# noahares/raxtax

Hardware: AMD Instinct MI355X
Metric: classified queries/sec (whole node) (higher is better)
Workload: dtype u32 bit-planes + f64

## Files before the change

include/raxtax_hip.h:

```cpp
#ifndef RAXTAX_HIP_H
#define RAXTAX_HIP_H

#include <stddef.h>
#include <stdint.h>

#ifdef __cplusplus
extern "C" {
#endif

#define RTX_ABI_VERSION 6
#define RTX_NUM_KMERS 65536u
#define RTX_MAX_DEPTH 32u

#define RTX_OK 0
#define RTX_ERR_INVALID (-1)
#define RTX_ERR_HIP (-2)
#define RTX_ERR_NO_DEVICE (-3)
#define RTX_ERR_OOM (-4)
#define RTX_ERR_PARSE (-5)
#define RTX_ERR_DEPTH (-6)
#define RTX_ERR_STATE (-7)
#define RTX_ERR_TOO_LONG (-8)
#define RTX_ERR_SENDER (-9)
#define RTX_RETRY_CHUNK 1
// ... 48 lines not shown
typedef struct rtx_queries rtx_queries;
int rtx_queries_parse_fasta(const char *text, uint64_t len, const char *const *skip, uint64_t n_skip,
                            rtx_queries **out);
#define RTX_FASTA_MORE_FOLLOWS 1u
#define RTX_FASTA_NOT_FIRST 2u
uint64_t rtx_fasta_block_end(const char *text, uint64_t len);
int rtx_queries_parse_fasta_block(const char *text, uint64_t len, const char *const *skip, uint64_t n_skip, uint32_t flags,
                                  rtx_queries **out);
void rtx_queries_destroy(rtx_queries *q);
uint64_t rtx_queries_len(const rtx_queries *q);
const char *rtx_queries_label(const rtx_queries *q, uint64_t i);
int rtx_queries_data(const rtx_queries *q, const uint8_t **bases, const uint64_t **base_off);

int rtx_index_create(int device, uint64_t n_refs, const uint64_t *offsets ,
                     const uint32_t *postings, uint32_t n_nodes, const uint32_t *node_begin,
                     const uint32_t *node_end, const uint32_t *node_first_child,
                     const uint32_t *node_n_children, const uint8_t *node_type, rtx_index **out);
int rtx_index_create_shard(int device, uint64_t n_refs_total, uint64_t ref_lo, uint64_t ref_hi,
                           const uint64_t *shard_cuts, uint32_t n_cuts, const uint64_t *offsets,
                           const uint32_t *postings, uint32_t n_nodes, const uint32_t *node_begin,
                           const uint32_t *node_end, const uint32_t *node_first_child,
                           const uint32_t *node_n_children, const uint8_t *node_type, rtx_index **out);
int rtx_index_create_from_sequences(int device, uint64_t n_refs, const uint8_t *seq_bytes, const uint64_t *seq_off,
                                    uint32_t n_nodes, const uint32_t *node_begin, const uint32_t *node_end,
                                    const uint32_t *node_first_child, const uint32_t *node_n_children,
                                    const uint8_t *node_type, rtx_index **out);
int rtx_index_create_from_tree(int device, const rtx_tree *tree, rtx_index **out);
void rtx_index_destroy(rtx_index *index);
uint64_t rtx_index_num_refs(const rtx_index *index);
uint64_t rtx_index_device_bytes(const rtx_index *index);
uint64_t rtx_index_workspace_bytes(const rtx_index *index);
int rtx_index_workspace_parts(const rtx_index *index, uint64_t out[9]);
int rtx_index_set_batch(rtx_index *index, uint32_t sub_batch);
#define RTX_OPT_SUB_BATCH 1
#define RTX_OPT_PROB_MODE 2
#define RTX_OPT_STAGE_TIMING 6
#define RTX_OPT_DEBUG_TAPS 14
#define RTX_OPT_DEVICE_EXACT 15
#define RTX_OPT_CLUSTER 7
#define RTX_OPT_PACKED_COUNTS 8
#define RTX_OPT_HIT_PAIR 11
#define RTX_OPT_TILE_SKIP 10
#define RTX_OPT_LOCATOR 12
#define RTX_OPT_TILE_PRUNE 13
#define RTX_OPT_FINE_BOUNDS 17
#define RTX_OPT_RECORDS 18
#define RTX_OPT_OVERLAP 19
#define RTX_OPT_MIN_SUB_BATCHES 20
#define RTX_OPT_TWO_LEVEL_BOUNDS 21
#define RTX_OPT_PRUNE_SELF_SAMPLE 22
#define RTX_OPT_RUN_AHEAD 23
#define RTX_OPT_DEVICE_TEXT 24
#define RTX_OPT_STRAND 25
int rtx_index_set_option(rtx_index *index, int option, uint64_t value);

int rtx_index_self_sample(rtx_index *index, const uint8_t *seq_bytes, const uint64_t *seq_off, uint64_t n_refs, uint32_t n_sample, double *live_fraction);
int rtx_index_prune_verdict(const rtx_index *index, int *pruning, double *live_fraction);
int rtx_index_run_ahead_stats(const rtx_index *index, uint64_t *enqueued_ahead, uint64_t *abandoned);
#define RTX_DEFAULT_SEGMENT_CLASSES 1
#define RTX_DEFAULT_EXACT_HASH_MASK 2
int rtx_set_default_option(int option, uint64_t value);

typedef struct {
    uint32_t n_queries;
    uint64_t n_rows;
    const uint32_t *t;
    const uint8_t *status;
    const double *global_signal;
    const uint64_t *row_begin;
    const uint32_t *row_count;
    const uint32_t *row_lineage;
    const uint32_t *row_node;
    const uint32_t *row_depth;
    const double *row_conf;
    const double *row_local_signal;
    uint32_t row_conf_stride;
    const uint8_t *row_depth_u8;
    const uint8_t *row_conf_hundredths;
} rtx_result_view;

int rtx_batch_prefetch(rtx_index *index, uint64_t n_queries, const uint8_t *bases, const uint64_t *base_off,
                       const uint32_t *exact_ids, const uint64_t *exact_off);
int rtx_batch_activate(rtx_index *index);
int rtx_pack_bases(const uint8_t *bases, uint64_t n_bases, uint8_t *packed);
int rtx_classify_batch(rtx_index *index, uint64_t n_queries, const uint8_t *bases,
                       const uint64_t *base_off, const uint32_t *exact_ids,
                       const uint64_t *exact_off, uint32_t flags, rtx_result_view *out);
int rtx_index_has_exact_lookup(const rtx_index *index);
int rtx_batch_exact_matches(rtx_index *index, const uint64_t **exact_off , const uint32_t **exact_ids);

int rtx_batch_strands(rtx_index *index, const uint8_t **strand, const uint32_t **peak);
int rtx_revcomp(const uint8_t *in, uint64_t n, uint8_t *out);

int rtx_batch_upload(rtx_index *index, uint64_t n_queries, const uint8_t *bases,
                     const uint64_t *base_off, const uint32_t *exact_ids,
                     const uint64_t *exact_off);
int rtx_batch_run(rtx_index *index, uint32_t flags);
int rtx_batch_sync(rtx_index *index);
int rtx_batch_download(rtx_index *index, rtx_result_view *out);
int rtx_batch_download_then_run(rtx_index *index, rtx_result_view *out, uint32_t flags);

typedef struct {
    uint64_t n_queries;
    const char *out;
    const uint64_t *out_off;
    const char *tsv;
    const uint64_t *tsv_off;
} rtx_text_view;
int rtx_index_text_setup(rtx_index *index, const rtx_tree *tree, uint32_t flags);
int rtx_batch_prefetch_labels(rtx_index *index, uint64_t n_queries, const char *const *labels);
int rtx_batch_text(rtx_index *index, rtx_text_view *out);

#define RTX_BUF_HIST 1
#define RTX_BUF_PREFIX 2
int rtx_shard_begin(rtx_index *index, uint32_t *n_sub_batches, uint32_t *sub_batch);
#define RTX_OPT_SHARD_PRUNE 16
int rtx_shard_prunes(const rtx_index *index);
int rtx_shard_bounds(rtx_index *index, uint32_t sub_batch_idx, uint32_t flags);
int rtx_shard_count(rtx_index *index, uint32_t sub_batch_idx, uint32_t flags);
int rtx_shard_prob(rtx_index *index, uint32_t sub_batch_idx);
int rtx_shard_walk(rtx_index *index, uint32_t sub_batch_idx, const double *prefix_global );
int rtx_shard_info(const rtx_index *index, uint64_t *ref_lo, uint64_t *ref_hi, uint32_t *n_bnd_global,
                   uint32_t *n_bnd_local, uint32_t *first_bnd);
int rtx_device_buffer(rtx_index *index, int which, void **device_ptr, uint64_t *row_stride_elems);
#define RTX_BUF_COUNTS 3
#define RTX_BUF_BEST 4
int rtx_shard_buffer(rtx_index *index, uint32_t sub_batch_idx, int which, void **device_ptr, uint64_t *row_stride_elems);
int rtx_shard_rehist(rtx_index *index, uint32_t sub_batch_idx);
int rtx_index_stream(rtx_index *index, void **hip_stream);

#define RTX_STAGE_KMER_EXTRACT 0
#define RTX_STAGE_HIT_COUNT 1
#define RTX_STAGE_PROB_TABLE 2
#define RTX_STAGE_TAXON_PREFIX 3
#define RTX_STAGE_LINEAGE_WALK 4
#define RTX_STAGE_TILE_BOUNDS 5
#define RTX_STAGE_TILE_PRUNE 6
#define RTX_STAGE_EXACT_MATCH 7
#define RTX_STAGE_ORDER 8
#define RTX_STAGE_PAIR_UNION 9
#define RTX_NUM_STAGES 10
int rtx_batch_stage_times(rtx_index *index, float ms[RTX_NUM_STAGES], uint32_t launches[RTX_NUM_STAGES]);
int rtx_batch_work(rtx_index *index, uint64_t *sum_hits, uint64_t *sum_query_bytes,
                   uint64_t *bitmap_bytes_read);
int rtx_batch_work_split(rtx_index *index, uint64_t *live_bytes, uint64_t *bounds_bytes);
int rtx_batch_prob_work(rtx_index *index, uint64_t *sum_grid_points, uint64_t *sum_distinct_counts);

int rtx_debug_kmers(rtx_index *index, uint64_t query, uint16_t *kmers , uint32_t *t);
int rtx_debug_hit_counts(rtx_index *index, uint64_t query, uint16_t *counts );
int rtx_debug_prob_table(rtx_index *index, uint64_t query, double *table_over_z , double *z);
int rtx_debug_probs(rtx_index *index, uint64_t query, double *probs );
int rtx_debug_tile_bounds(rtx_index *index, uint64_t query, uint16_t *tile_ub );
int rtx_debug_order(rtx_index *index, uint32_t *perm );
int rtx_batch_sub_batch(const rtx_index *index, uint32_t *sub_batch, uint32_t *n_sub_batches);
int rtx_batch_last_sub_batch(const rtx_index *index, uint64_t *first, uint32_t *n);
int rtx_batch_classes(const rtx_index *index, uint32_t *n_classes, uint64_t out[20]);
int rtx_debug_prune_stats(rtx_index *index, uint64_t *out );
int rtx_debug_pruned_prob_table(rtx_index *index, uint64_t query, double *table_over_z , double *z, uint32_t *threshold);
int rtx_debug_run_counts(rtx_index *index, uint64_t query, uint16_t *counts , uint8_t *tile_live ,
                         uint32_t *hist , uint32_t *threshold, uint32_t *i1);
int rtx_debug_run_mode(rtx_index *index, uint64_t query, uint32_t *n_segments);
int rtx_debug_prune_detail(rtx_index *index, uint64_t query, uint32_t *out );
int rtx_debug_evaluate(rtx_index *index, const double *probs , rtx_result_view *out);

int64_t rtx_format_query(const rtx_tree *tree, const rtx_result_view *res, uint64_t q,
                         const char *label, const uint8_t *seq, uint64_t seq_len,
                         const uint32_t *exact_ids, uint64_t n_exact, uint32_t flags, char *out_buf,
                         uint64_t out_cap, char *tsv_buf, uint64_t tsv_cap, int64_t *tsv_len);

int64_t rtx_result_pack(const rtx_result_view *res, uint8_t *buf, uint64_t cap);

#define RTX_NEED_BASE 1024
int64_t rtx_records_format(const rtx_tree *tree, const uint8_t *records, uint64_t n_bytes, const char *const *labels,
                           const uint32_t *exact_one, uint32_t flags, char *out, uint64_t cap, uint64_t *line_off, uint32_t threads);

typedef int (*rtx_sender_fn)(void *ctx, const char *label, const char *out_lines, const char *tsv_lines);
int rtx_raxtax(rtx_index *index, const rtx_tree *tree, uint64_t n_queries, const char *const *labels,
               const uint8_t *bases, const uint64_t *base_off, int skip_exact_matches, int raw_confidence,
               uint64_t chunk_size, rtx_sender_fn sender, void *sender_ctx, int tsv);

int rtx_raxtax_multi(rtx_index *const *indices, uint32_t n_indices, const rtx_tree *tree, uint64_t n_queries,
                     const char *const *labels, const uint8_t *bases, const uint64_t *base_off, int skip_exact_matches,
                     int raw_confidence, uint64_t chunk_size, rtx_sender_fn sender, void *sender_ctx, int tsv);
typedef int (*rtx_query_info_fn)(void *ctx, const char *label, int strand, uint32_t peak, uint32_t t);
int rtx_raxtax_multi_ex(rtx_index *const *indices, uint32_t n_indices, const rtx_tree *tree, uint64_t n_queries,
                        const char *const *labels, const uint8_t *bases, const uint64_t *base_off, int skip_exact_matches,
                        int raw_confidence, uint64_t chunk_size, rtx_sender_fn sender, void *sender_ctx, int tsv,
                        rtx_query_info_fn info, void *info_ctx);
int rtx_sender_discard(void *ctx, const char *label, const char *out_lines, const char *tsv_lines);
int rtx_raxtax_last_timing(double busy[4], uint64_t *n_chunks);

int rtx_set_host_share(uint32_t n_ranks_on_this_host);
uint32_t rtx_host_threads(void);

#ifdef __cplusplus
}
#endif
#endif
```

raxtax_amd/_build.py:

```python
from __future__ import annotations

import os
import shutil
import subprocess
from pathlib import Path

PKG = Path(__file__).resolve().parent
ROOT = PKG.parent
CSRC = PKG / "csrc"
LIB = PKG / "libraxtax_hip.so"
SOURCES = ["rtx_kernels.hip", "rtx_hit_pair.hip", "rtx_prob_tables.hip", "rtx_cluster.hip", "rtx_segments.hip", "rtx_prune.hip", "rtx_bounds2.hip", "rtx_records.hip", "rtx_finalise.hip", "rtx_text.hip", "rtx_exact.hip", "rtx_strand.hip", "rtx_ingest.hip", "rtx_api_index.hip", "rtx_api_batch.hip", "rtx_api_download.hip", "rtx_api_shard.hip", "rtx_api_debug.hip", "host_tree.cpp", "host_format.cpp", "host_raxtax.cpp", "host_bin.cpp", "host_threads.cpp"]
HEADERS = ["rtx_index.hpp", "rtx_kernels.hpp", "rtx_hit_common.hpp", "rtx_internal.hpp", "rtx_math.hpp", "rtx_wave.hpp", "rtx_walk.hpp", "host_raxtax.hpp"]
CLI = PKG / "raxtax-hip"
SYNTH = PKG / "raxtax-synth"


def _hipcc() -> str:
    for c in (os.environ.get("HIPCC"), shutil.which("hipcc"), "/opt/rocm/bin/hipcc"):
        if c and Path(c).exists():
            return c
    raise RuntimeError("hipcc not found (ROCm toolchain required to build libraxtax_hip.so)")


def _stale(target: Path, deps) -> bool:
    if not target.exists():
        return True
    t = target.stat().st_mtime
    return any(Path(d).stat().st_mtime > t for d in deps if Path(d).exists())


OBJ = PKG / "_obj"


def build_lib(force: bool = False, verbose: bool = False) -> Path:
    from concurrent.futures import ThreadPoolExecutor

    srcs = [CSRC / s for s in SOURCES if (CSRC / s).exists()]
    hdrs = [CSRC / h for h in HEADERS] + [ROOT / "include" / "raxtax_hip.h"]
    if not force and not _stale(LIB, srcs + hdrs):
        return LIB
    OBJ.mkdir(exist_ok=True)
    flags = ["--offload-arch=gfx950", "-O3", "-std=c++17", "-fPIC", f"-I{ROOT / 'include'}", f"-I{CSRC}"] + os.environ.get("RTX_EXTRA_CXXFLAGS", "").split()

    def compile_one(src: Path) -> Path:
        obj = OBJ / (src.name + ".o")
        if force or _stale(obj, [src] + hdrs):
            cmd = [_hipcc()] + flags + ["-x", "hip", "-c", str(src), "-o", str(obj)]
            if verbose:
                print(" ".join(cmd))
            subprocess.check_call(cmd)
        return obj

    with ThreadPoolExecutor(max_workers=min(len(srcs), os.cpu_count() or 1)) as ex:
        objs = list(ex.map(compile_one, srcs))
    cmd = [_hipcc(), "--offload-arch=gfx950", "-fPIC", "-shared", "-o", str(LIB)] + [str(o) for o in objs] + ["-lpthread"]
    if verbose:
        print(" ".join(cmd))
    subprocess.check_call(cmd)
    return LIB


def build_cli(force: bool = False) -> Path | None:
    main = CSRC / "cli_main.cpp"
    if not main.exists():
        return None
# ... 21 lines not shown
```

raxtax_amd/_lib.py:

```python
from __future__ import annotations

import ctypes as C
from pathlib import Path

import numpy as np

PKG = Path(__file__).resolve().parent
import os as _os

LIB_PATH = Path(_os.environ.get("RTX_LIB_PATH") or PKG / "libraxtax_hip.so")

RTX_MAX_DEPTH = 32
RTX_NUM_KMERS = 65536
RTX_OK = 0
RTX_ERR_INVALID, RTX_ERR_HIP, RTX_ERR_NO_DEVICE, RTX_ERR_OOM = -1, -2, -3, -4
RTX_ERR_PARSE, RTX_ERR_DEPTH, RTX_ERR_STATE, RTX_ERR_TOO_LONG = -5, -6, -7, -8
RTX_SKIP_EXACT_MATCHES = 1
RTX_RAW_CONFIDENCE = 2
RTX_TEXT_TSV = 4
RTX_Q_OK, RTX_Q_NO_KMERS, RTX_Q_ALL_KMERS = 0, 1, 2
STAGES = ("kmer_extract", "hit_count", "prob_table", "taxon_prefix", "lineage_walk", "tile_bounds", "tile_prune", "exact_match", "order", "pair_union")

u8p = C.POINTER(C.c_uint8)
u16p = C.POINTER(C.c_uint16)
# ... 56 lines not shown
    "rtx_index_create": (C.c_int, [C.c_int, C.c_uint64, u64p, u32p, C.c_uint32, u32p, u32p, u32p, u32p, u8p,
                                   C.POINTER(C.c_void_p)]),
    "rtx_index_create_shard": (C.c_int, [C.c_int, C.c_uint64, C.c_uint64, C.c_uint64, u64p, C.c_uint32, u64p, u32p, C.c_uint32,
                                        u32p, u32p, u32p, u32p, u8p, C.POINTER(C.c_void_p)]),
    "rtx_shard_begin": (C.c_int, [C.c_void_p, u32p, u32p]),
    "rtx_shard_count": (C.c_int, [C.c_void_p, C.c_uint32, C.c_uint32]),
    "rtx_shard_bounds": (C.c_int, [C.c_void_p, C.c_uint32, C.c_uint32]),
    "rtx_shard_prunes": (C.c_int, [C.c_void_p]),
    "rtx_shard_prob": (C.c_int, [C.c_void_p, C.c_uint32]),
    "rtx_shard_walk": (C.c_int, [C.c_void_p, C.c_uint32, C.c_void_p]),
    "rtx_shard_info": (C.c_int, [C.c_void_p, u64p, u64p, u32p, u32p, u32p]),
    "rtx_device_buffer": (C.c_int, [C.c_void_p, C.c_int, C.POINTER(C.c_void_p), u64p]),
    "rtx_shard_buffer": (C.c_int, [C.c_void_p, C.c_uint32, C.c_int, C.POINTER(C.c_void_p), u64p]),
    "rtx_shard_rehist": (C.c_int, [C.c_void_p, C.c_uint32]),
    "rtx_index_stream": (C.c_int, [C.c_void_p, C.POINTER(C.c_void_p)]),
    "rtx_index_create_from_sequences": (C.c_int, [C.c_int, C.c_uint64, u8p, u64p, C.c_uint32, u32p, u32p, u32p, u32p, u8p,
                                                 C.POINTER(C.c_void_p)]),
    "rtx_index_create_from_tree": (C.c_int, [C.c_int, C.c_void_p, C.POINTER(C.c_void_p)]),
    "rtx_index_destroy": (None, [C.c_void_p]),
    "rtx_index_num_refs": (C.c_uint64, [C.c_void_p]),
    "rtx_index_device_bytes": (C.c_uint64, [C.c_void_p]),
    "rtx_index_workspace_bytes": (C.c_uint64, [C.c_void_p]),
    "rtx_index_workspace_parts": (C.c_int, [C.c_void_p, u64p]),
    "rtx_index_set_batch": (C.c_int, [C.c_void_p, C.c_uint32]),
    "rtx_set_default_option": (C.c_int, [C.c_int, C.c_uint64]),
    "rtx_index_set_option": (C.c_int, [C.c_void_p, C.c_int, C.c_uint64]),
    "rtx_index_self_sample": (C.c_int, [C.c_void_p, C.c_void_p, C.c_void_p, C.c_uint64, C.c_uint32, C.POINTER(C.c_double)]),
    "rtx_index_prune_verdict": (C.c_int, [C.c_void_p, C.POINTER(C.c_int), C.POINTER(C.c_double)]),
    "rtx_index_run_ahead_stats": (C.c_int, [C.c_void_p, C.POINTER(C.c_uint64), C.POINTER(C.c_uint64)]),
    "rtx_classify_batch": (C.c_int, [C.c_void_p, C.c_uint64, u8p, u64p, u32p, u64p, C.c_uint32,
                                     C.POINTER(ResultView)]),
    "rtx_index_has_exact_lookup": (C.c_int, [C.c_void_p]),
    "rtx_batch_exact_matches": (C.c_int, [C.c_void_p, C.POINTER(u64p), C.POINTER(u32p)]),
    "rtx_batch_upload": (C.c_int, [C.c_void_p, C.c_uint64, u8p, u64p, u32p, u64p]),
    "rtx_batch_run": (C.c_int, [C.c_void_p, C.c_uint32]),
    "rtx_batch_sync": (C.c_int, [C.c_void_p]),
    "rtx_batch_download": (C.c_int, [C.c_void_p, C.POINTER(ResultView)]),
    "rtx_batch_download_then_run": (C.c_int, [C.c_void_p, C.POINTER(ResultView), C.c_uint32]),
    "rtx_index_text_setup": (C.c_int, [C.c_void_p, C.c_void_p, C.c_uint32]),
    "rtx_batch_prefetch_labels": (C.c_int, [C.c_void_p, C.c_uint64, C.POINTER(C.c_char_p)]),
    "rtx_batch_text": (C.c_int, [C.c_void_p, C.POINTER(TextView)]),
    "rtx_batch_stage_times": (C.c_int, [C.c_void_p, f32p, u32p]),
    "rtx_batch_work": (C.c_int, [C.c_void_p, u64p, u64p, u64p]),
    "rtx_batch_prob_work": (C.c_int, [C.c_void_p, u64p, u64p]),
    "rtx_batch_work_split": (C.c_int, [C.c_void_p, u64p, u64p]),
    "rtx_debug_kmers": (C.c_int, [C.c_void_p, C.c_uint64, u16p, u32p]),
    "rtx_debug_hit_counts": (C.c_int, [C.c_void_p, C.c_uint64, u16p]),
    "rtx_debug_prob_table": (C.c_int, [C.c_void_p, C.c_uint64, f64p, f64p]),
    "rtx_debug_pruned_prob_table": (C.c_int, [C.c_void_p, C.c_uint64, f64p, f64p, u32p]),
    "rtx_debug_probs": (C.c_int, [C.c_void_p, C.c_uint64, f64p]),
    "rtx_debug_order": (C.c_int, [C.c_void_p, u32p]),
    "rtx_debug_tile_bounds": (C.c_int, [C.c_void_p, C.c_uint64, u16p]),
    "rtx_debug_prune_stats": (C.c_int, [C.c_void_p, u64p]),
    "rtx_debug_run_counts": (C.c_int, [C.c_void_p, C.c_uint64, u16p, u8p, u32p, u32p, u32p]),
    "rtx_debug_run_mode": (C.c_int, [C.c_void_p, C.c_uint64, u32p]),
    "rtx_batch_last_sub_batch": (C.c_int, [C.c_void_p, u64p, u32p]),
    "rtx_batch_classes": (C.c_int, [C.c_void_p, u32p, u64p]),
    "rtx_debug_prune_detail": (C.c_int, [C.c_void_p, C.c_uint64, u32p]),
    "rtx_debug_evaluate": (C.c_int, [C.c_void_p, f64p, C.POINTER(ResultView)]),
    "rtx_result_pack": (C.c_int64, [C.POINTER(ResultView), u8p, C.c_uint64]),
    "rtx_records_format": (C.c_int64, [C.c_void_p, u8p, C.c_uint64, C.POINTER(C.c_char_p), u32p, C.c_uint32, C.c_char_p, C.c_uint64, u64p, C.c_uint32]),
    "rtx_format_query": (C.c_int64, [C.c_void_p, C.POINTER(ResultView), C.c_uint64, C.c_char_p, u8p, C.c_uint64,
                                     u32p, C.c_uint64, C.c_uint32, C.c_char_p, C.c_uint64, C.c_char_p, C.c_uint64,
                                     C.POINTER(C.c_int64)]),
    "rtx_raxtax": (C.c_int, None),
    "rtx_raxtax_multi": (C.c_int, None),
    "rtx_raxtax_multi_ex": (C.c_int, None),
    "rtx_batch_strands": (C.c_int, [C.c_void_p, C.POINTER(u8p), C.POINTER(u32p)]),
    "rtx_revcomp": (C.c_int, [u8p, C.c_uint64, u8p]),
    "rtx_sender_discard": (C.c_int, [C.c_void_p, C.c_char_p, C.c_char_p, C.c_char_p]),
    "rtx_batch_prefetch": (C.c_int, [C.c_void_p, C.c_uint64, u8p, u64p, u32p, u64p]),
    "rtx_batch_activate": (C.c_int, [C.c_void_p]),
    "rtx_pack_bases": (C.c_int, [u8p, C.c_uint64, u8p]),
    "rtx_batch_sub_batch": (C.c_int, [C.c_void_p, C.POINTER(C.c_uint32), C.POINTER(C.c_uint32)]),
    "rtx_raxtax_last_timing": (C.c_int, [C.POINTER(C.c_double), C.POINTER(C.c_uint64)]),
    "rtx_set_host_share": (C.c_int, [C.c_uint32]),
    "rtx_host_threads": (C.c_uint32, []),
}

_lib = None


def load() -> C.CDLL:
    global _lib
    if _lib is not None:
        return _lib
    if not LIB_PATH.exists():
        raise ImportError(
            f"{LIB_PATH} is missing: build it with `python -m raxtax_amd._build` (hipcc, gfx950). "
            "raxtax_amd has no CPU fallback.")
    try:
        import torch
    except Exception:
        pass
    lib = C.CDLL(str(LIB_PATH))
    for name, (res, args) in _SIGNATURES.items():
        fn = getattr(lib, name)
        fn.restype = res
        if args is not None:
            fn.argtypes = args
    _lib = lib
    return lib


def check(code: int):
    if code < 0:
# ... 7 lines not shown
```

raxtax_amd/api.py:

```python
from __future__ import annotations

import ctypes as C
from dataclasses import dataclass
from typing import Callable, List, Optional, Sequence, Tuple

import numpy as np

from . import _lib
from ._lib import (RTX_MAX_DEPTH, RTX_RAW_CONFIDENCE, RTX_SKIP_EXACT_MATCHES, NodesView, ResultView, RtxError, check,
                   f32p, f64p, ptr, u8p, u16p, u32p, u64p)


def _flatten(seqs: Sequence[np.ndarray]) -> Tuple[np.ndarray, np.ndarray]:
    off = np.zeros(len(seqs) + 1, dtype=np.uint64)
    if len(seqs):
        off[1:] = np.cumsum([len(s) for s in seqs], dtype=np.uint64)
    flat = np.zeros(max(int(off[-1]), 1), dtype=np.uint8)
    for i, s in enumerate(seqs):
        flat[int(off[i]):int(off[i + 1])] = np.asarray(s, dtype=np.uint8)
    return flat, off


class Tree:

# ... 125 lines not shown
class EvaluationResult:
    lineage: int
    node: int
    confidence_values: List[float]
    local_signal: float
    global_signal: float


class Result:

    def __init__(self, view: ResultView, strand: Optional[np.ndarray] = None, peak: Optional[np.ndarray] = None):
        nq, nr = view.n_queries, view.n_rows
        self.strand, self.peak = strand, peak
        arr = lambda p, n: (np.ctypeslib.as_array(p, shape=(n,)).copy() if n else np.zeros(0))
        self.n_queries = nq
        self.t = arr(view.t, nq)
        self.status = arr(view.status, nq)
        self.global_signal = arr(view.global_signal, nq)
        begin = arr(view.row_begin, nq).astype(np.int64)
        count = arr(view.row_count, nq).astype(np.int64)
        self.row_off = np.zeros(nq + 1, dtype=np.uint64)
        self.row_off[1:] = np.cumsum(count)
        src = (np.repeat(begin - self.row_off[:-1].astype(np.int64), count) + np.arange(int(count.sum()))) if nq else np.zeros(0, np.int64)
        assert len(src) <= nr
        self.row_lineage = arr(view.row_lineage, nr)[src]
        self.row_node = arr(view.row_node, nr)[src]
        self.row_depth = arr(view.row_depth, nr)[src]
        stride = int(view.row_conf_stride) or RTX_MAX_DEPTH
        self.row_conf = (np.ctypeslib.as_array(view.row_conf, shape=(nr, stride))[src] if nr
                         else np.zeros((0, stride)))
        self.row_local_signal = arr(view.row_local_signal, nr)[src]

    def rows(self, q: int) -> List[EvaluationResult]:
        out = []
        for r in range(int(self.row_off[q]), int(self.row_off[q + 1])):
            d = int(self.row_depth[r])
            out.append(EvaluationResult(int(self.row_lineage[r]), int(self.row_node[r]),
                                        [float(x) for x in self.row_conf[r, :d]],
                                        float(self.row_local_signal[r]), float(self.global_signal[q])))
        return out


DEFAULT_SEGMENT_CLASSES = 1


class Index:

    def __init__(self, tree: Tree, device: int = 0, sub_batch: int = 0, prob_mode: int = 0,
                 stage_timing: bool = False, cluster: Optional[bool] = None, segment_classes=None,
                 packed_counts: Optional[bool] = None,
                 tile_skip: Optional[bool] = None, hit_pair=None, locator: Optional[bool] = None, tile_prune: Optional[bool] = None,
                 debug_taps: bool = False, device_exact: Optional[bool] = None, fine_bounds: Optional[bool] = None,
                 records: Optional[int] = None, overlap: Optional[bool] = None, two_level: Optional[int] = None,
                 prune_self_sample: Optional[bool] = None, device_text: bool = False, strand: str = "plus"):
        self._lib = _lib.load()
        self.tree = tree
        if segment_classes is None:
            segment_classes = DEFAULT_SEGMENT_CLASSES
        check(self._lib.rtx_set_default_option(1, int(segment_classes)))
        h = C.c_void_p()
        check(self._lib.rtx_index_create_from_tree(device, tree._h, C.byref(h)))
        self._h = h
        self.n_refs = self._lib.rtx_index_num_refs(self._h)
        if sub_batch:
            check(self._lib.rtx_index_set_batch(self._h, sub_batch))
        if prob_mode:
            check(self._lib.rtx_index_set_option(self._h, 2, prob_mode))
        if stage_timing:
            check(self._lib.rtx_index_set_option(self._h, 6, 1))
        if cluster is not None:
            check(self._lib.rtx_index_set_option(self._h, 7, int(cluster)))
        if packed_counts is not None:
            check(self._lib.rtx_index_set_option(self._h, 8, int(packed_counts)))
        if tile_skip is not None:
            check(self._lib.rtx_index_set_option(self._h, 10, int(tile_skip)))
        if hit_pair is not None:
            check(self._lib.rtx_index_set_option(self._h, 11, int(hit_pair)))
        if locator is not None:
            check(self._lib.rtx_index_set_option(self._h, 12, int(locator)))
        if tile_prune is not None:
            check(self._lib.rtx_index_set_option(self._h, 13, int(tile_prune)))
            if tile_prune and prune_self_sample is None:
                check(self._lib.rtx_index_set_option(self._h, 22, 0))
        if debug_taps:
            check(self._lib.rtx_index_set_option(self._h, 14, 1))
        if device_exact is not None:
            check(self._lib.rtx_index_set_option(self._h, 15, int(device_exact)))
        if device_text:
            check(self._lib.rtx_index_set_option(self._h, 24, 1))
        if fine_bounds is not None:
            check(self._lib.rtx_index_set_option(self._h, 17, int(fine_bounds)))
        if records is not None:
            check(self._lib.rtx_index_set_option(self._h, 18, int(records)))
        if overlap is not None:
            check(self._lib.rtx_index_set_option(self._h, 19, int(overlap)))
        if two_level is not None:
            check(self._lib.rtx_index_set_option(self._h, 21, int(two_level)))
        if prune_self_sample is not None:
            check(self._lib.rtx_index_set_option(self._h, 22, int(prune_self_sample)))
        if strand not in ("plus", "both"):
            raise ValueError(f"strand must be 'plus' or 'both', not {strand!r}")
        self.strand = strand
        if strand == "both":
            check(self._lib.rtx_index_set_option(self._h, 25, 1))
        self._view = ResultView()
        self._keep = None

    @property
    def prune_verdict(self):
        on, frac = C.c_int(), C.c_double()
        check(self._lib.rtx_index_prune_verdict(self._h, C.byref(on), C.byref(frac)))
        return bool(on.value), float(frac.value)

    @property
    def run_ahead_stats(self):
        a, b = C.c_uint64(), C.c_uint64()
        check(self._lib.rtx_index_run_ahead_stats(self._h, C.byref(a), C.byref(b)))
        return int(a.value), int(b.value)

    def __del__(self):
        try:
            if self._h:
                self._lib.rtx_index_destroy(self._h)
                self._h = None
        except Exception:
            pass

    @property
    def device_bytes(self) -> int:
        return self._lib.rtx_index_device_bytes(self._h)

    @property
    def workspace_bytes(self) -> int:
        return self._lib.rtx_index_workspace_bytes(self._h)

    def workspace_parts(self) -> dict:
        out = np.zeros(9, dtype=np.uint64)
        check(self._lib.rtx_index_workspace_parts(self._h, ptr(out, u64p)))
        names = ("prob_tables", "counts", "record_segments", "prefix_sums", "tile_masks_and_slot_lists", "other_scratch", "inputs_and_order", "results")
        d = {k: int(v) for k, v in zip(names, out[:8])}
        d["scratch_sets"] = int(out[8])
        return d

    def upload(self, bases: np.ndarray, base_off: np.ndarray, exact_ids: Optional[np.ndarray] = None,
               exact_off: Optional[np.ndarray] = None):
        self.prefetch(bases, base_off, exact_ids, exact_off)
        self.activate()

    def prefetch(self, bases: np.ndarray, base_off: np.ndarray, exact_ids: Optional[np.ndarray] = None,
                 exact_off: Optional[np.ndarray] = None):
        bases = np.ascontiguousarray(bases, dtype=np.uint8)
        base_off = np.ascontiguousarray(base_off, dtype=np.uint64)
# ... 121 lines not shown

    def debug_run_counts(self, q: int, t: int) -> dict:
        counts = np.zeros(self.n_refs, dtype=np.uint16)
        live = np.zeros((self.n_refs + 8191) // 8192, dtype=np.uint8)
        hist = np.zeros(t + 1, dtype=np.uint32)
        thr, i1 = C.c_uint32(), C.c_uint32()
        check(self._lib.rtx_debug_run_counts(self._h, q, ptr(counts, u16p), ptr(live, u8p), ptr(hist, u32p), C.byref(thr), C.byref(i1)))
        nseg = C.c_uint32()
        check(self._lib.rtx_debug_run_mode(self._h, q, C.byref(nseg)))
        return dict(counts=counts, tile_live=live.astype(bool), hist=hist, threshold=int(thr.value), i1=int(i1.value), record_segments=int(nseg.value))

    def debug_tile_bounds(self, q: int) -> np.ndarray:
        out = np.zeros((self.n_refs + 8191) // 8192, dtype=np.uint16)
        check(self._lib.rtx_debug_tile_bounds(self._h, q, ptr(out, u16p)))
        return out

    def debug_prune_detail(self, q: int) -> dict:
        out = np.zeros(72, dtype=np.uint32)
        check(self._lib.rtx_debug_prune_detail(self._h, q, ptr(out, u32p)))
        return dict(block=int(out[0]), M=int(out[1]), threshold=int(out[2]), i1=int(out[3]), largest_bound=int(out[4]), t=int(out[5]),
                    block_counts=out[8:72].copy())

    def debug_probs(self, q: int) -> np.ndarray:
        out = np.zeros(self.n_refs, dtype=np.float64)
        check(self._lib.rtx_debug_probs(self._h, q, ptr(out, f64p)))
        return out

    def sub_batch_size(self) -> int:
        b, n = C.c_uint32(), C.c_uint32()
        check(self._lib.rtx_batch_sub_batch(self._h, C.byref(b), C.byref(n)))
        return int(b.value)

    def last_sub_batch(self):
        first, n = C.c_uint64(), C.c_uint32()
        check(self._lib.rtx_batch_last_sub_batch(self._h, C.byref(first), C.byref(n)))
        return int(first.value), int(n.value)

    def batch_classes(self) -> list:
        n = C.c_uint32()
        out = np.zeros(20, dtype=np.uint64)
        check(self._lib.rtx_batch_classes(self._h, C.byref(n), ptr(out, u64p)))
        res = []
        for c in range(int(n.value)):
            f = int(out[4 * c + 3])
            res.append(dict(queries=int(out[4 * c]), longest=int(out[4 * c + 1]), sub_batch=int(out[4 * c + 2]), planes=f & 0xFF, tables=bool(f >> 8 & 1),
                            pair=bool(f >> 9 & 1), prune=bool(f >> 10 & 1), records=bool(f >> 11 & 1), global_memory_forms=bool(f >> 12 & 1)))
        return res

    def debug_order(self, n_queries: int) -> np.ndarray:
        out = np.zeros(n_queries, dtype=np.uint32)
        check(self._lib.rtx_debug_order(self._h, ptr(out, u32p)))
        return out

    def debug_prune_stats(self) -> dict:
        out = np.zeros(16, dtype=np.uint64)
        check(self._lib.rtx_debug_prune_stats(self._h, ptr(out, u64p)))
        pairs, nq = max(int(out[1]), 1), max(int(out[5]), 1)
        counted = int(out[12]) if int(out[11]) or int(out[12]) else int(out[0])
        return {"live_tiles_per_pair": counted / pairs, "live_tiles_per_pair_first_stage": int(out[0]) / pairs,
                "fine_blocks_per_pair": int(out[11]) / pairs, "fine_cleared_per_query": int(out[10]) / nq, "pairs": int(out[1]), "mean_best_hit_lower_bound": int(out[2]) / nq,
                "mean_threshold": int(out[3]) / nq, "mean_largest_tile_bound": int(out[4]) / nq, "bound_violations": int(out[6]), "live_tiles_per_query": int(out[7]) / nq,
                "tiles_above_threshold_per_query": int(out[8]) / max(int(out[9]), 1), "queries_with_threshold": int(out[9]),
                "record_queries": int(out[14]), "records_per_record_query": int(out[13]) / max(int(out[14]), 1), "record_slow_path_queries": int(out[15])}

    def debug_evaluate(self, probs) -> Result:
        probs = np.ascontiguousarray(probs, dtype=np.float64)
        assert len(probs) == self.n_refs
        check(self._lib.rtx_debug_evaluate(self._h, ptr(probs, f64p), C.byref(self._view)))
        return Result(self._view)

    def format_query(self, q: int, label: str, seq: np.ndarray, exact_ids: np.ndarray, flags: int = 0,
                     tsv: bool = False):
        seq = np.ascontiguousarray(seq, dtype=np.uint8)
        ex = np.ascontiguousarray(exact_ids if len(exact_ids) else np.zeros(1, np.uint32), dtype=np.uint32)
        cap = 1 << 20
        out = C.create_string_buffer(cap)
        tbuf = C.create_string_buffer(cap) if tsv else None
        tlen = C.c_int64()
        n = self._lib.rtx_format_query(self.tree._h, C.byref(self._view), q, label.encode(), ptr(seq, u8p), len(seq),
                                       ptr(ex, u32p), len(exact_ids), flags, out, cap, tbuf, cap, C.byref(tlen))
        check(n)
        return out.raw[:n].decode(), (tbuf.raw[:tlen.value].decode() if tsv else None)


_SENDER = C.CFUNCTYPE(C.c_int, C.c_void_p, C.c_char_p, C.c_char_p, C.c_char_p)
_INFO = C.CFUNCTYPE(C.c_int, C.c_void_p, C.c_char_p, C.c_int, C.c_uint32, C.c_uint32)


def revcomp(seq: np.ndarray) -> np.ndarray:
    seq = np.ascontiguousarray(seq, dtype=np.uint8)
    out = np.zeros(len(seq), dtype=np.uint8)
    check(_lib.load().rtx_revcomp(ptr(seq, u8p), len(seq), ptr(out, u8p)))
    return out


def raxtax(queries: Sequence[Tuple[str, np.ndarray]], tree, skip_exact_matches: bool, raw_confidence: bool,
           chunk_size: int, sender: Callable[[str, str, Optional[str]], None], tsv: bool,
           info: Optional[Callable[[str, int, int, int], None]] = None) -> None:
    lib = _lib.load()
    lib.rtx_raxtax.argtypes = [C.c_void_p, C.c_void_p, C.c_uint64, C.POINTER(C.c_char_p), u8p, u64p, C.c_int, C.c_int,
                               C.c_uint64, _SENDER, C.c_void_p, C.c_int]
    lib.rtx_raxtax_multi.argtypes = [C.POINTER(C.c_void_p), C.c_uint32] + lib.rtx_raxtax.argtypes[1:]
    lib.rtx_raxtax_multi_ex.argtypes = lib.rtx_raxtax_multi.argtypes + [_INFO, C.c_void_p]
    handles = list(tree) if isinstance(tree, (list, tuple)) else [tree]
    labels = (C.c_char_p * max(len(queries), 1))(*[q[0].encode() for q in queries])
    flat, off = _flatten([q[1] for q in queries])
# ... 41 lines not shown
```

raxtax_amd/csrc/rtx_api_batch.hip:

```cpp
#include "rtx_index.hpp"

#ifndef RTX_B2_HEAVY_PER_ATILE
#define RTX_B2_HEAVY_PER_ATILE 4u
#endif

namespace rtxi {

int bind(rtx_index *ix) {
    if (!ix) { set_error("null index handle"); return RTX_ERR_INVALID; }
    RTX_HIP(hipSetDevice(ix->device));
    return RTX_OK;
}

int ensure_events(rtx_index *ix, size_t count) {
    while (ix->events.size() < count) {
        hipEvent_t e;
        RTX_HIP(hipEventCreate(&e));
        ix->events.push_back(e);
    }
    return RTX_OK;
}


SubBatch sub_batch_of(rtx_index *ix, uint32_t sb, bool timed) {
    const rtx_index::SubPlan &p = ix->plan[sb];
    SubBatch b;
    b.sb = sb;
    b.q0 = p.q0;
    b.nq = p.nq;
    b.cls = &ix->cls[p.cls];
    b.set = ix->staged ? (sb & 1u) : 0u;
    b.s = ix->stream;
    b.timed = timed;
    b.timed_all = timed && ix->stage_timing != 0;
    return b;
}

int plan_sub_batches(rtx_index *ix) {
    ix->plan.clear();
    uint64_t pos = 0;
    for (uint32_t c = 0; c < ix->n_cls; c++) {
        ix->cls[c].pos0 = pos;
        pos += ix->cls[c].n;
    }
    if (pos != ix->n_q) { set_error("internal: the length classes hold %llu of %llu queries", (unsigned long long)pos, (unsigned long long)ix->n_q); return RTX_ERR_STATE; }
    for (int pass = 0; pass < 2; pass++)
        for (uint32_t c = 0; c < ix->n_cls; c++) {
            rtx_index::BatchClass &k = ix->cls[c];
            if (k.side != (pass == 0)) continue;
            k.sb0 = ix->n_sub_total();
            for (uint64_t a = 0; a < k.n; a += k.sub_batch) ix->plan.push_back({k.pos0 + a, (uint32_t)std::min<uint64_t>(k.sub_batch, k.n - a), c});
            k.n_sub = ix->n_sub_total() - k.sb0;
        }
    return RTX_OK;
}

constexpr uint32_t kDietMinRows = 1024;
// ... 76 lines not shown
    hp.ref_base = ix->ref_lo;
    hp.rows = sc.d_rows.p;
    hp.rstride = k.rstride;
    hp.dmask = sc.d_dmask.p;
    hp.nrows = sc.d_nrows.p;
    hp.zero_row = ix->n_rows;
    hp.srows = sc.d_srows.p;
    hp.nsparse = sc.d_nsparse.p;
    hp.segslots = ix->d_segslots.p;
    hp.ntiles = ix->ntiles;
    hp.t = sc.d_t.p;
    hp.counts = sc.d_counts.p;
    hp.counts_lo = ix->packs(k.planes) ? counts_lo(ix, sc) : nullptr;
    hp.counts_hi = ix->packs(k.planes) ? counts_hi(ix, k, sc) : nullptr;
    hp.npad = ix->npad;
    hp.hist = sc.d_hist.p;
    hp.hstride = k.hstride;
    hp.tile_max = sc.d_tilemax.p;
    hp.flags = flags;
    hp.q0 = b.q0;
    hp.perm = r.d_perm.p;
    hp.exact = ExactRef{ix->in[ix->cur_in].d_exact_ids.p, ix->in[ix->cur_in].d_exact_off.p, r.dev_exact ? r.d_exact_grp.p : nullptr, ix->d_em_goff.p, ix->d_em_gids.p};
    hp.nq = b.nq;
    hp.group_rows = k.pair ? ix->d_group_rows.p : nullptr;
    hp.group_base = b.sb * ix->groups_per_sub;
    hp.pair_urec = sc.d_urec.p;
    hp.pair_nu = sc.d_nu.p;
    hp.pair_ustride = 2u * k.rstride;
    return hp;
}

static HitParams bounds_params(const rtx_index *ix, const rtx_index::Scratch &sc, const HitParams &hp) {
    HitParams up = hp;
    up.bitmap = ix->d_ubitmap.p;
    up.stride_bytes = ix->u_stride_bytes;
    up.n_refs = ix->u_nblocks;
    up.dmask = nullptr;
    up.nsparse = nullptr;
    up.ntiles = ix->u_ntiles;
    up.counts = nullptr;
    up.counts_lo = nullptr;
    up.counts_hi = nullptr;
    up.hist = nullptr;
    up.tile_max = nullptr;
    up.bounds_tile_ub = sc.d_tile_ub.p;
    up.bounds_tile_stride = ix->ntiles;
    up.bounds_ntiles = ix->ntiles;
    up.bounds_best = sc.d_best_key.p;
    up.flags = 0;
    up.group_base = hp.group_base + ix->n_groups_run;
    return up;
}

static Bounds2Params bounds2_params(const rtx_index *ix, const rtx_index::Scratch &sc, const HitParams &up, bool heavy) {
    Bounds2Params bp{};
    bp.abitmap = ix->d_abitmap.p;
    bp.bbitmap = ix->d_bbitmap.p;
    bp.n_rows1 = ix->n_rows + 1;
    bp.n_atiles = ix->n_atiles;
    bp.ntiles = ix->ntiles;
    bp.zero_row = ix->n_rows;
    bp.pair_urec = sc.d_urec.p;
    bp.pair_nu = sc.d_nu.p;
    bp.pair_ustride = up.pair_ustride;
    bp.nq = up.nq;
    bp.t = sc.d_t.p;
    bp.tile_ub = sc.d_tile_ub.p;
    bp.tile_ub_stride = ix->ntiles;
    bp.best_key = sc.d_best_key.p;
    bp.delta_ct = ix->b2_delta[0];
    bp.delta_cm = ix->b2_delta[1];
    bp.delta_lo = ix->b2_delta[2];
    bp.delta_hi = ix->b2_delta[3];
    bp.group_rows = up.group_rows;
    bp.group_base = up.group_base;
    bp.heavy = heavy ? sc.d_heavy.p : nullptr;
    bp.heavy_max = std::max<uint32_t>(1u, std::min<uint32_t>(RTX_B2_HEAVY_PER_ATILE * ix->n_atiles, ix->n_btiles / 2u));
    return bp;
}

static PruneParams prune_params(rtx_index *ix, const SubBatch &b, uint32_t flags, int part, const ExactRef &exact) {
    rtx_index::Scratch &sc = ix->sc[b.set];
    const rtx_index::BatchClass &k = *b.cls;
    PruneParams pr{};
    pr.tile_ub = sc.d_tile_ub.p;
    pr.best_key = sc.d_best_key.p;
    pr.tile_ub_stride = ix->ntiles;
    pr.ntiles = ix->ntiles;
    pr.nq = b.nq;
    pr.n_refs = ix->n_refs;
    pr.n_total = ix->n_total;
    pr.ref_base = ix->ref_lo;
    pr.phase = (uint32_t)part;
    pr.best = part ? sc.d_best.p : nullptr;
    pr.bitmap = ix->d_bitmap.p;
    pr.cbitmap = part == 0 && (ix->two_level_used || (k.planes > kBounds2MaxPlanes && ix->two_level_opt && ix->n_refs == ix->n_total)) ? reinterpret_cast<const uint2 *>(ix->d_cbitmap.p) : nullptr;
    pr.n_rows1 = ix->n_rows + 1;
    pr.stride_bytes = ix->stride_bytes;
    pr.rows = sc.d_rows.p;
    pr.rstride = k.rstride;
    pr.nrows = sc.d_nrows.p;
    pr.t = sc.d_t.p;
    pr.flags = flags;
    pr.q0 = b.q0;
    pr.perm = ix->res().d_perm.p;
    pr.exact = exact;
    pr.lnfact = ix->d_lnfact.p;
    pr.inv = ix->d_inv.p;
    pr.nlf = std::min<uint32_t>(kLnFactLen, k.tmax + k.tmax / 2 + 2);
    pr.hist = sc.d_hist.p;
    pr.hstride = k.hstride;
    pr.live = sc.d_live.p;
    pr.live_words = LiveLayout{ix->ntiles}.words();
    pr.pair_live = ItemsLayout(b.nq, ix->ntiles).pair_live(sc.d_items.p);
    pr.thr_out = sc.d_prune_thr.p;
    pr.i1_out = sc.d_prune_i1.p;
    pr.stats = ix->d_prune_stats.p;
    pr.detail = ix->debug_taps && ix->d_prune_detail.n >= (size_t)b.nq * kPruneDetailWords ? ix->d_prune_detail.p : nullptr;
    return pr;
}

static HitParams fine_params(const rtx_index *ix, const rtx_index::Scratch &sc, const HitParams &hp) {
    HitParams fp = hp;
    fp.bitmap = ix->d_fbitmap.p;
    fp.stride_bytes = ix->f_stride_bytes;
    fp.n_refs = ix->f_nblocks;
    fp.ntiles = ix->f_ntiles;
    fp.counts = nullptr;
    fp.counts_lo = nullptr;
    fp.counts_hi = nullptr;
    fp.tile_max = nullptr;
    fp.flags = 0;
    fp.group_rows = nullptr;
    fp.live = sc.d_live.p;
    fp.live_words = LiveLayout{ix->ntiles}.words();
    fp.prune_thr = sc.d_prune_thr.p;
    fp.fine_n_refs = ix->n_refs;
    fp.fine_ref_ntiles = ix->ntiles;
    fp.fine_stats = ix->d_prune_stats.p + 2 * kPruneStatCopies * 8;
    return fp;
}

int enqueue_hit(rtx_index *ix, const SubBatch &b, uint32_t flags, hipStream_t s, int part, hipStream_t s_mid) {
    rtx_index::Scratch &sc = ix->sc[b.set];
    rtx_index::ResultSet &r = ix->res();
    const rtx_index::BatchClass &k = *b.cls;
    ix->last_set = b.set;
    HitParams hp = hit_params(ix, b, flags);
    const bool prune = run_prunes(ix, k);
    if (k.pair && part != 2) {
        if (b.timed_all) RTX_HIP(hipEventRecord(stage_event(ix, b, RTX_STAGE_PAIR_UNION, 0), s));
        launch_pair_union(s, sc.d_rows.p, sc.d_nrows.p, k.rstride, b.nq, sc.d_urec.p, sc.d_nu.p, 2u * k.rstride);
        if (b.timed_all) RTX_HIP(hipEventRecord(stage_event(ix, b, RTX_STAGE_PAIR_UNION, 1), s));
    }
    if (b.timed && !prune) RTX_HIP(hipEventRecord(stage_event(ix, b, RTX_STAGE_HIT_COUNT, 0), s));
    if (part != 0 && !prune) { set_error("internal: a split run without tile pruning"); return RTX_ERR_STATE; }
    if (prune) {
        if (part != 2) {
            const HitParams up = bounds_params(ix, sc, hp);
            if (b.timed) RTX_HIP(hipEventRecord(stage_event(ix, b, RTX_STAGE_TILE_BOUNDS, 0), s));
            ix->two_level_used = part == 0 && ix->two_level_opt && ix->d_abitmap.p && ix->d_bbitmap.p && ix->n_refs == ix->n_total && k.planes <= kBounds2MaxPlanes;
            if (ix->two_level_used) {
                const bool heavy_ok = sc.d_heavy.p && sc.d_heavy_items.p && sc.d_heavy_items.n >= HeavyItemsLayout(b.nq, ix->u_ntiles).total();
                launch_bounds2(s, bounds2_params(ix, sc, up, heavy_ok), b.nq, k.planes, up, ix->u_ntiles, heavy_ok ? sc.d_heavy_items.p : nullptr);
            } else {
                RTX_HIP(hipMemsetAsync(sc.d_best_key.p, 0, (size_t)b.nq * 4, s));
                launch_hit_count_pair_bounds(s, up, b.nq, ix->u_ntiles, k.planes);
            }
            if (b.timed) RTX_HIP(hipEventRecord(stage_event(ix, b, RTX_STAGE_TILE_BOUNDS, 1), s));
        }
        if (s_mid && s_mid != s && part == 0) {
            RTX_HIP(hipEventRecord(ix->ev_mid[b.sb], s));
            RTX_HIP(hipStreamWaitEvent(s_mid, ix->ev_mid[b.sb], 0));
            s = s_mid;
        }
        if (b.timed && part != 1) RTX_HIP(hipEventRecord(stage_event(ix, b, RTX_STAGE_TILE_PRUNE, 0), s));
        PruneParams pr = prune_params(ix, b, flags, part, hp.exact);
        const bool records = part == 0 && on_records_path(ix, k, sc), diet = part == 0 && on_diet(ix, k, sc);
        const RecordRef rr = record_ref(ix, sc, r);
        if (records) { pr.rec = rr; pr.rec_max_slots = rr.stride; }
        if (k.diet && !diet) { set_error("internal: the counts buffer is on its diet without the records path"); return RTX_ERR_STATE; }
        if (diet) {
            RTX_HIP(hipMemsetAsync(sc.d_cnt_cursor.p, 0, 4, s));
            pr.cnt_row = sc.d_cnt_row.p;
            pr.cnt_cursor = sc.d_cnt_cursor.p;
            pr.cnt_cap = k.cnt_rows;
            pr.flags_out = r.d_flags.p;
            hp.cnt_row = sc.d_cnt_row.p;
        }
        launch_prune(s, pr, prob_tables(ix), b.nq);
        if (part == 1) { RTX_HIP(hipGetLastError()); return RTX_OK; }
        if (part == 0 && ix->fine_opt && ix->d_fbitmap.p && k.pair && sc.d_fine_items.p) {
            const FineItemsLayout fine(b.nq, ix->f_ntiles);
            uint32_t *const fi = sc.d_fine_items.p;
            launch_fine_bounds(s, fine_params(ix, sc, hp), b.nq, ix->ntiles, ix->f_ntiles, pr.pair_live, fine.cursors(fi), fine.items(fi), fine.count(fi), k.planes);
        }
        RTX_HIP(hipMemsetAsync(sc.d_tilemax.p, 0, (size_t)b.nq * ix->ntiles * 2, s));
        hp.live = sc.d_live.p;
        hp.live_words = pr.live_words;
        hp.prune_thr = sc.d_prune_thr.p;
        if (records) hp.rec = rr;
        if (k.pair) {
            const ItemsLayout items(b.nq, ix->ntiles);
            launch_live_items(s, sc.d_live.p, pr.live_words, pr.pair_live, b.nq, ix->ntiles, items.offsets(sc.d_items.p), items.items(sc.d_items.p), items.count(sc.d_items.p));
            hp.items = items.items(sc.d_items.p);
            hp.n_items = items.count(sc.d_items.p);
        }
        if (ix->seg_blocks) {
            KmerParams kp = kmer_params(ix, b);
            kp.mode = 2u;
            kp.live = sc.d_live.p;
            kp.live_words = pr.live_words;
            launch_kmer_extract(s, kp, b.nq);
        }
        if (b.timed) {
            RTX_HIP(hipEventRecord(stage_event(ix, b, RTX_STAGE_TILE_PRUNE, 1), s));
            RTX_HIP(hipEventRecord(stage_event(ix, b, RTX_STAGE_HIT_COUNT, 0), s));
        }
    }
    if (k.pair) launch_hit_count_pair(s, hp, b.nq, ix->ntiles, k.planes);
    else launch_hit_count(s, hp, b.nq, ix->ntiles, k.planes);
    if (b.timed) RTX_HIP(hipEventRecord(stage_event(ix, b, RTX_STAGE_HIT_COUNT, 1), s));
    ix->hit_stream = s;
    return RTX_OK;
}

int enqueue_count(rtx_index *ix, const SubBatch &b, uint32_t flags, hipStream_t s_mid) {
    int rc = enqueue_kmer(ix, b, b.s);
    return rc ? rc : enqueue_hit(ix, b, flags, b.s, 0, s_mid);
}

static WalkParams walk_params(rtx_index *ix, const SubBatch &b, const double *prefix);
static int reset_sub_alloc(rtx_index *ix, hipStream_t s);

int enqueue_prob_prefix(rtx_index *ix, const SubBatch &b, bool fuse_walk, bool prob_only) {
    rtx_index::Scratch &sc = ix->sc[b.set];
    const rtx_index::BatchClass &k = *b.cls;
    hipStream_t s = b.s;
    ProbParams pp{};
    pp.t = sc.d_t.p;
    pp.hist = sc.d_hist.p;
    pp.hstride = k.hstride;
    pp.tmax = k.tmax;
    pp.n1max = k.tmax / 2 + 1;
    pp.lnfact = ix->d_lnfact.p;
    pp.n_refs = ix->n_total;
    pp.q0 = b.q0;
    pp.table_z = sc.d_table_z.p;
    rtx_index::ResultSet &r = ix->res();
    pp.z = r.d_z.p;
    pp.gs = r.d_gs.p;
    pp.status = r.d_status.p;
    pp.ndist = r.d_ndist.p;
    pp.prune_thr = run_prunes(ix, k) ? sc.d_prune_thr.p : nullptr;
    pp.prune_i1 = pp.prune_thr ? sc.d_prune_i1.p : nullptr;
    if (b.timed_all) RTX_HIP(hipEventRecord(stage_event(ix, b, RTX_STAGE_PROB_TABLE, 0), s));
    if (k.use_tables) {
        launch_prob_order(s, sc.d_t.p, b.nq, sc.d_order.p);
        pp.order = sc.d_order.p;
        launch_prob_lookup(s, pp, prob_tables(ix), b.nq);
    } else {
        if (k.huge) {
            pp.gstride = (uint32_t)((prob_table_lds_bytes(k.tmax) + 7) / 8);
            if (ix->d_prob_scratch.n < (size_t)b.nq * pp.gstride) { set_error("internal: scratch of prob_table too small"); return RTX_ERR_STATE; }
            pp.gscratch = ix->d_prob_scratch.p;
        }
        launch_prob_table(s, pp, b.nq);
    }
    if (b.timed_all) RTX_HIP(hipEventRecord(stage_event(ix, b, RTX_STAGE_PROB_TABLE, 1), s));
    if (prob_only) return RTX_OK;

    PrefixParams fp{};
// ... 246 lines not shown
    }
    RTX_HIP(hipMemsetAsync(r.d_flags.p, 0, sizeof(uint32_t), ix->stream));
    RTX_HIP(hipMemsetAsync(r.d_fin_cursor.p, 0, 2 * sizeof(unsigned long long), ix->stream));
    const bool whole = ix->n_refs == ix->n_total && !ix->staged;
    const bool shard = ix->staged && ix->shard_prune_opt && ix->n_refs != ix->n_total;
    auto scratch_ok = [&](const rtx_index::Scratch &sc, uint32_t B) {
        const ScratchNeed n = ScratchNeed().set_queries(ix, B);
        return sc.d_tile_ub.p != nullptr && sc.d_tile_ub.n >= n.tile_ub && sc.d_best_key.n >= n.best_key && sc.d_prune_thr.n >= n.prune_thr &&
               sc.d_live.n >= n.live && sc.d_best.n >= n.best && sc.d_items.n >= n.items;
    };
    bool any_pair = false, any_prune = false;
    uint32_t b_max = 1;
    for (uint32_t c = 0; c < ix->n_cls; c++) {
        rtx_index::BatchClass &k = ix->cls[c];
        k.pair = ix->pair_opt && cluster && k.planes <= 11 && ix->n_q > 1 && k.rstride <= 4096;
        const rtx_index::Scratch &s0 = ix->sc[k.side ? kSideSet : 0u];
        ScratchNeed need = ScratchNeed().set_queries(ix, k.sub_batch);
        if (whole && ix->rec_opt != 0u && ix->pruning())
            for (uint32_t j = 0; j < 4u; j++) {
                rtx_index::Scratch &sc = ix->sc[j];
                if ((j == kSideSet) != k.side || sc.d_kmers.p == nullptr || sc.d_rec.p == nullptr || sc.d_rec.n >= need.rec) continue;
                RTX_HIP(hipStreamSynchronize(ix->stream));
                if (sc.d_rec.alloc(need.rec)) sc.d_rec.release();
            }
        k.prune = ix->pruning() && k.pair && k.use_tables && ix->tile_skip && ix->d_ubitmap.p && (whole || shard) &&
                  scratch_ok(s0, k.sub_batch) && (!ix->staged || scratch_ok(ix->sc[1], k.sub_batch));
        k.rec = k.prune && whole && ix->rec_opt != 0u && ix->n_bnd_local == ix->n_bnd && s0.d_rec.p != nullptr && s0.d_rec.n >= need.rec;
        auto diet_ok = [&](const rtx_index::Scratch &sc) { return sc.d_rec.p != nullptr && sc.d_cnt_row.p != nullptr && sc.d_cnt_cursor.p != nullptr && sc.d_cnt_row.n >= need.cnt_row; };
        k.diet = k.rec && diet_rows(ix, k.sub_batch) < k.sub_batch && diet_ok(s0);
        if (k.diet && !k.side)
            for (uint32_t j = 1; j <= 2u; j++)
                if (ix->sc[j].d_kmers.p != nullptr && !diet_ok(ix->sc[j])) k.diet = false;
        k.cnt_rows = k.diet ? diet_rows(ix, k.sub_batch) : k.sub_batch;
        {
            need.add_class(ix, k, k.sub_batch, k.cnt_rows);
            for (uint32_t j = 0; j < 4u; j++) {
                rtx_index::Scratch &sc = ix->sc[j];
                if ((j == kSideSet) != k.side || sc.d_kmers.p == nullptr || (sc.d_counts.n >= need.counts && sc.d_prefix.n >= need.prefix)) continue;
                RTX_HIP(hipStreamSynchronize(ix->stream));
                int rc_c = sc.d_counts.alloc(need.counts);
                if (!rc_c) rc_c = sc.d_prefix.alloc(need.prefix);
                if (rc_c) return rc_c;
            }
        }
        any_pair = any_pair || k.pair;
        any_prune = any_prune || k.prune;
        b_max = std::max(b_max, k.sub_batch);
    }
    ix->sub_batch_max = b_max;
    ix->any_prune = any_prune;
    ix->groups_per_sub = (b_max + 1u) / 2u;
    ix->dbg_full = false;
    if (any_prune) {
        int rc_s = ix->d_prune_stats.alloc(kPruneStatCopies * 32);
        if (!rc_s && ix->debug_taps) rc_s = ix->d_prune_detail.alloc((size_t)b_max * kPruneDetailWords);
        if (rc_s) return rc_s;
        RTX_HIP(hipMemsetAsync(ix->d_prune_stats.p, 0, kPruneStatCopies * 256, ix->stream));
    }
    if (any_pair) {
        ix->n_groups_run = n_sub * ix->groups_per_sub;
        int rc_g = ix->d_group_rows.alloc((size_t)2 * n_sub * ix->groups_per_sub);
        if (rc_g) return rc_g;
        RTX_HIP(hipMemsetAsync(ix->d_group_rows.p, 0, (size_t)2 * n_sub * ix->groups_per_sub * 4, ix->stream));
    }
    ix->n_sub_last = timed ? n_sub : 0;
    ix->overlap_used = 0;
    if (ix->overlap_opt != 0u && whole && n_sub >= 2 && !ix->shared_device && any_prune && ix->sc[1].d_kmers.p != nullptr && scratch_ok(ix->sc[1], b_max) == scratch_ok(ix->sc[0], b_max)) {
        ix->overlap_used = 2;
        if (ix->overlap_opt >= 2u && n_sub >= 3 && ix->sc[2].d_kmers.p != nullptr && scratch_ok(ix->sc[2], b_max) == scratch_ok(ix->sc[0], b_max)) ix->overlap_used = 3;
    }
    if (r.dev_exact) {
        ExactParams xp{ix->d_bases.p, ix->in[ix->cur_in].d_base_off.p, (uint32_t)ix->n_q, ix->d_em_table.p, ix->em_bits, ix->d_em_rep_off.p,
                       ix->d_em_rep_bytes.p, r.d_exact_grp.p, ix->em_hash_mask};
        const bool ev = timed && ix->stage_timing;
        if (ev) RTX_HIP(hipEventRecord(ix->events[(size_t)RTX_STAGE_EXACT_MATCH * 2], ix->stream));
        launch_exact_match(ix->stream, xp);
        if (ev) RTX_HIP(hipEventRecord(ix->events[(size_t)RTX_STAGE_EXACT_MATCH * 2 + 1], ix->stream));
        if (!r.ev_exact) RTX_HIP(hipEventCreateWithFlags(&r.ev_exact, hipEventDisableTiming));
        RTX_HIP(hipEventRecord(r.ev_exact, ix->stream));
    }
    *n_sub_out = n_sub;
    *timed_out = timed;
    return RTX_OK;
}

int enqueue_batch(rtx_index *ix, uint32_t flags) {
    if (ix->n_refs != ix->n_total) {
        set_error("this handle holds a reference shard: drive it with rtx_shard_count/_prob/_walk");
        return RTX_ERR_STATE;
    }
    uint32_t n_sub = 0;
    bool timed = false;
    int rc;
    if (ix->join_pending && !ix->hold_join && (rc = settle_join(ix))) return rc;
    rc = begin_run(ix, &n_sub, &timed, ix->cluster != 0);
    if (rc) return rc;
    rtx_index::ResultSet &r = ix->res();
    if (n_sub <= 4096) {
        if (!ix->copy_stream) RTX_HIP(hipStreamCreateWithFlags(&ix->copy_stream, hipStreamNonBlocking));
        while (r.ev_sub.size() < n_sub) {
            hipEvent_t e;
            RTX_HIP(hipEventCreateWithFlags(&e, hipEventDisableTiming));
            r.ev_sub.push_back(e);
        }
        if ((rc = r.h_cursor_sub.resize(n_sub)) || (rc = r.h_fin_sub.resize(n_sub))) return rc;
        r.stream_dl = true;
    }
    const bool fuse = ix->n_bnd_local == ix->n_bnd;
    const uint32_t nsets = ix->overlap_used;
    const bool overlap = nsets != 0u;
// ... 271 lines not shown
        for (uint32_t c = 1; c < ix->n_cls; c++)
            if (ix->cls[c].n > ix->cls[bulk].n) bulk = c;
        worst = 0;
        for (uint32_t c = 0; c < ix->n_cls; c++) {
            ix->cls[c].side = ix->n_refs == ix->n_total && c != bulk && ix->cls[c].n <= kSideMaxQueries && ix->cls[c].n * 64u <= ix->cls[bulk].n;
            if (!ix->cls[c].side) worst = std::max<uint64_t>(worst, (uint64_t)ix->cls[c].sub_batch * class_per_q(ix, ix->cls[c]));
        }
    }
    {
        uint64_t n_side_q = 0;
        for (uint32_t c = 0; c < ix->n_cls; c++)
            if (ix->cls[c].side) n_side_q += ix->cls[c].n;
        const uint64_t want2 = want_arena + (n_side_q ? n_side_q * kWalkMaxRows + 64 : 0);
        if (r.arena_cap < want2) {
            if ((rc = r.d_arena.alloc(want2))) return rc;
            r.arena_cap = want2;
        }
    }
    while (n_sets > 1u && (uint64_t)n_sets * worst > budget) n_sets--;
    ix->staged = false;
    if ((rc = plan_sub_batches(ix))) return rc;
    if ((rc = alloc_scratch_set(ix, 0))) return rc;
    {
        bool any_side = false;
        for (uint32_t c = 0; c < ix->n_cls; c++) any_side = any_side || ix->cls[c].side;
        if (any_side) { if ((rc = alloc_scratch_set(ix, kSideSet))) return rc; }
        else ix->sc[kSideSet].release_all();
    }
    for (uint32_t k = 1; k <= 2u; k++) {
        if (k < n_sets && ix->n_sub_total() > 1) {
            if (alloc_scratch_set(ix, k)) ix->sc[k].d_kmers.release();
        } else if (ix->n_refs == ix->n_total) {
            ix->sc[k].release_all();
        }
    }
    return RTX_OK;
}

int alloc_scratch_set(rtx_index *ix, uint32_t k) {
    int rc;
    rtx_index::Scratch &sc = ix->sc[k];
    const ScratchNeed n = scratch_set_need(ix, k);
    if ((rc = sc.d_kmers.alloc(n.kmers)) || (rc = sc.d_rows.alloc(n.rows)) || (rc = sc.d_dmask.alloc(n.dmask)) || (rc = sc.d_nsparse.alloc(n.nsparse)) || (rc = sc.d_srows.alloc(n.srows)) ||
        (rc = sc.d_t.alloc(n.t)) || (rc = sc.d_nrows.alloc(n.nrows)) || (rc = sc.d_counts.alloc(n.counts)) || (rc = sc.d_hist.alloc(n.hist)) || (rc = sc.d_table_z.alloc(n.hist)) ||
        (rc = sc.d_prefix.alloc(n.prefix)) || (rc = sc.d_order.alloc(n.order)) || (rc = sc.d_tilemax.alloc(n.tilemax)) || (rc = sc.d_urec.alloc(n.urec)) || (rc = sc.d_nu.alloc(n.nu)))
        return rc;
    if (n.prob_scratch && (rc = ix->d_prob_scratch.alloc(std::max(n.prob_scratch, ix->d_prob_scratch.n)))) return rc;
    if (ix->pruning() && ix->d_ubitmap.p && (ix->n_refs == ix->n_total || ix->shard_prune_opt)) {
        if ((rc = sc.d_tile_ub.alloc(n.tile_ub)) || (rc = sc.d_best_key.alloc(n.best_key)) || (rc = sc.d_prune_thr.alloc(n.prune_thr)) || (rc = sc.d_prune_i1.alloc(n.prune_i1)) ||
            (rc = sc.d_best.alloc(n.best)) || (rc = sc.d_live.alloc(n.live)) || (rc = sc.d_items.alloc(n.items)))
            return rc;
        if (ix->d_abitmap.p && (sc.d_heavy.alloc(n.heavy) || sc.d_heavy_items.alloc(n.heavy_items))) { sc.d_heavy.release(); sc.d_heavy_items.release(); }
        if (ix->d_fbitmap.p && sc.d_fine_items.alloc(n.fine_items)) sc.d_fine_items.release();
        if (ix->rec_opt && ix->n_refs == ix->n_total) {
            if (sc.d_rec_nslots.alloc(n.rec_nslots) || sc.d_rec_slots.alloc(n.rec_slots) || sc.d_rec_cnt.alloc(n.rec_cnt) ||
                sc.d_rec.alloc(n.rec) || sc.d_cnt_row.alloc(n.cnt_row) || sc.d_cnt_cursor.alloc(n.cnt_cursor))
                sc.d_rec.release();
        }
    }
    return RTX_OK;
}

}

extern "C" {

int rtx_batch_prefetch(rtx_index *ix, uint64_t n_queries, const uint8_t *bases, const uint64_t *base_off,
                       const uint32_t *exact_ids, const uint64_t *exact_off) {
    int rc = bind(ix);
    if (rc) return rc;
    rtx_index::Inputs &in = ix->in[ix->cur_in ^ 1u];
    const bool with_labels = in.labels_pending && in.n_labels == n_queries;
    in.labels_pending = in.has_labels = false;
    if (n_queries == 0 || !base_off || (!bases && base_off[n_queries])) {
        set_error("rtx_batch_upload: invalid argument");
        return RTX_ERR_INVALID;
    }
    const bool both = ix->strand_opt != 0u;
    if (both) {
        if (exact_off || exact_ids) { set_error("RTX_OPT_STRAND: exact-match ids cannot be passed in (those of the reverse complements must come from the same lookup: pass NULL)"); return RTX_ERR_INVALID; }
        if (!rtx_index_has_exact_lookup(ix) || ix->n_refs != ix->n_total) { set_error("RTX_OPT_STRAND needs the exact-match lookup of the device (a handle built from the reference sequences, RTX_OPT_DEVICE_EXACT on)"); return RTX_ERR_STATE; }
        if (n_queries > 0x7FFFFFFFull) { set_error("RTX_OPT_STRAND: too many queries in one batch"); return RTX_ERR_INVALID; }
    }
    const uint64_t n_dev = both ? 2 * n_queries : n_queries;
    if (!ix->h2d_stream) RTX_HIP(hipStreamCreateWithFlags(&ix->h2d_stream, hipStreamNonBlocking));
    if (!in.ready) RTX_HIP(hipEventCreateWithFlags(&in.ready, hipEventDisableTiming));
    if (in.recorded) RTX_HIP(hipEventSynchronize(in.ready));
    in.staged = false;
    if (ix->ev_activated) RTX_HIP(hipStreamWaitEvent(ix->h2d_stream, ix->ev_activated, 0));
    uint64_t max_len = 0;
    uint64_t cls_n[5] = {0, 0, 0, 0, 0}, cls_max[5] = {0, 0, 0, 0, 0};
    {
        const uint64_t lim3 = class3_max_len();
        for (uint64_t q = 0; q < n_queries; q++) {
            if (base_off[q + 1] < base_off[q]) { set_error("base_off not monotone at query %llu", (unsigned long long)q); return RTX_ERR_INVALID; }
            const uint64_t len = base_off[q + 1] - base_off[q];
            max_len = std::max(max_len, len);
            const int c = len <= 262 ? 0 : (len <= 1030 ? 1 : (len <= kMidClassMaxT + 7 ? 2 : (len <= lim3 ? 3 : 4)));
            cls_n[c]++;
            cls_max[c] = std::max(cls_max[c], len);
        }
    }
    const uint64_t total = base_off[n_queries] - base_off[0];
    uint64_t n_exact = 0;
    if (exact_off) {
        if (exact_off[0] != 0) { set_error("exact_off[0] must be 0"); return RTX_ERR_INVALID; }
// ... 108 lines not shown
```

raxtax_amd/csrc/rtx_api_debug.hip:

```cpp
#include "rtx_index.hpp"

extern "C" {

int rtx_batch_stage_times(rtx_index *ix, float ms[RTX_NUM_STAGES], uint32_t launches[RTX_NUM_STAGES]) {
    int rc = bind(ix);
    if (rc) return rc;
    if (!ix->synced) { set_error("rtx_batch_stage_times: batch not synchronised"); return RTX_ERR_STATE; }
    for (int s = 0; s < RTX_NUM_STAGES; s++) { ms[s] = 0.f; launches[s] = 0; }
    for (uint32_t sb = 0; sb < ix->n_sub_last; sb++) {
        const rtx_index::BatchClass &kc = ix->cls[ix->plan[sb].cls];
        for (int s = 0; s < RTX_NUM_STAGES; s++) {
            if (s == RTX_STAGE_EXACT_MATCH) {
                if (sb != 0 || !ix->dev_exact_used || !ix->stage_timing) continue;
            } else if (s == RTX_STAGE_ORDER) {
                if (sb != 0 || !ix->stage_timing) continue;
            } else if (s == RTX_STAGE_PAIR_UNION) {
                if (!kc.pair || !ix->stage_timing) continue;
            } else if (s == RTX_STAGE_TILE_BOUNDS || s == RTX_STAGE_TILE_PRUNE ? !kc.prune : (s != RTX_STAGE_HIT_COUNT && !ix->stage_timing)) continue;
            float t = 0.f;
            RTX_HIP(hipEventElapsedTime(&t, ix->events[((size_t)sb * RTX_NUM_STAGES + s) * 2],
                                        ix->events[((size_t)sb * RTX_NUM_STAGES + s) * 2 + 1]));
            ms[s] += t;
            launches[s]++;
        }
// ... 264 lines not shown
}

int rtx_debug_run_mode(rtx_index *ix, uint64_t query, uint32_t *n_segments) {
    uint32_t slot;
    int rc = debug_slot_as_run(ix, query, &slot);
    if (rc) return rc;
    if (!n_segments) { set_error("null argument"); return RTX_ERR_INVALID; }
    uint16_t n_seg = 0;
    rtx_index::Scratch &sc = ix->sc[ix->last_set];
    if (ix->last_cls().prune && ix->last_cls().rec && sc.d_rec_nslots.p) RTX_HIP(hipMemcpy(&n_seg, sc.d_rec_nslots.p + slot, 2, hipMemcpyDeviceToHost));
    *n_segments = n_seg;
    return RTX_OK;
}

int rtx_debug_prune_detail(rtx_index *ix, uint64_t query, uint32_t *out) {
    uint32_t slot;
    int rc = debug_slot_as_run(ix, query, &slot);
    if (rc) return rc;
    if (!out) { set_error("null argument"); return RTX_ERR_INVALID; }
    if (!ix->last_cls().prune || !ix->debug_taps || ix->d_prune_detail.n < (size_t)(slot + 1) * kPruneDetailWords) {
        set_error("rtx_debug_prune_detail: the last run did not prune, or RTX_OPT_DEBUG_TAPS was off");
        return RTX_ERR_STATE;
    }
    RTX_HIP(hipMemcpy(out, ix->d_prune_detail.p + (size_t)slot * kPruneDetailWords, kPruneDetailWords * 4, hipMemcpyDeviceToHost));
    return RTX_OK;
}

int rtx_debug_tile_bounds(rtx_index *ix, uint64_t query, uint16_t *tile_ub) {
    uint32_t slot;
    int rc = debug_slot_as_run(ix, query, &slot);
    if (rc) return rc;
    if (!tile_ub) { set_error("null argument"); return RTX_ERR_INVALID; }
    rtx_index::Scratch &sc = ix->sc[ix->last_set];
    if (!ix->last_cls().prune || sc.d_tile_ub.n < (size_t)(slot + 1) * ix->ntiles) { set_error("rtx_debug_tile_bounds: the last run did not prune"); return RTX_ERR_STATE; }
    RTX_HIP(hipMemcpy(tile_ub, sc.d_tile_ub.p + (size_t)slot * ix->ntiles, (size_t)ix->ntiles * 2, hipMemcpyDeviceToHost));
    return RTX_OK;
}

int rtx_debug_prune_stats(rtx_index *ix, uint64_t *out) {
    if (!ix || !out) { set_error("null argument"); return RTX_ERR_INVALID; }
    std::memset(out, 0, 128);
    if (!ix->any_prune || !ix->d_prune_stats.p) return RTX_OK;
    RTX_HIP(hipStreamSynchronize(ix->stream));
    unsigned long long h[kPruneStatCopies * 32];
    RTX_HIP(hipMemcpy(h, ix->d_prune_stats.p, sizeof(h), hipMemcpyDeviceToHost));
    for (uint32_t c = 0; c < kPruneStatCopies; c++) {
        for (uint32_t k = 0; k < 8; k++) out[k] += h[c * 8 + k];
        for (uint32_t k = 0; k < 2; k++) out[8 + k] += h[(kPruneStatCopies + c) * 8 + k];
        for (uint32_t k = 0; k < 3; k++) out[10 + k] += h[(2 * kPruneStatCopies + c) * 8 + k];
        out[13] += h[(3 * kPruneStatCopies + c) * 8 + 0];
        out[14] += h[(3 * kPruneStatCopies + c) * 8 + 1];
        out[15] += h[(3 * kPruneStatCopies + c) * 8 + 3];
    }
    return RTX_OK;
}

int rtx_batch_sub_batch(const rtx_index *ix, uint32_t *sub_batch, uint32_t *n_sub) {
    if (!ix) { set_error("null index handle"); return RTX_ERR_INVALID; }
    if (!ix->uploaded || ix->n_cls == 0 || ix->cls[ix->n_cls - 1].sub_batch == 0) { set_error("rtx_batch_sub_batch: no batch has been uploaded"); return RTX_ERR_STATE; }
    if (sub_batch) *sub_batch = ix->cls[ix->n_cls - 1].sub_batch;
    if (n_sub) *n_sub = ix->n_sub_total();
    return RTX_OK;
}

int rtx_batch_last_sub_batch(const rtx_index *ix, uint64_t *first, uint32_t *n) {
    if (!ix) { set_error("null index handle"); return RTX_ERR_INVALID; }
    if (!ix->uploaded) { set_error("rtx_batch_last_sub_batch: no batch has been uploaded"); return RTX_ERR_STATE; }
    if (first) *first = ix->plan.back().q0;
    if (n) *n = ix->plan.back().nq;
    return RTX_OK;
}

int rtx_batch_classes(const rtx_index *ix, uint32_t *n_classes, uint64_t out[20]) {
    if (!ix || !n_classes || !out) { set_error("null argument"); return RTX_ERR_INVALID; }
    if (!ix->uploaded) { set_error("rtx_batch_classes: no batch has been uploaded"); return RTX_ERR_STATE; }
    *n_classes = ix->n_cls;
    for (uint32_t c = 0; c < ix->n_cls && c < 5u; c++) {
        out[c * 4 + 0] = ix->cls[c].n;
        out[c * 4 + 1] = ix->cls[c].max_len;
        out[c * 4 + 2] = ix->cls[c].sub_batch;
        out[c * 4 + 3] = (uint64_t)ix->cls[c].planes | (ix->cls[c].use_tables ? 1ull << 8 : 0) | (ix->cls[c].pair ? 1ull << 9 : 0) | (ix->cls[c].prune ? 1ull << 10 : 0) |
                         (ix->cls[c].rec ? 1ull << 11 : 0) | (ix->cls[c].huge ? 1ull << 12 : 0);
    }
    return RTX_OK;
}

int rtx_debug_order(rtx_index *ix, uint32_t *perm) {
    if (!ix || !perm) { set_error("null argument"); return RTX_ERR_INVALID; }
    int rc = bind(ix);
    if (rc) return rc;
    if (!ix->ran || ix->res().d_perm.n < ix->n_q) { set_error("rtx_debug_order: no batch has been run"); return RTX_ERR_STATE; }
    RTX_HIP(hipStreamSynchronize(ix->stream));
    RTX_HIP(hipMemcpy(perm, ix->res().d_perm.p, (size_t)ix->n_q * 4, hipMemcpyDeviceToHost));
    return RTX_OK;
}

int rtx_debug_probs(rtx_index *ix, uint64_t query, double *probs) {
    uint32_t slot;
    int rc = debug_slot(ix, query, &slot);
    if (rc) return rc;
    if ((rc = ix->d_probs_dbg.alloc(ix->n_refs))) return rc;
    const uint16_t *src = nullptr;
    if ((rc = debug_counts_u16(ix, slot, &src))) return rc;
    launch_probs_expand(ix->stream, src, ix->sc[ix->last_set].d_table_z.p + (size_t)slot * ix->last_cls().hstride, ix->n_refs, ix->d_probs_dbg.p);
    RTX_HIP(hipStreamSynchronize(ix->stream));
    RTX_HIP(hipMemcpy(probs, ix->d_probs_dbg.p, ix->n_refs * 8, hipMemcpyDeviceToHost));
// ... 78 lines not shown
```

raxtax_amd/csrc/rtx_api_index.hip:

```cpp
#include "rtx_index.hpp"

namespace rtx {
int index_device(const rtx_index *index) { return index ? index->device : -1; }
void index_set_shared_device(rtx_index *index, bool shared) { if (index) index->shared_device = shared; }
uint32_t index_swap_min_subs(rtx_index *index, uint32_t v) { if (!index) return 0; const uint32_t old = index->min_subs; index->min_subs = v; return old; }
bool index_strand(const rtx_index *index) { return index && index->strand_opt != 0u; }
bool index_device_text(const rtx_index *index) { return index && index->device_text_opt != 0u; }
uint32_t index_swap_run_ahead(rtx_index *index, uint32_t v) {
    if (!index) return 0;
    const uint32_t old = index->run_ahead_opt;
    (void)rtx_index_set_option(index, RTX_OPT_RUN_AHEAD, v);
    return old;
}
}

namespace {

double statrs_ln_gamma(double x) {
    static const double dk[11] = {2.48574089138753565546e-5, 1.05142378581721974210,  -3.45687097222016235469,
                                  4.51227709466894823700,    -2.98285225323576655721, 1.05639711577126713077,
                                  -1.95428773191645869583e-1, 1.70970543404441224307e-2,
                                  -5.71926117404305781283e-4, 4.63399473359905636708e-6,
                                  -2.71994908488607703910e-9};
    const double r = 10.900511, ln_2_sqrt_e_over_pi = 0.6207822376352452223455184457816472122518527279025978;
    double s = dk[0];
    for (int i = 1; i < 11; i++) s += dk[i] / (x + (double)i - 1.0);
    return std::log(s) + ln_2_sqrt_e_over_pi + (x - 0.5) * std::log((x - 0.5 + r) / M_E);
}
void fill_ln_factorial(std::vector<double> &lf) {
    lf.resize(kLnFactLen);
    double f = 1.0;
    for (uint32_t x = 0; x < kLnFactLen; x++) {
        if (x <= 170) {
            if (x > 0) f *= (double)x;
            lf[x] = std::log(f);
        } else {
            lf[x] = statrs_ln_gamma((double)x + 1.0);
        }
    }
}

}

extern "C" {

int rtx_device_count(void) {
    int n = 0;
    if (hipGetDeviceCount(&n) != hipSuccess) return 0;
    return n;
}


static int create_common(int device, uint64_t n_total, uint64_t ref_lo, uint64_t ref_hi, const uint64_t *cuts,
                         uint32_t n_cuts, uint32_t n_nodes, const uint32_t *node_begin, const uint32_t *node_end,
                         const uint32_t *node_first_child, const uint32_t *node_n_children, const uint8_t *node_type,
                         rtx_index **out) {
    if (!out || !node_begin || !node_end || !node_first_child || !node_n_children || !node_type || n_total == 0 ||
        n_total > 0xFFFFFFFFull || ref_lo >= ref_hi || ref_hi > n_total) {
        set_error("rtx_index_create: invalid argument");
        return RTX_ERR_INVALID;
    }
    const uint64_t n_refs = ref_hi - ref_lo;
    int ndev = 0;
    if (hipGetDeviceCount(&ndev) != hipSuccess || ndev <= 0 || device < 0 || device >= ndev) {
        set_error("no usable HIP device (requested %d of %d); libraxtax_hip has no CPU fallback", device, ndev);
        return RTX_ERR_NO_DEVICE;
    }
    RTX_HIP(hipSetDevice(device));
    hipDeviceProp_t prop;
    RTX_HIP(hipGetDeviceProperties(&prop, device));
    if (strncmp(prop.gcnArchName, "gfx950", 6) != 0) {
        set_error("device %d is %s; this library carries gfx950 (MI355X) code objects only", device, prop.gcnArchName);
        return RTX_ERR_NO_DEVICE;
    }
    auto ix = new rtx_index();
    ix->device = device;
    ix->n_refs = n_refs;
    ix->n_total = n_total;
    ix->ref_lo = (uint32_t)ref_lo;
    int rc = RTX_OK;
    auto fail = [&](int code) { delete ix; return code; };
    if (!derive_flat_nodes(n_total, n_nodes, node_begin, node_end, node_first_child, node_n_children, node_type, ix->nodes))
        return fail(RTX_ERR_INVALID);
    if (ix->nodes.max_depth > RTX_MAX_DEPTH) {
        set_error("lineage depth %u exceeds RTX_MAX_DEPTH=%u", ix->nodes.max_depth, RTX_MAX_DEPTH);
        return fail(RTX_ERR_DEPTH);
    }
    if ((rc = node_tables(ix))) return fail(rc);
    if (hipStreamCreateWithFlags(&ix->stream, hipStreamNonBlocking) != hipSuccess) {
        set_error("hipStreamCreate failed");
        return fail(RTX_ERR_HIP);
    }
    {
        std::vector<uint32_t> b;
        b.reserve(2 * (size_t)n_nodes + 2);
        b.push_back(0);
        b.push_back((uint32_t)n_total);
        b.push_back((uint32_t)ref_lo);
        b.push_back((uint32_t)ref_hi);
        for (uint32_t c = 0; c < n_cuts; c++) {
            if (cuts[c] > n_total) { set_error("shard cut %llu beyond n_refs", (unsigned long long)cuts[c]); return fail(RTX_ERR_INVALID); }
            b.push_back((uint32_t)cuts[c]);
        }
        for (uint32_t v = 0; v < n_nodes; v++) { b.push_back(ix->nodes.begin[v]); b.push_back(ix->nodes.end[v]); }
        std::sort(b.begin(), b.end());
        b.erase(std::unique(b.begin(), b.end()), b.end());
        ix->bnd = std::move(b);
        ix->n_bnd = (uint32_t)ix->bnd.size();
        std::vector<uint32_t> blo(n_nodes), bhi(n_nodes);
        for (uint32_t v = 0; v < n_nodes; v++) {
            blo[v] = (uint32_t)(std::lower_bound(ix->bnd.begin(), ix->bnd.end(), ix->nodes.begin[v]) - ix->bnd.begin());
            bhi[v] = (uint32_t)(std::lower_bound(ix->bnd.begin(), ix->bnd.end(), ix->nodes.end[v]) - ix->bnd.begin());
        }
        const size_t nchunk = (size_t)((n_refs + 7) / 8);
        std::vector<uint8_t> bits(nchunk, 0);
        std::vector<uint32_t> rank(nchunk, 0);
        ix->bnd_first = (uint32_t)(std::lower_bound(ix->bnd.begin(), ix->bnd.end(), (uint32_t)ref_lo) - ix->bnd.begin());
        ix->n_bnd_local = 1;
        for (uint32_t j = 1; j < ix->n_bnd; j++) {
            if (ix->bnd[j] <= ref_lo || ix->bnd[j] > ref_hi) continue;
            const uint32_t r = ix->bnd[j] - 1 - (uint32_t)ref_lo;
            bits[r >> 3] |= (uint8_t)(1u << (r & 7u));
            ix->n_bnd_local++;
        }
        uint32_t run = 1;
        for (size_t c = 0; c < nchunk; c++) {
            rank[c] = run;
            run += (uint32_t)__builtin_popcount(bits[c]);
// ... 290 lines not shown
    ix->u_stride_bytes = ix->u_ntiles * 1024u;
    const size_t words = (size_t)(ix->n_rows + 1) * (ix->u_stride_bytes / 4);
    if (ix->d_ubitmap.alloc(words)) { ix->d_ubitmap.release(); return false; }
    if (hipMemsetAsync(ix->d_ubitmap.p, 0, words * 4, ix->stream) != hipSuccess) { (void)hipGetLastError(); ix->d_ubitmap.release(); return false; }
    return true;
}

static bool prepare_fine_bitmap(rtx_index *ix) {
    if (!ix->d_ubitmap.p || ix->ntiles < kFineMinTiles || ix->n_refs != ix->n_total) return false;
    ix->f_nblocks = (ix->n_refs + (1ull << kFineShift) - 1) >> kFineShift;
    ix->f_ntiles = (uint32_t)((ix->f_nblocks + 8191) / 8192);
    ix->f_stride_bytes = ix->f_ntiles * 1024u;
    const size_t words = (size_t)(ix->n_rows + 1) * (ix->f_stride_bytes / 4);
    if (ix->d_fbitmap.alloc(words)) { ix->d_fbitmap.release(); return false; }
    if (hipMemsetAsync(ix->d_fbitmap.p, 0, words * 4, ix->stream) != hipSuccess) { (void)hipGetLastError(); ix->d_fbitmap.release(); return false; }
    return true;
}

static void build_two_level(rtx_index *ix) {
    if (!ix->d_ubitmap.p || ix->n_refs != ix->n_total || ix->ntiles < kTwoLevelMinTiles) return;
    static_assert(kPruneShift == 6, "level B of the two-level bounds pass holds the blocks of the union bitmap");
    ix->n_btiles = (uint32_t)((ix->u_nblocks + 511) / 512);
    ix->n_atiles = (uint32_t)((ix->u_nblocks + 8191) / 8192);
    const size_t rows1 = (size_t)ix->n_rows + 1;
    if (rows1 * 256u > 0xFFFFFFFFull) return;
    if ((uint64_t)ix->u_ntiles * rows1 * 256u > 0xFFFFFFFFull) return;
    if ((size_t)ix->n_atiles * 256u + 32768u > 160u * 1024u) { ix->n_atiles = ix->n_btiles = 0; return; }
    if (ix->d_abitmap.alloc((size_t)ix->n_atiles * rows1 * 64) || ix->d_bbitmap.alloc((size_t)ix->n_btiles * rows1 * 64)) {
        ix->d_abitmap.release();
        ix->d_bbitmap.release();
        return;
    }
    hipError_t e = hipMemsetAsync(ix->d_abitmap.p, 0, (size_t)ix->n_atiles * rows1 * 256, ix->stream);
    if (e == hipSuccess) e = hipMemsetAsync(ix->d_bbitmap.p, 0, (size_t)ix->n_btiles * rows1 * 64, ix->stream);
    if (e == hipSuccess) {
        launch_bounds2_build(ix->stream, ix->d_ubitmap.p, (uint32_t)rows1, ix->u_ntiles, ix->d_bbitmap.p, ix->d_abitmap.p);
        e = hipGetLastError();
        if (e == hipSuccess) e = hipStreamSynchronize(ix->stream);
    }
    if (e != hipSuccess) { (void)hipGetLastError(); ix->d_abitmap.release(); ix->d_bbitmap.release(); return; }
    const size_t cbytes = (size_t)((ix->n_refs + 63) / 64) * rows1 * 8;
    size_t free_b = 0, total_b = 0;
    if (hipMemGetInfo(&free_b, &total_b) != hipSuccess || cbytes > free_b / 4 || cbytes > total_b / 16 || ix->d_cbitmap.alloc(cbytes)) {
        (void)hipGetLastError();
        ix->d_cbitmap.release();
        return;
    }
    e = hipMemsetAsync(ix->d_cbitmap.p, 0, cbytes, ix->stream);
    if (e == hipSuccess) {
        launch_block_major_build(ix->stream, ix->d_bitmap.p, (uint32_t)rows1, ix->ntiles, ix->stride_bytes, ix->d_cbitmap.p);
        e = hipGetLastError();
        if (e == hipSuccess) e = hipStreamSynchronize(ix->stream);
    }
    if (e != hipSuccess) { (void)hipGetLastError(); ix->d_cbitmap.release(); }
}

static void build_locator(rtx_index *ix, const uint8_t *d_seq, const uint64_t *d_off, uint64_t n_refs) {
    if (ix->n_refs != ix->n_total || n_refs < 256) return;
    DevBuf<uint32_t> d_cnt;
    if (ix->d_loc_table.alloc(kLocTableEntries) || d_cnt.alloc(kLocTableEntries)) { ix->d_loc_table.release(); return; }
    hipError_t e = hipMemsetAsync(ix->d_loc_table.p, 0xFF, (size_t)kLocTableEntries * 4, ix->stream);
    if (e == hipSuccess) e = hipMemsetAsync(d_cnt.p, 0, (size_t)kLocTableEntries * 4, ix->stream);
    if (e == hipSuccess) {
        launch_loc_mark(ix->stream, d_seq, d_off, n_refs, ix->d_loc_table.p, d_cnt.p);
        launch_loc_finish(ix->stream, ix->d_loc_table.p, d_cnt.p);
        e = hipStreamSynchronize(ix->stream);
    }
    if (e != hipSuccess) { (void)hipGetLastError(); ix->d_loc_table.release(); }
}

static thread_local bool g_from_tree = false;

int rtx_index_create_from_sequences(int device, uint64_t n_refs, const uint8_t *seq_bytes, const uint64_t *seq_off,
                                    uint32_t n_nodes, const uint32_t *node_begin, const uint32_t *node_end,
                                    const uint32_t *node_first_child, const uint32_t *node_n_children,
                                    const uint8_t *node_type, rtx_index **out) {
    if (!seq_off || (!seq_bytes && n_refs && seq_off[n_refs])) { set_error("rtx_index_create_from_sequences: null sequences"); return RTX_ERR_INVALID; }
    rtx_index *ix = nullptr;
    int rc = create_common(device, n_refs, 0, n_refs, nullptr, 0, n_nodes, node_begin, node_end, node_first_child,
                           node_n_children, node_type, &ix);
    if (rc) return rc;
    auto fail = [&](int code) { delete ix; return code; };
    const uint64_t total = seq_off[n_refs] - seq_off[0];
    DevBuf<uint8_t> d_seq;
    DevBuf<uint64_t> d_off;
    DevBuf<uint32_t> d_present;
    if ((rc = d_seq.alloc(total + 16)) || (rc = d_off.alloc(n_refs + 1)) || (rc = d_present.alloc(2048)) ||
        (rc = ix->d_row_of.alloc(RTX_NUM_KMERS)) || (rc = ix->d_list_len.alloc(RTX_NUM_KMERS)))
        return fail(rc);
    std::vector<uint64_t> off0(n_refs + 1);
    for (uint64_t i = 0; i <= n_refs; i++) off0[i] = seq_off[i] - seq_off[0];
    hipError_t e = hipMemcpy(d_seq.p, seq_bytes + seq_off[0], total, hipMemcpyHostToDevice);
    if (e == hipSuccess) e = hipMemcpy(d_off.p, off0.data(), (n_refs + 1) * 8, hipMemcpyHostToDevice);
    if (e == hipSuccess) e = hipMemsetAsync(d_present.p, 0, 2048 * 4, ix->stream);
    if (e == hipSuccess) {
        launch_ref_kmer_mark(ix->stream, d_seq.p, d_off.p, n_refs, d_present.p);
        e = hipStreamSynchronize(ix->stream);
    }
    std::vector<uint32_t> present(2048, 0), row_of(RTX_NUM_KMERS, kEmptyRow);
    if (e == hipSuccess) e = hipMemcpy(present.data(), d_present.p, 2048 * 4, hipMemcpyDeviceToHost);
    if (e != hipSuccess) { set_error("k-mer marking failed: %s", hipGetErrorString(e)); return fail(RTX_ERR_HIP); }
    uint32_t nr = 0;
    for (uint32_t k = 0; k < RTX_NUM_KMERS; k++)
        if (present[k >> 5] & (1u << (k & 31u))) row_of[k] = nr++;
    ix->n_rows = nr;
    const size_t words = (size_t)(nr + 1) * (ix->stride_bytes / 4);
    if ((rc = ix->d_bitmap.alloc(words))) return fail(rc);
// ... 77 lines not shown
    ix->self_live = -1.0;
    if (ix->n_refs != ix->n_total || n_refs != ix->n_total || !ix->d_ubitmap.p || ix->ntiles < RTX_PRUNE_MIN_TILES) return RTX_OK;
    const uint64_t n = std::min<uint64_t>(n_sample ? n_sample : 1024u, n_refs);
    std::vector<uint64_t> off(n + 1, 0);
    std::vector<uint8_t> bases;
    for (uint64_t i = 0; i < n; i++) {
        const uint64_t r = i * n_refs / n;
        bases.insert(bases.end(), seq_bytes + seq_off[r], seq_bytes + seq_off[r + 1]);
        off[i + 1] = bases.size();
    }
    if (bases.empty()) return RTX_OK;
    const uint32_t prune_was = ix->prune_opt, taps_was = ix->debug_taps;
    ix->prune_opt = 1u;
    ix->debug_taps = 0u;
    uint64_t st[16] = {0};
    int rc = rtx_batch_upload(ix, n, bases.data(), off.data(), nullptr, nullptr);
    if (rc == RTX_OK) rc = rtx_batch_run(ix, RTX_SKIP_EXACT_MATCHES);
    if (rc == RTX_OK) rc = rtx_batch_sync(ix);
    if (rc == RTX_OK) rc = rtx_debug_prune_stats(ix, st);
    ix->prune_opt = prune_was;
    ix->debug_taps = taps_was;
    ix->uploaded = ix->ran = ix->synced = false;
    if (rc != RTX_OK) return RTX_OK;
    if (st[5] != 0) {
        ix->self_live = (double)st[7] / ((double)st[5] * (double)ix->ntiles);
        ix->prune_pays = ix->self_live < kSelfSampleOff;
    }
    if (live_fraction) *live_fraction = ix->self_live;
    return RTX_OK;
}
int rtx_index_prune_verdict(const rtx_index *ix, int *pruning, double *live_fraction) {
    if (!ix) { set_error("null index handle"); return RTX_ERR_INVALID; }
    if (pruning) *pruning = ix->pruning() ? 1 : 0;
    if (live_fraction) *live_fraction = ix->self_live;
    return RTX_OK;
}

int rtx_index_run_ahead_stats(const rtx_index *ix, uint64_t *enqueued_ahead, uint64_t *abandoned) {
    if (!ix) { set_error("null index handle"); return RTX_ERR_INVALID; }
    if (enqueued_ahead) *enqueued_ahead = ix->n_run_ahead;
    if (abandoned) *abandoned = ix->n_run_ahead_retry;
    return RTX_OK;
}

void rtx_index_destroy(rtx_index *index) {
    if (!index) return;
    (void)hipSetDevice(index->device);
    delete index;
}

uint64_t rtx_index_num_refs(const rtx_index *index) { return index ? index->n_total : 0; }
uint64_t rtx_index_device_bytes(const rtx_index *index) {
    if (!index) return 0;
    return index->d_seg_dbits.n * 8 + index->d_seg_sbits.n * 8 + index->d_seg_sbase.n * 4 + index->d_seginfo.n * 4 + index->d_segcls.n * 4 + index->d_segslots.n * 2 + index->d_bitmap.n * 4 + index->d_row_of.n * 4 + index->d_row_len.n * 8 + index->d_list_len.n * 4 + index->d_loc_table.n * 4 + index->d_ubitmap.n * 4 + index->d_fbitmap.n * 4 + index->d_abitmap.n * 4 + index->d_bbitmap.n + index->d_cbitmap.n + index->d_em_table.n * 8 + index->d_em_rep_off.n * 8 + index->d_em_rep_bytes.n + index->d_em_goff.n * 4 + index->d_em_gids.n * 4 + index->d_lnfact.n * 8 +
           index->d_noderec.n * 16 + index->d_bnd_bits.n + index->d_bnd_rank.n * 4;
}
uint64_t rtx_index_workspace_bytes(const rtx_index *ix) {
    if (!ix) return 0;
    uint64_t b = (ix->d_tab_cmf.n + ix->d_tab_ratio.n) * 8 + ix->d_tab_off.n * 8 + ix->d_tab_moff.n * 4 + (ix->d_tab_ilo.n + ix->d_tab_sat.n) * 2 + ix->d_node_depth.n + ix->d_node_sig0.n + ix->d_node_begin.n * 4 + ix->d_node_eb.n * 8;
    for (const auto &sc : ix->sc) b += sc.bytes();
    for (const auto &in : ix->in) b += in.d_packed.n + (in.d_base_off.n + in.d_exact_off.n) * 8 + in.d_exact_ids.n * 4;
    b += ix->d_bases.n + ix->d_prob_scratch.n * 8 + (ix->d_skey_in.n + ix->d_skey_out.n) * 8 + ix->d_sidx.n * 4 + ix->d_sort_tmp.n + ix->d_group_rows.n * 4;
    for (const auto &r : ix->rs) {
        const rtx_index::ResultSet::Bytes s = r.bytes();
        b += s.order + s.groups + s.rest;
    }
    return b;
}
int rtx_index_workspace_parts(const rtx_index *ix, uint64_t out[9]) {
    if (!ix || !out) { set_error("null argument"); return RTX_ERR_INVALID; }
    for (int i = 0; i < 9; i++) out[i] = 0;
    out[0] = (ix->d_tab_cmf.n + ix->d_tab_ratio.n) * 8 + ix->d_tab_off.n * 8 + ix->d_tab_moff.n * 4 + (ix->d_tab_ilo.n + ix->d_tab_sat.n) * 2;
    for (const auto &sc : ix->sc) {
        if (!sc.d_kmers.p) continue;
        out[8]++;
        out[1] += sc.d_counts.bytes();
        out[2] += sc.d_rec.bytes() + sc.d_rec_cnt.bytes() + sc.d_rec_nslots.bytes() + sc.d_rec_slots.bytes();
        out[3] += sc.d_prefix.bytes();
        out[4] += sc.d_dmask.bytes() + sc.d_srows.bytes() + sc.d_nsparse.bytes();
    }
    out[6] = ix->d_bases.n + (ix->d_skey_in.n + ix->d_skey_out.n) * 8 + ix->d_sidx.n * 4 + ix->d_sort_tmp.n;
    for (const auto &in : ix->in) out[6] += in.d_packed.n + (in.d_base_off.n + in.d_exact_off.n) * 8 + in.d_exact_ids.n * 4;
    for (const auto &r : ix->rs) {
        const rtx_index::ResultSet::Bytes s = r.bytes();
        out[6] += s.order;
        out[7] += s.rest;
    }
    const uint64_t all = rtx_index_workspace_bytes(ix);
    uint64_t named = 0;
    for (int i = 0; i < 8; i++) named += out[i];
    out[5] = all > named ? all - named : 0;
    return RTX_OK;
}
int rtx_index_set_batch(rtx_index *index, uint32_t sub_batch) {
    if (!index) { set_error("null index handle"); return RTX_ERR_INVALID; }
    index->uploaded = index->ran = index->synced = false;
    index->sub_batch_req = sub_batch;
    return RTX_OK;
}

int rtx_set_default_option(int option, uint64_t value) {
    if (option == RTX_DEFAULT_SEGMENT_CLASSES) { g_seg_classes = value ? 1 : 0; return RTX_OK; }
    if (option == RTX_DEFAULT_EXACT_HASH_MASK) { g_em_hash_mask = value ? value : ~0ull; return RTX_OK; }
    set_error("rtx_set_default_option: unknown option %d", option);
    return RTX_ERR_INVALID;
}

int rtx_index_set_option(rtx_index *index, int option, uint64_t value) {
    if (!index) { set_error("null index handle"); return RTX_ERR_INVALID; }
    switch (option) {
        case RTX_OPT_SUB_BATCH: case RTX_OPT_PACKED_COUNTS: case RTX_OPT_HIT_PAIR: case RTX_OPT_TILE_PRUNE: case RTX_OPT_PROB_MODE:
            index->uploaded = index->ran = index->synced = false;
            break;
        default: break;
    }
    switch (option) {
        case RTX_OPT_SUB_BATCH: index->sub_batch_req = (uint32_t)value; return RTX_OK;
        case RTX_OPT_STAGE_TIMING:
            index->stage_timing = value ? 1u : 0u;
            return RTX_OK;
        case RTX_OPT_DEBUG_TAPS:
            index->debug_taps = value ? 1u : 0u;
            return RTX_OK;
        case RTX_OPT_SHARD_PRUNE:
            index->uploaded = index->ran = index->synced = false;
            index->shard_prune_opt = value ? 1u : 0u;
            return RTX_OK;
        case RTX_OPT_DEVICE_EXACT:
            index->uploaded = index->ran = index->synced = false;
            index->dev_exact_opt = value ? 1u : 0u;
            return RTX_OK;
        case RTX_OPT_CLUSTER:
            index->cluster = value ? 1u : 0u;
            return RTX_OK;
        case RTX_OPT_PACKED_COUNTS:
            index->packed_opt = value ? 1u : 0u;
            return RTX_OK;
        case RTX_OPT_HIT_PAIR:
            index->pair_opt = value ? 1u : 0u;
            return RTX_OK;
        case RTX_OPT_TILE_SKIP:
            index->tile_skip = value ? 1u : 0u;
            return RTX_OK;
        case RTX_OPT_LOCATOR:
            index->locator_opt = value ? 1u : 0u;
            return RTX_OK;
        case RTX_OPT_TILE_PRUNE:
            index->prune_opt = value ? 1u : 0u;
            return RTX_OK;
        case RTX_OPT_FINE_BOUNDS:
            index->fine_opt = value ? 1u : 0u;
            return RTX_OK;
        case RTX_OPT_PRUNE_SELF_SAMPLE:
            index->uploaded = index->ran = index->synced = false;
            index->self_sample_opt = value ? 1u : 0u;
            return RTX_OK;
        case RTX_OPT_RUN_AHEAD:
            index->run_ahead_opt = (uint32_t)std::min<uint64_t>(value, 2u);
            if (!value && index->join_pending) {
                int rc_b = bind(index);
                if (!rc_b) rc_b = settle_join(index);
                return rc_b;
            }
            return RTX_OK;
        case RTX_OPT_DEVICE_TEXT:
            index->device_text_opt = value ? 1u : 0u;
            return RTX_OK;
        case RTX_OPT_STRAND:
            if (value > 1) break;
            if (value && index->n_refs != index->n_total) { set_error("RTX_OPT_STRAND: not on a reference-shard handle (the peak of a query is spread over the shards)"); return RTX_ERR_INVALID; }
            index->uploaded = index->ran = index->synced = false;
            index->in[0].staged = index->in[1].staged = false;
            index->ws_valid = false;
            index->strand_opt = (uint32_t)value;
            return RTX_OK;
        case RTX_OPT_TWO_LEVEL_BOUNDS:
            index->two_level_opt = value ? 1u : 0u;
            if (value > 1) {
                index->b2_delta[0] = (uint32_t)(value & 0xFFFFu);
                index->b2_delta[1] = (uint32_t)((value >> 16) & 0xFFFFu);
                index->b2_delta[2] = (uint32_t)((value >> 32) & 0xFFFFu);
                index->b2_delta[3] = (uint32_t)((value >> 48) & 0xFFFFu);
            }
            return RTX_OK;
        case RTX_OPT_MIN_SUB_BATCHES:
            if (value < 1 || value > 64) break;
            index->uploaded = index->ran = index->synced = false;
            index->min_subs = (uint32_t)value;
            return RTX_OK;
        case RTX_OPT_OVERLAP:
            index->uploaded = index->ran = index->synced = false;
            if (value > 2) break;
            index->overlap_opt = (uint32_t)value;
            return RTX_OK;
        case RTX_OPT_RECORDS:
            if (value > kRecMaxSlots) break;
            index->uploaded = index->ran = index->synced = false;
            index->rec_opt = (uint32_t)value;
            return RTX_OK;
        case RTX_OPT_PROB_MODE:
            if (value > 2) break;
            index->prob_mode = (int)value;
            return RTX_OK;
        default: break;
    }
    set_error("rtx_index_set_option: unknown option %d / value %llu", option, (unsigned long long)value);
    return RTX_ERR_INVALID;
}

}
```

raxtax_amd/csrc/rtx_bounds2.hip:

```cpp
#include <hip/hip_runtime.h>

#include <algorithm>
#include <type_traits>

#include "rtx_hit_common.hpp"

namespace rtx {

constexpr uint32_t kB2Pad = 256u;
constexpr uint32_t b2_cap(int planes) { return planes > 10 ? 2048u : 1024u; }
constexpr uint32_t b2_lds_dw(int planes) { return 3u * b2_cap(planes) + kB2Pad; }

template <int SHIFT>
__device__ __forceinline__ void load_unit(uint4 (&buf)[8], __amdgpu_buffer_rsrc_t rsrc, const uint32_t *unit, uint32_t grp, uint32_t col) {
    const uint4 i0 = reinterpret_cast<const uint4 *>(unit)[grp * 2u], i1 = reinterpret_cast<const uint4 *>(unit)[grp * 2u + 1u];
    const uint32_t id[8] = {i0.x, i0.y, i0.z, i0.w, i1.x, i1.y, i1.z, i1.w};
#pragma unroll
    for (int j = 0; j < 8; j++) {
        const u32x4_t v = __builtin_amdgcn_raw_buffer_load_b128(rsrc, (id[j] << SHIFT) + col, 0, 0);
        buf[j] = make_uint4(v.x, v.y, v.z, v.w);
    }
}

template <int NP, int MODE, int R, int NB, int SHIFT>
__device__ __forceinline__ void fold_list(uint32_t (&pa)[4][NP], uint32_t (&pb)[4][NP], uint4 (&buf)[4][8], const uint32_t *list, uint32_t ng,
                                          const uint32_t *next, uint32_t grp, uint32_t col, __amdgpu_buffer_rsrc_t rsrc) {
    constexpr uint32_t kUnit = 8u * (uint32_t)R, kGroup = kUnit * (uint32_t)NB;
    for (uint32_t g = 0; g < ng; g++) {
        const uint32_t *src = g + 1 < ng ? list + (g + 1) * kGroup : next;
        uint4 c[NB];
#pragma unroll
        for (int b = 0; b < NB; b++) {
            c[b] = MODE == 1 ? tree8<NP>(pa, buf[b]) : tree8<NP>(pb, buf[b]);
            load_unit<SHIFT>(buf[b], rsrc, src + (uint32_t)b * kUnit, grp, col);
        }
        if (MODE == 1) {
            if constexpr (NB == 4) ripple4<NP, 5>(pa, csa_plane<NP, 4>(pa, csa_plane<NP, 3>(pa, c[0], c[1]), csa_plane<NP, 3>(pa, c[2], c[3])));
            else ripple4<NP, 4>(pa, csa_plane<NP, 3>(pa, c[0], c[1]));
        } else {
            if constexpr (NB == 4) ripple4<NP, 5>(pb, csa_plane<NP, 4>(pb, csa_plane<NP, 3>(pb, c[0], c[1]), csa_plane<NP, 3>(pb, c[2], c[3])));
            else ripple4<NP, 4>(pb, csa_plane<NP, 3>(pb, c[0], c[1]));
        }
    }
}

template <int NP>
__device__ __forceinline__ void reduce_rows(const uint32_t (&pl)[4][NP], uint32_t lane, uint32_t (&out)[NP]) {
    const bool hi = (lane & 32u) != 0u, mid = (lane & 16u) != 0u;
    uint32_t k0[NP], k1[NP];
    {
        uint32_t s0[NP], s1[NP];
#pragma unroll
        for (int p = 0; p < NP; p++) {
            k0[p] = hi ? pl[2][p] : pl[0][p];
            k1[p] = hi ? pl[3][p] : pl[1][p];
            s0[p] = (uint32_t)__shfl_xor((int)(hi ? pl[0][p] : pl[2][p]), 32, 64);
            s1[p] = (uint32_t)__shfl_xor((int)(hi ? pl[1][p] : pl[3][p]), 32, 64);
        }
        planes_add<NP>(k0, s0);
        planes_add<NP>(k1, s1);
    }
    uint32_t s[NP];
#pragma unroll
    for (int p = 0; p < NP; p++) {
        out[p] = mid ? k1[p] : k0[p];
        s[p] = (uint32_t)__shfl_xor((int)(mid ? k0[p] : k1[p]), 16, 64);
    }
    planes_add<NP>(out, s);
}

__device__ __forceinline__ uint32_t umax(uint32_t a, uint32_t b) { return a > b ? a : b; }

template <int NP>
__global__ __launch_bounds__(64, 2) void bounds2_kernel(Bounds2Params p) {
    extern __shared__ uint32_t b2_lds[];
    const uint32_t lane = threadIdx.x;
    const uint32_t np8 = gridDim.x >> 3;
    const uint32_t pair = blockIdx.x < np8 * 8u ? (blockIdx.x & 7u) * np8 + (blockIdx.x >> 3) : blockIdx.x;
    const uint32_t qa = pair * 2u, qb = qa + 1u;
    const bool has_b = qb < p.nq;
    constexpr uint32_t kB2Cap = b2_cap(NP);
    uint32_t *l_both = b2_lds, *l_a = b2_lds + kB2Cap, *l_b = b2_lds + 2u * kB2Cap, *l_zero = b2_lds + 3u * kB2Cap;
    uint16_t *l_keep = reinterpret_cast<uint16_t *>(l_zero + kB2Pad);
    for (uint32_t i = lane; i < kB2Pad; i += 64) l_zero[i] = p.zero_row;

    const uint2 *urec = p.pair_urec + (size_t)pair * p.pair_ustride;
    const uint32_t n_u = std::min<uint32_t>(p.pair_nu[pair], p.pair_ustride);
    const unsigned long long lt_mask = (1ull << lane) - 1ull;
    uint32_t n_both = 0, n_a = 0, n_b = 0;
    for (uint32_t u0 = 0; u0 < n_u; u0 += 512u) {
        uint2 rec[8];
#pragma unroll
        for (int c = 0; c < 8; c++) {
            const uint32_t i = u0 + (uint32_t)c * 64u + lane;
            rec[c] = urec[i < p.pair_ustride ? i : p.pair_ustride - 1u];
        }
#pragma unroll
        for (int c = 0; c < 8; c++) {
            const uint32_t i = u0 + (uint32_t)c * 64u + lane;
            const bool in = i < n_u;
            const bool ia = in && (rec[c].x & (1u << 30)), ib = in && (rec[c].x & (1u << 31)) && has_b;
            const uint32_t row = rec[c].x & 0x3FFFFFFFu;
            const bool sh = ia && ib, oa = ia && !ib, ob = ib && !ia;
            const unsigned long long bs = __ballot(sh), ba = __ballot(oa), bo = __ballot(ob);
            const uint32_t ps = n_both + (uint32_t)__popcll(bs & lt_mask), pa_ = n_a + (uint32_t)__popcll(ba & lt_mask), pb_ = n_b + (uint32_t)__popcll(bo & lt_mask);
            if (sh && ps < kB2Cap) l_both[ps] = row;
            if (oa && pa_ < kB2Cap) l_a[pa_] = row;
            if (ob && pb_ < kB2Cap) l_b[pb_] = row;
            n_both += (uint32_t)__popcll(bs);
            n_a += (uint32_t)__popcll(ba);
            n_b += (uint32_t)__popcll(bo);
        }
    }
    n_both = std::min(n_both, kB2Cap);
    n_a = std::min(n_a, kB2Cap);
    n_b = std::min(n_b, kB2Cap);
    for (uint32_t i = n_both + lane; i < ((n_both + kB2Pad - 1u) & ~(kB2Pad - 1u)); i += 64) l_both[i] = p.zero_row;
    for (uint32_t i = n_a + lane; i < ((n_a + kB2Pad - 1u) & ~(kB2Pad - 1u)); i += 64) l_a[i] = p.zero_row;
    for (uint32_t i = n_b + lane; i < ((n_b + kB2Pad - 1u) & ~(kB2Pad - 1u)); i += 64) l_b[i] = p.zero_row;
    wave_lds_sync();

    const uint32_t t_a = p.t[qa], t_b = has_b ? p.t[qb] : 0u;
    uint16_t *tub_a = p.tile_ub + (size_t)qa * p.tile_ub_stride, *tub_b = p.tile_ub + (size_t)(has_b ? qb : qa) * p.tile_ub_stride;
    uint32_t pa[4][NP], pb[4][NP];
// ... 32 lines not shown
        const char *base = reinterpret_cast<const char *>(p.abitmap) + (size_t)at * p.n_rows1 * 256u;
        const __amdgpu_buffer_rsrc_t rsrc = __builtin_amdgcn_make_buffer_rsrc(const_cast<char *>(base), 0, p.n_rows1 * 256u, 0x00027000);
        fold_level(std::integral_constant<int, 4>{}, std::integral_constant<int, 4>{}, std::integral_constant<int, 8>{}, rsrc, row4, (lane & 15u) * 16u, true, has_b);
        uint32_t ra[NP], rb[NP], cand;
        reduce_rows<NP>(pa, lane, ra);
        reduce_rows<NP>(pb, lane, rb);
        const uint32_t T = at * 64u + (lane & 15u) * 4u + row4;
        const uint32_t ma = planes_max<NP>(ra, cand), mb = planes_max<NP>(rb, cand);
        if (T < p.ntiles) {
            tub_a[T] = (uint16_t)ma;
            if (has_b) tub_b[T] = (uint16_t)mb;
        }
        max_a = umax(max_a, ma);
        max_b = umax(max_b, mb);
        l_keep[at * 128u + lane] = (uint16_t)ma;
        l_keep[at * 128u + 64u + lane] = (uint16_t)mb;
    }
    max_a = wave_max_u32(max_a);
    max_b = wave_max_u32(max_b);
    wave_lds_sync();
    auto delta_of = [&](uint32_t t, uint32_t mx) -> uint32_t {
        const uint32_t up = p.delta_ct * t, dn = p.delta_cm * mx;
        const uint32_t d = up > dn ? (up - dn) >> 8 : 0u, lo = (p.delta_lo * t) >> 8, hi = (p.delta_hi * t) >> 8;
        return d < lo ? lo : (d > hi ? hi : d);
    };
    const uint32_t dl_a = umax(delta_of(t_a, max_a), 1u), dl_b = umax(delta_of(t_b, max_b), 1u);

    const uint32_t sub4 = lane & 3u, grp16 = lane >> 2;
    auto wanted = [&](uint32_t at, uint32_t &mask_a, uint32_t &mask_b) {
        uint32_t ma = l_keep[at * 128u + lane], mb = l_keep[at * 128u + 64u + lane];
        ma = umax(ma, (uint32_t)__shfl_xor((int)ma, 16, 64));
        ma = umax(ma, (uint32_t)__shfl_xor((int)ma, 32, 64));
        mb = umax(mb, (uint32_t)__shfl_xor((int)mb, 16, 64));
        mb = umax(mb, (uint32_t)__shfl_xor((int)mb, 32, 64));
        mask_a = (uint32_t)(__ballot(ma + dl_a > max_a && ma != 0u && lane < 16u) & 0xFFFFull);
        mask_b = has_b ? (uint32_t)(__ballot(mb + dl_b > max_b && mb != 0u && lane < 16u) & 0xFFFFull) : 0u;
    };
    bool heavy_a = false, heavy_b = false;
    if (p.heavy) {
        uint32_t na = 0, nb = 0;
        for (uint32_t at = 0; at < p.n_atiles; at++) {
            uint32_t mask_a, mask_b;
            wanted(at, mask_a, mask_b);
            na += (uint32_t)__popc(mask_a);
            nb += (uint32_t)__popc(mask_b);
        }
        heavy_a = na > p.heavy_max;
        heavy_b = nb > p.heavy_max;
        if (lane == 0u) {
            p.heavy[qa] = heavy_a ? 1u : 0u;
            if (has_b) p.heavy[qb] = heavy_b ? 1u : 0u;
        }
    }
    for (uint32_t at = 0; at < p.n_atiles; at++) {
        uint32_t mask_a, mask_b;
        wanted(at, mask_a, mask_b);
        mask_a = heavy_a ? 0u : mask_a;
        mask_b = heavy_b ? 0u : mask_b;
        uint32_t todo = mask_a | mask_b;
        while (todo) {
            const uint32_t s = (uint32_t)__builtin_ctz(todo);
            todo &= todo - 1u;
            const uint32_t bt = at * 16u + s;
            if (bt * 4u >= p.ntiles) break;
            const bool for_a = (mask_a >> s) & 1u, for_b = (mask_b >> s) & 1u;
            const char *base = reinterpret_cast<const char *>(p.bbitmap) + (size_t)bt * p.n_rows1 * 64u;
            const __amdgpu_buffer_rsrc_t rsrc = __builtin_amdgcn_make_buffer_rsrc(const_cast<char *>(base), 0, p.n_rows1 * 64u, 0x00027000);
            fold_level(std::integral_constant<int, 16>{}, std::integral_constant<int, 2>{}, std::integral_constant<int, 6>{}, rsrc, grp16, sub4 * 16u, for_a, for_b);
            const uint32_t T = bt * 4u + sub4;
            const bool real = T < p.ntiles;
            auto finish = [&](const uint32_t (&pl)[4][NP], uint16_t *tub, uint32_t &best) {
                uint32_t r[NP];
                reduce_rows<NP>(pl, lane, r);
#pragma unroll
                for (int k = 0; k < 2; k++) {
                    uint32_t sh[NP];
#pragma unroll
                    for (int pp = 0; pp < NP; pp++)
                        sh[pp] = k == 0 ? (uint32_t)__builtin_amdgcn_update_dpp(0, (int)r[pp], 0x124, 0xF, 0xF, true)
                                        : (uint32_t)__builtin_amdgcn_update_dpp(0, (int)r[pp], 0x128, 0xF, 0xF, true);
                    planes_add<NP>(r, sh);
                }
                uint32_t c;
                const uint32_t w = planes_max<NP>(r, c);
                uint32_t key = (w << 8) | (127u - (row4 * 32u + (uint32_t)__builtin_ctz(c)));
                key = umax(key, (uint32_t)__shfl_xor((int)key, 16, 64));
                key = umax(key, (uint32_t)__shfl_xor((int)key, 32, 64));
                if (real && lane < 4u) tub[T] = (uint16_t)(key >> 8);
                const uint32_t g = real ? ((key >> 8) << 20) | (0xFFFFFu - (T * 128u + (127u - (key & 0xFFu)))) : 0u;
                best = umax(best, wave_max_u32(g));
            };
            if (for_a) finish(pa, tub_a, best_a);
            if (for_b) finish(pb, tub_b, best_b);
        }
    }
    if (lane == 0u) {
        p.best_key[qa] = heavy_a ? 0u : best_a;
        if (has_b) p.best_key[qb] = heavy_b ? 0u : best_b;
        if (p.group_rows) atomicAdd(&p.group_rows[p.group_base + pair], n_instr);
    }
}

__global__ __launch_bounds__(1024) void heavy_items_kernel(const uint8_t *__restrict__ heavy, uint32_t nq, uint32_t u_ntiles, uint32_t *__restrict__ items,
                                                           uint32_t *__restrict__ n_items) {
    __shared__ uint32_t wsum[2][16];
    const uint32_t tid = threadIdx.x, lane = tid & 63u, wave = tid >> 6, np = (nq + 1u) / 2u;
    constexpr uint32_t kPer = 32;
    uint32_t carry = 0, buf = 0;
    for (uint32_t base = 0; base < np; base += 1024u * kPer, buf ^= 1u) {
        const uint32_t p0 = base + tid * kPer;
        uint32_t bits = 0;
        if (p0 < np) {
            if (p0 + kPer <= np && 2u * (p0 + kPer) <= nq) {
                const uint4 *f = reinterpret_cast<const uint4 *>(heavy + (size_t)p0 * 2u);
                const uint4 v[4] = {f[0], f[1], f[2], f[3]};
#pragma unroll
                for (int k = 0; k < 4; k++) {
                    const uint32_t w[4] = {v[k].x, v[k].y, v[k].z, v[k].w};
#pragma unroll
                    for (int j = 0; j < 4; j++) {
                        if (w[j] & 0x0000FFFFu) bits |= 1u << (k * 8 + j * 2);
                        if (w[j] & 0xFFFF0000u) bits |= 1u << (k * 8 + j * 2 + 1);
                    }
                }
            } else {
                for (uint32_t j = 0; j < kPer && p0 + j < np; j++) {
                    const uint32_t pr = p0 + j;
                    if (heavy[pr * 2u] || (pr * 2u + 1u < nq && heavy[pr * 2u + 1u])) bits |= 1u << j;
                }
            }
        }
        const uint32_t cnt = (uint32_t)__popc(bits);
        const uint32_t incl = wave_incl_scan_u32(cnt);
        if (lane == 63u) wsum[buf][wave] = incl;
        __syncthreads();
        uint32_t o = carry + incl - cnt, tot = 0;
#pragma unroll
        for (uint32_t w = 0; w < 16u; w++) {
            const uint32_t sw = wsum[buf][w];
            o += w < wave ? sw : 0u;
            tot += sw;
        }
        while (bits) {
            const uint32_t j = (uint32_t)__builtin_ctz(bits);
            bits &= bits - 1u;
            for (uint32_t ut = 0; ut < u_ntiles; ut++) items[(size_t)o * u_ntiles + ut] = (p0 + j) * u_ntiles + ut;
            o++;
        }
        carry += tot;
    }
    if (tid == 0u) n_items[0] = carry * u_ntiles;
    if (tid >= 1u && tid <= 8u) n_items[tid] = 0;
// ... 48 lines not shown
```

raxtax_amd/csrc/rtx_index.hpp:

```cpp
#pragma once

#include <hip/hip_runtime.h>

#include <algorithm>
#include <cmath>
#include <cstdlib>
#include <cstring>
#include <thread>

#include "rtx_internal.hpp"
#include "rtx_kernels.hpp"
#include "rtx_math.hpp"

using namespace rtx;

namespace rtxi {


constexpr uint32_t kEmptyRow = 0xFFFFFFFFu;
constexpr uint32_t kLnFactLen = 98320;

#define RTX_HIP(call)                                                                          \
    do {                                                                                       \
        hipError_t e_ = (call);                                                                \
// ... 114 lines not shown
    std::vector<uint32_t> bnd;
    uint32_t n_bnd = 0;
    DevBuf<uint4> d_noderec;
    DevBuf<uint8_t> d_node_depth, d_node_sig0;
    DevBuf<uint32_t> d_node_begin;
    DevBuf<double> d_node_eb;
    uint32_t fin_D = 1;
    DevBuf<uint32_t> d_bnd_rank;
    DevBuf<uint8_t> d_bnd_bits;
    uint32_t dev_exact_opt = 1;
    uint32_t strand_opt = 0;
    bool strand_used = false;
    uint64_t n_user = 0;
    uint32_t em_groups = 0, em_bits = 0;
    uint64_t em_hash_mask = ~0ull;
    DevBuf<uint2> d_em_table;
    DevBuf<uint64_t> d_em_rep_off;
    DevBuf<uint8_t> d_em_rep_bytes;
    DevBuf<uint32_t> d_em_goff, d_em_gids;
    std::vector<uint32_t> h_em_goff, h_em_gids;
    bool dev_exact_used = false;
    struct HostExact {
        std::vector<uint32_t> grp;
        std::vector<uint64_t> off;
        std::vector<uint32_t> ids;
        bool csr_valid = false, valid = false;
    } host_exact[2];
    uint64_t n_q = 0;
    bool uploaded = false, ran = false, synced = false;
    uint32_t last_flags = 0;
    uint32_t cluster = 1;
    uint32_t packed_opt = 1;
    uint32_t tile_skip = 1;
    uint32_t pair_opt = 1;
    uint32_t prune_opt = 1;
    uint32_t self_sample_opt = 1;
    bool prune_pays = true;
    double self_live = -1.0;
    bool pruning() const { return prune_opt != 0u && (prune_pays || self_sample_opt == 0u); }
    bool dbg_full = false;
    bool dbg_full_run = false;
    DevBuf<uint32_t> d_ubitmap;
    uint32_t u_stride_bytes = 0, u_ntiles = 0;
    uint64_t u_nblocks = 0;
    DevBuf<uint32_t> d_fbitmap;
    uint32_t f_stride_bytes = 0, f_ntiles = 0;
    uint64_t f_nblocks = 0;
    uint32_t fine_opt = 1;
    DevBuf<uint32_t> d_abitmap;
    DevBuf<uint8_t> d_bbitmap;
    uint32_t n_atiles = 0, n_btiles = 0;
    DevBuf<uint8_t> d_cbitmap;
    uint32_t two_level_opt = 1;
    uint32_t b2_delta[4] = {283u, 205u, 92u, 128u};
    bool two_level_used = false;
    uint32_t rec_seg_len = 1024;
    uint32_t diet_shift = 3;
    uint32_t rec_opt = 4;
    uint32_t rec_slots() const { return std::min<uint32_t>(rec_opt, kRecMaxSlots); }
    uint32_t overlap_opt = 1;
    uint32_t overlap_used = 0;
    hipStream_t stream2 = nullptr, stream3 = nullptr, hit_stream = nullptr;
    std::vector<hipEvent_t> ev_front, ev_back, ev_mid;
    DevBuf<unsigned long long> d_prune_stats;
    uint32_t shard_prune_opt = 0;
    uint32_t debug_taps = 0;
    DevBuf<uint32_t> d_prune_detail;
    uint32_t locator_opt = 1;
    DevBuf<uint32_t> d_loc_table;
    DevBuf<uint32_t> d_group_rows;
    uint32_t n_groups_run = 0;
    uint32_t groups_per_sub = 0;
    bool packs(int pl) const { return packed_opt && pl <= 10; }
    DevBuf<uint64_t> d_skey_in, d_skey_out;
    DevBuf<uint32_t> d_sidx;
    DevBuf<uint8_t> d_sort_tmp;
    DevBuf<uint8_t> d_bases;
    struct Inputs {
        DevBuf<uint8_t> d_packed;
        DevBuf<uint64_t> d_base_off, d_exact_off;
        DevBuf<uint32_t> d_exact_ids;
        PinBuf<uint8_t> h_packed;
        PinBuf<uint64_t> h_base_off, h_exact_off;
        PinBuf<uint32_t> h_exact_ids;
        uint64_t n_q = 0, total = 0, max_len = 0, n_exact = 0;
        uint64_t n_user = 0;
        uint64_t cls_n[5] = {0, 0, 0, 0, 0}, cls_max[5] = {0, 0, 0, 0, 0};
        bool packed = true, has_exact = false, staged = false, recorded = false;
        DevBuf<char> d_labels;
        DevBuf<uint64_t> d_label_off;
        PinBuf<char> h_labels;
        PinBuf<uint64_t> h_label_off;
        uint64_t n_labels = 0;
        bool labels_pending = false, has_labels = false;
        hipEvent_t ready = nullptr;
    } in[2];
    uint32_t cur_in = 0;
    hipStream_t h2d_stream = nullptr;
    hipEvent_t ev_activated = nullptr;
    uint64_t sum_query_bytes = 0;
    uint32_t sub_batch_req = 0;
    uint32_t min_subs = 4;
    uint64_t ws_key[14] = {0};
    bool ws_valid = false;
    struct BatchClass {
        uint64_t pos0 = 0, n = 0, max_len = 0;
        uint32_t tmax = 0, kstride = 0, rstride = 0, hstride = 0, sub_batch = 0, sb0 = 0, n_sub = 0;
        int planes = 10;
        bool use_tables = false, pair = false, prune = false, rec = false, huge = false, will_prune = false;
        bool side = false;
        bool diet = false;
        uint32_t cnt_rows = 0;
    } cls[5];
    uint32_t n_cls = 0;
    uint64_t key_lim[4] = {~0ull, ~0ull, ~0ull, ~0ull};
    struct SubPlan { uint64_t q0; uint32_t nq, cls; };
    std::vector<SubPlan> plan;
    uint32_t n_sub_total() const { return (uint32_t)plan.size(); }
    uint32_t sub_batch_max = 0;
    bool any_prune = false;
    DevBuf<double> d_prob_scratch;
    struct Scratch {
        DevBuf<uint16_t> d_kmers, d_counts, d_tilemax;
        DevBuf<uint32_t> d_rows, d_t, d_nrows, d_hist, d_order, d_srows, d_nsparse;
        DevBuf<unsigned long long> d_dmask;
        DevBuf<double> d_table_z, d_prefix;
        DevBuf<uint2> d_urec;
        DevBuf<uint32_t> d_nu;
        DevBuf<uint32_t> d_live, d_best_key;
        DevBuf<uint32_t> d_items;
        DevBuf<uint16_t> d_tile_ub, d_prune_thr, d_prune_i1;
        DevBuf<uint32_t> d_best;
        DevBuf<uint8_t> d_heavy;
        DevBuf<uint32_t> d_heavy_items;
        DevBuf<uint32_t> d_fine_items;
        DevBuf<uint16_t> d_rec_nslots, d_rec_slots;
        DevBuf<uint32_t> d_rec_cnt, d_rec;
        DevBuf<uint32_t> d_cnt_row, d_cnt_cursor;
        template <class S, class F>
        static void each(S &s, F &&f) {
            f(s.d_kmers); f(s.d_counts); f(s.d_tilemax); f(s.d_rows); f(s.d_t); f(s.d_nrows); f(s.d_hist); f(s.d_order); f(s.d_srows); f(s.d_nsparse);
            f(s.d_dmask); f(s.d_table_z); f(s.d_prefix); f(s.d_urec); f(s.d_nu); f(s.d_live); f(s.d_best_key); f(s.d_items); f(s.d_tile_ub); f(s.d_prune_thr);
            f(s.d_prune_i1); f(s.d_best); f(s.d_heavy); f(s.d_heavy_items); f(s.d_fine_items); f(s.d_rec_nslots); f(s.d_rec_slots); f(s.d_rec_cnt); f(s.d_rec);
            f(s.d_cnt_row); f(s.d_cnt_cursor);
        }
        void release_all() { each(*this, [](auto &b) { b.release(); }); }
        uint64_t bytes() const {
            uint64_t b = 0;
            each(*this, [&](const auto &buf) { b += buf.bytes(); });
            return b - d_cnt_row.bytes() - d_cnt_cursor.bytes();
        }
    } sc[4];
    bool staged = false;
    uint32_t last_set = 0;
    const BatchClass &last_cls() const { return cls[staged ? 0u : plan.back().cls]; }
    DevBuf<double> d_probs_dbg;
    DevBuf<uint16_t> d_counts_dbg;
    DevBuf<unsigned long long> d_sub_alloc;
    struct ResultSet {
        DevBuf<uint8_t> d_status;
        DevBuf<uint32_t> d_t_all, d_nrows_all, d_n_rows, d_flags, d_ndist;
        DevBuf<double> d_gs, d_z;
        DevBuf<unsigned long long> d_hq, d_row_start, d_cursor;
        DevBuf<DevRow> d_arena;
        uint64_t arena_cap = 0;
        uint64_t side_base = 0;
        PinBuf<unsigned long long> h_side_base;
        DevBuf<uint32_t> d_fin_t, d_fin_row_count, d_fin_lineage, d_fin_node, d_fin_depth;
        DevBuf<uint8_t> d_fin_status, d_fin_depth8, d_fin_hund;
        DevBuf<double> d_fin_gs, d_fin_local, d_fin_conf;
        DevBuf<unsigned long long> d_fin_row_begin, d_fin_cursor;
        uint64_t fin_cap = 0;
        DevBuf<uint32_t> d_perm, d_iperm;
        DevBuf<uint32_t> d_exact_grp;
        DevBuf<uint32_t> d_peak2, d_peak, d_sel_t, d_sel_row_count;
        DevBuf<uint8_t> d_strand, d_sel_status;
        DevBuf<double> d_sel_gs;
        DevBuf<unsigned long long> d_sel_row_begin;
        hipEvent_t ev_select = nullptr;
        uint64_t n_user = 0;
        bool has_peak = false;
        hipEvent_t ev_exact = nullptr;
        PinBuf<uint32_t> h_flags;
        hipEvent_t ev_flags = nullptr;
        std::vector<hipEvent_t> ev_sub;
        PinBuf<unsigned long long> h_cursor_sub, h_fin_sub;
        uint64_t n_q = 0;
        uint32_t n_sub = 0, n_side = 0;
        uint32_t in_set = 0;
        bool dev_exact = false;
        bool stream_dl = false;
        struct Bytes { uint64_t order, groups, rest; };
        Bytes bytes() const {
            return {(d_perm.n + d_iperm.n) * 4, d_exact_grp.n * 4,
                    d_status.n + (d_t_all.n + d_nrows_all.n + d_n_rows.n + d_ndist.n) * 4 + (d_gs.n + d_z.n + d_hq.n + d_row_start.n) * 8 + d_arena.n * sizeof(DevRow) +
                        (d_fin_t.n + d_fin_row_count.n + d_fin_lineage.n + d_fin_node.n + d_fin_depth.n) * 4 + d_fin_status.n + d_fin_depth8.n + d_fin_hund.n +
                        (d_fin_gs.n + d_fin_local.n + d_fin_conf.n + d_fin_row_begin.n) * 8};
        }
        void destroy_events() {
// ... 87 lines not shown
uint16_t *counts_hi(rtx_index *ix, const rtx_index::BatchClass &k, rtx_index::Scratch &sc);
uint32_t counts_rows_layout(const rtx_index *ix, const rtx_index::BatchClass &k);
uint32_t diet_rows(const rtx_index *ix, uint32_t B);
int ensure_full_counts(rtx_index *ix, const rtx_index::BatchClass &k, rtx_index::Scratch &sc);
hipEvent_t stage_event(rtx_index *ix, const SubBatch &b, int stage, int which);
int enqueue_kmer(rtx_index *ix, const SubBatch &b, hipStream_t s);
int enqueue_hit(rtx_index *ix, const SubBatch &b, uint32_t flags, hipStream_t s, int part = 0, hipStream_t s_mid = nullptr);
int enqueue_count(rtx_index *ix, const SubBatch &b, uint32_t flags, hipStream_t s_mid = nullptr);
int enqueue_prob_prefix(rtx_index *ix, const SubBatch &b, bool fuse_walk, bool prob_only = false);
int enqueue_walk(rtx_index *ix, const SubBatch &b, const double *prefix, hipStream_t s);
int order_batch(rtx_index *ix, bool cluster);
void record_batch(rtx_index *ix);
int begin_run(rtx_index *ix, uint32_t *n_sub_out, bool *timed_out, bool cluster);
int enqueue_batch(rtx_index *ix, uint32_t flags);
int ensure_prob_tables(rtx_index *ix, uint32_t tmax, bool *usable);
uint32_t length_class(uint64_t len);
uint64_t class3_max_len();
int prepare_workspace(rtx_index *ix, uint64_t n_queries, const uint64_t cls_n[5], const uint64_t cls_max[5]);
int prepare_workspace_single(rtx_index *ix, uint64_t n_queries, uint64_t tmax, uint64_t max_len);
int plan_sub_batches(rtx_index *ix);
int alloc_scratch_set(rtx_index *ix, uint32_t k);
constexpr uint32_t kSideSet = 3;
int node_tables(rtx_index *ix);
int alloc_result_set(rtx_index *ix, rtx_index::ResultSet &r, uint64_t n_queries, uint64_t min_arena = 0);
int settle_join(rtx_index *ix);
int alloc_final(rtx_index *ix, rtx_index::ResultSet &r, uint64_t n_queries);
int enqueue_finalise(rtx_index *ix, const SubBatch &b, hipStream_t s);
int enqueue_text(rtx_index *ix, const rtx_index::ResultSet &r);


struct ItemList {
    size_t np, ntiles;
    ItemList(size_t nq, size_t tiles) : np((nq + 1u) / 2u), ntiles(tiles) {}
    size_t cap() const { return np * ntiles; }
    size_t end() const { return cap() + 9u; }
    uint32_t *items(uint32_t *p) const { return p; }
    uint32_t *count(uint32_t *p) const { return p + cap(); }
};
struct ItemsLayout : ItemList {
    using ItemList::ItemList;
    size_t total() const { return end() + 2u * np; }
    uint32_t *pair_live(uint32_t *p) const { return p + end(); }
    uint32_t *offsets(uint32_t *p) const { return p + end() + np; }
};
struct FineItemsLayout : ItemList {
    using ItemList::ItemList;
    size_t total() const { return end() + ntiles; }
    uint32_t *cursors(uint32_t *p) const { return p + end(); }
};
struct HeavyItemsLayout : ItemList {
    using ItemList::ItemList;
    size_t total() const { return end(); }
};
struct LiveLayout {
    uint32_t ntiles;
    uint32_t words() const { return (ntiles + 31u) / 32u + 1u; }
    size_t total(size_t B) const { return (B + 1u) * words(); }
};

inline size_t counts_elems(const rtx_index *ix, int planes, size_t rows) { return ix->packs(planes) ? rows * ix->npad * 5 / 8 : rows * ix->npad; }

struct ScratchNeed {
    size_t kmers = 0, rows = 0, dmask = 0, counts = 0, hist = 0 , prefix = 0, urec = 0;
    size_t prob_scratch = 0;
    size_t nsparse = 0, srows = 0, t = 0, nrows = 0, order = 0, tilemax = 0, nu = 0;
    size_t tile_ub = 0, best_key = 0, prune_thr = 0, prune_i1 = 0, best = 0, live = 0, items = 0;
    size_t heavy = 0, heavy_items = 0, fine_items = 0;
    size_t rec_nslots = 0, rec_slots = 0, rec_cnt = 0, rec = 0, cnt_row = 0, cnt_cursor = 0;
    ScratchNeed &set_queries(const rtx_index *ix, size_t B) {
        const size_t nt = ix->ntiles;
        t = nrows = order = best_key = prune_thr = prune_i1 = rec_nslots = cnt_row = B;
        nsparse = tilemax = tile_ub = B * nt;
        srows = B * nt * (kSegMaxSparseRows + 1);
        nu = (B + 1u) / 2u;
        best = B * kPruneBestWords;
        live = LiveLayout{ix->ntiles}.total(B);
        items = ItemsLayout(B, nt).total();
        heavy = B + 1u;
        heavy_items = HeavyItemsLayout(B, ix->u_ntiles).total();
        fine_items = FineItemsLayout(B, ix->f_ntiles).total();
        rec_slots = rec_cnt = B * kRecMaxSlots;
        rec = B * ix->rec_slots() * ix->rec_seg_len;
        cnt_cursor = 4;
        return *this;
    }
    void add_class(const rtx_index *ix, const rtx_index::BatchClass &kc, size_t B, size_t cnt_rows) {
        auto up = [](size_t &a, size_t v) { a = std::max(a, v); };
        up(kmers, B * kc.kstride);
        up(rows, B * kc.rstride);
        up(dmask, B * ix->ntiles * (kc.rstride / 64));
        up(counts, counts_elems(ix, kc.planes, cnt_rows));
        up(prefix, cnt_rows * ix->n_bnd_local);
        up(hist, B * kc.hstride);
        up(urec, ((B + 1u) / 2u) * 2u * kc.rstride);
        if (kc.huge) up(prob_scratch, B * ((prob_table_lds_bytes(kc.tmax) + 7) / 8));
    }
};

inline ScratchNeed scratch_set_need(const rtx_index *ix, uint32_t k) {
    ScratchNeed n;
    size_t b_max = 1;
    for (uint32_t c = 0; c < ix->n_cls; c++) {
        const rtx_index::BatchClass &kc = ix->cls[c];
        if (kc.side != (k == kSideSet)) continue;
        const size_t B = kc.sub_batch;
        b_max = std::max(b_max, B);
        const bool diet = kc.will_prune && ix->rec_opt != 0u && ix->n_refs == ix->n_total && ix->n_bnd_local == ix->n_bnd;
        n.add_class(ix, kc, B, diet ? diet_rows(ix, (uint32_t)B) : B);
    }
    return n.set_queries(ix, b_max);
}

inline uint64_t class_per_q(const rtx_index *ix, const rtx_index::BatchClass &k) {
    return (uint64_t)k.kstride * 2 + (uint64_t)k.rstride * 12 + 4 + (uint64_t)ix->ntiles * (k.rstride / 8 + ((kSegMaxSparseRows + 1) * 4 + 10)) + (ix->packs(k.planes) ? ix->npad * 5 / 4 : ix->npad * 2) +
           (uint64_t)k.hstride * 12 + (uint64_t)ix->n_bnd_local * 8 + 64 + (k.huge ? prob_table_lds_bytes(k.tmax) : 0) +
           (k.will_prune ? (uint64_t)ix->ntiles * 2 + 12 + (ix->ntiles + 31u) / 32u * 2u + 2u + kPruneBestWords * 4 +
                               ((uint64_t)ix->ntiles + 2u) * 2u   +
                               (ix->d_fbitmap.p ? (uint64_t)ix->f_ntiles * 2u + 1u : 0u)  +
                               (ix->rec_opt && ix->n_refs == ix->n_total ? (uint64_t)std::min<uint32_t>(ix->rec_opt, kRecMaxSlots) * 32768u + kRecMaxSlots * 6u + 2u : 0u)
                           : 0);
}

}
```

raxtax_amd/csrc/rtx_kernels.hpp:

```cpp
#pragma once

#include <hip/hip_runtime.h>

#include <cstdint>

#include "raxtax_hip.h"

namespace rtx {

#ifndef RTX_NODE_TYPES_DEFINED
#define RTX_NODE_TYPES_DEFINED
enum NodeType : uint8_t { kInner = 0, kTaxon = 1, kSequence = 2 };
#endif

constexpr uint32_t kWalkMaxRows = 208;
constexpr uint32_t kSegSlotEntries = 16, kSegSparseMax = 16, kSegMaxSparseRows = 255;
constexpr uint32_t kSegPad = 8192;
__host__ __device__ inline uint32_t seg_pad(uint32_t i) { return kSegPad + ((i & 63u) << 2); }
constexpr uint32_t kKmerFewLive = 8;
constexpr uint32_t kHitListCap = 1024;

struct DevRow {
    uint32_t node;
    uint8_t k[RTX_MAX_DEPTH];
// ... 127 lines not shown
    const uint32_t *srows;
    const uint32_t *nsparse;
    const uint16_t *segslots;
    uint32_t ntiles;
    const uint32_t *t;
    uint16_t *counts;
    uint8_t *counts_lo;
    uint16_t *counts_hi;
    uint64_t npad;
    uint32_t *hist;
    uint32_t hstride;
    uint16_t *tile_max;
    uint32_t flags;
    uint64_t q0;
    const uint32_t *perm;
    ExactRef exact;
    uint32_t nq;
    uint32_t *group_rows;
    uint32_t group_base;
    const uint2 *pair_urec;
    const uint32_t *pair_nu;
    uint32_t pair_ustride;
    const uint32_t *live;
    uint32_t live_words;
    const uint16_t *prune_thr;
    const uint32_t *items;
    uint32_t *n_items;
    uint16_t *bounds_tile_ub;
    uint32_t bounds_tile_stride, bounds_ntiles;
    uint32_t *bounds_best;
    const uint8_t *bounds_heavy;
    uint64_t fine_n_refs;
    uint32_t fine_ref_ntiles;
    unsigned long long *fine_stats;
    RecordRef rec;
    const uint32_t *cnt_row;
};
struct Bounds2Params {
    const uint32_t *abitmap;
    const uint8_t *bbitmap;
    uint32_t n_rows1, n_atiles, ntiles, zero_row;
    const uint2 *pair_urec;
    const uint32_t *pair_nu;
    uint32_t pair_ustride, nq;
    const uint32_t *t;
    uint16_t *tile_ub;
    uint32_t tile_ub_stride;
    uint32_t *best_key;
    uint32_t delta_ct, delta_cm, delta_lo, delta_hi;
    uint8_t *heavy;
    uint32_t heavy_max;
    uint32_t *group_rows;
    uint32_t group_base;
};
struct HitParams;
void launch_bounds2(hipStream_t s, const Bounds2Params &p, uint32_t nq, int planes, const HitParams &hp, uint32_t u_ntiles, uint32_t *items);
constexpr uint32_t kTwoLevelMinTiles = 16;
void launch_bounds2_build(hipStream_t s, const uint32_t *ubitmap, uint32_t n_rows1, uint32_t u_ntiles, uint8_t *bbitmap, uint32_t *abitmap);
constexpr uint32_t kFineShift = 3;
constexpr uint32_t kFineMinLive = 4;
constexpr uint32_t kFineMinTiles = 16;

constexpr uint32_t kPruneStatCopies = 64;
#ifndef RTX_PRUNE_SHIFT
#define RTX_PRUNE_SHIFT 6
#endif
constexpr uint32_t kPruneShift = RTX_PRUNE_SHIFT;
static_assert(kPruneShift >= 3 && kPruneShift <= 6, "blocks of 8 .. 64 references");
constexpr uint32_t kPruneBestWords = 66;
struct PruneParams {
    const uint16_t *tile_ub;
    const uint32_t *best_key;
    uint32_t tile_ub_stride, ntiles, nq;
    uint64_t n_refs;
    uint64_t n_total;
    uint32_t ref_base;
    uint32_t phase;
    uint32_t *best;
    const uint2 *cbitmap;
    const uint32_t *bitmap;
    uint32_t n_rows1, stride_bytes;
    const uint32_t *rows;
    uint32_t rstride;
    const uint32_t *nrows, *t;
    uint32_t flags;
    uint64_t q0;
    const uint32_t *perm;
    ExactRef exact;
    const double *lnfact, *inv;
    uint32_t nlf;
    uint32_t *hist;
    uint32_t hstride;
    uint32_t *live;
    uint32_t live_words;
    uint32_t *pair_live;
    uint16_t *thr_out;
    uint16_t *i1_out;
    unsigned long long *stats;
    uint32_t *detail;
    RecordRef rec;
    uint32_t rec_max_slots;
    uint32_t *cnt_row;
    uint32_t *cnt_cursor;
    uint32_t cnt_cap;
    uint32_t *flags_out;
};
constexpr uint32_t kPruneDetailWords = 72;
struct ProbTables;
void launch_prune(hipStream_t s, const PruneParams &p, const ProbTables &tb, uint32_t nq);
// ... 96 lines not shown
    const uint8_t *bnd_bits;
    const uint32_t *bnd_rank;
    double *prefix;
    uint32_t n_bnd;
    const uint16_t *tile_max;
    uint32_t ntiles;
    const uint16_t *prune_thr;
    unsigned long long *prune_stats;
    uint32_t fuse_walk;
    WalkParams walk;
    const uint16_t *rec_nslots;
    const uint32_t *cnt_row;
};


struct TailParams {
    RecordRef rec;
    const uint32_t *t;
    const double *table_z;
    uint32_t hstride;
    const uint8_t *bnd_bits;
    const uint32_t *bnd_rank;
    double *prefix;
    uint32_t *cnt_cursor;
    uint32_t cnt_cap;
    uint32_t *flags_out;
    uint32_t n_bnd;
    uint32_t nq;
    WalkParams walk;
    unsigned long long *prefix_stats;
    unsigned long long *stats;
};
void launch_records_tail(hipStream_t s, const TailParams &p, uint32_t nq);

void launch_bitmap_build(hipStream_t s, const uint64_t *off, const uint32_t *post, const uint32_t *row_of,
                         uint32_t *bitmap, uint32_t stride_words, uint32_t n_rows1, uint32_t ref_lo, uint32_t ref_hi, uint32_t shift = 0);
void launch_ref_kmer_mark(hipStream_t s, const uint8_t *bases, const uint64_t *off, uint64_t n_refs, uint32_t *present);
void launch_ref_bitmap_set(hipStream_t s, const uint8_t *bases, const uint64_t *off, uint64_t n_refs,
                           const uint32_t *row_of, uint32_t *bitmap, uint32_t stride_words, uint32_t n_rows1, uint32_t shift = 0);
void launch_row_len_pack(hipStream_t s, const uint32_t *row_of, const uint32_t *list_len, uint2 *out);
void launch_row_popcount(hipStream_t s, const uint32_t *row_of, const uint32_t *bitmap, uint32_t stride_words, uint32_t n_rows1,
                         uint32_t *list_len);
void launch_kmer_extract(hipStream_t s, const KmerParams &p, uint32_t nq);
void launch_hit_count(hipStream_t s, const HitParams &p, uint32_t nq, uint32_t ntiles, int planes);
void launch_pair_union(hipStream_t s, const uint32_t *rows, const uint32_t *nrows, uint32_t rstride, uint32_t nq, uint2 *urec,
                       uint32_t *nu, uint32_t ustride);
void launch_hit_count_pair(hipStream_t s, const HitParams &p, uint32_t nq, uint32_t ntiles, int planes);
void launch_live_items(hipStream_t s, const uint32_t *live, uint32_t live_words, const uint32_t *pair_live, uint32_t nq, uint32_t ntiles, uint32_t *off,
                       uint32_t *items, uint32_t *n_items);
void launch_hit_count_pair_bounds(hipStream_t s, const HitParams &p, uint32_t nq, uint32_t u_ntiles, int planes);
void launch_hit_count_pair_bounds_items(hipStream_t s, const HitParams &p, uint32_t nq, uint32_t u_ntiles, int planes);
void launch_fine_bounds(hipStream_t s, const HitParams &p, uint32_t nq, uint32_t ntiles, uint32_t f_ntiles, uint32_t *pair_live, uint32_t *cnt,
                        uint32_t *items, uint32_t *n_items, int planes);
size_t prob_table_lds_bytes(uint32_t tmax);
void launch_prob_table(hipStream_t s, const ProbParams &p, uint32_t nq);
size_t prob_lookup_lds_bytes(uint32_t tmax);
void launch_prob_tables_build(hipStream_t s, const ProbTables &tb, const double *lf, const double *inv);
void launch_prob_order(hipStream_t s, const uint32_t *t, uint32_t nq, uint32_t *order);
void launch_prob_lookup(hipStream_t s, const ProbParams &p, const ProbTables &tb, uint32_t nq);
void launch_seg_popcount(hipStream_t s, const uint32_t *bitmap, uint32_t stride_bytes, uint32_t n_rows1, uint32_t ntiles, uint16_t *pop);
void launch_seg_emit(hipStream_t s, const uint32_t *bitmap, uint32_t stride_bytes, uint32_t n_rows1, uint32_t ntiles,
                     const uint32_t *seginfo, uint32_t seg_stride, uint16_t *slots);
void launch_sketch(hipStream_t s, const uint8_t *bases, const uint64_t *off, uint32_t n_q, uint64_t *keys, uint32_t *idx);
void launch_invert_perm(hipStream_t s, const uint32_t *perm, uint32_t n, uint32_t *inv);
constexpr uint32_t kLocTableEntries = 1u << 24;
void launch_loc_mark(hipStream_t s, const uint8_t *bases, const uint64_t *off, uint64_t n_refs, uint32_t *pos_min, uint32_t *cnt);
void launch_loc_finish(hipStream_t s, uint32_t *pos_min, const uint32_t *cnt);
void launch_locator(hipStream_t s, const uint8_t *bases, const uint64_t *off, uint32_t n_q, const uint32_t *table, uint64_t n_refs,
                    uint64_t *keys);
void launch_identity_perm(hipStream_t s, uint32_t n, uint32_t *perm, uint32_t *inv);
int cluster_sort(hipStream_t s, void *tmp, size_t *tmp_bytes, const uint64_t *keys_in, uint64_t *keys_out, const uint32_t *idx_in,
                 uint32_t *perm_out, size_t n, bool with_class = false);
void launch_class_keys(hipStream_t s, uint64_t *keys, const uint64_t *off, uint32_t n, const uint64_t lim[4], bool from_index, uint32_t *idx);
void launch_taxon_prefix(hipStream_t s, const PrefixParams &p, uint32_t nq);
void launch_lineage_walk(hipStream_t s, const WalkParams &p, uint32_t nq);
void launch_finalise(hipStream_t s, const FinaliseParams &p);
void launch_probs_expand(hipStream_t s, const uint16_t *counts, const double *tz, uint64_t n, double *out);
void launch_rehist(hipStream_t s, const uint16_t *counts, uint64_t npad, uint64_t n_refs, const uint32_t *t, uint32_t *hist,
                   uint32_t hstride, uint16_t *tile_max, uint32_t ntiles, uint32_t nq);
void launch_counts_unpack(hipStream_t s, const uint8_t *lo, const uint16_t *hi, uint64_t n, uint16_t *out);

}
```

Before: 13.03 million.

## Add sub-tile hit counting path driven by kept two-level bounds

```diff
diff --git a/include/raxtax_hip.h b/include/raxtax_hip.h
--- a/include/raxtax_hip.h
+++ b/include/raxtax_hip.h
@@ -124,6 +124,7 @@
 #define RTX_OPT_RUN_AHEAD 23
 #define RTX_OPT_DEVICE_TEXT 24
 #define RTX_OPT_STRAND 25
+#define RTX_OPT_SUBTILE_COUNT 26
 int rtx_index_set_option(rtx_index *index, int option, uint64_t value);
 
 int rtx_index_self_sample(rtx_index *index, const uint8_t *seq_bytes, const uint64_t *seq_off, uint64_t n_refs, uint32_t n_sample, double *live_fraction);
@@ -131,6 +132,7 @@
 int rtx_index_run_ahead_stats(const rtx_index *index, uint64_t *enqueued_ahead, uint64_t *abandoned);
 #define RTX_DEFAULT_SEGMENT_CLASSES 1
 #define RTX_DEFAULT_EXACT_HASH_MASK 2
+#define RTX_DEFAULT_REC_SEG_LEN 3
 int rtx_set_default_option(int option, uint64_t value);
 
 typedef struct {
@@ -228,6 +230,8 @@
 int rtx_batch_last_sub_batch(const rtx_index *index, uint64_t *first, uint32_t *n);
 int rtx_batch_classes(const rtx_index *index, uint32_t *n_classes, uint64_t out[20]);
 int rtx_debug_prune_stats(rtx_index *index, uint64_t *out );
+int rtx_debug_subtile_stats(rtx_index *index, uint64_t *out );
+int rtx_debug_rec_seg_len(const rtx_index *index, uint32_t *seg_len);
 int rtx_debug_pruned_prob_table(rtx_index *index, uint64_t query, double *table_over_z , double *z, uint32_t *threshold);
 int rtx_debug_run_counts(rtx_index *index, uint64_t query, uint16_t *counts , uint8_t *tile_live ,
                          uint32_t *hist , uint32_t *threshold, uint32_t *i1);
diff --git a/raxtax_amd/_build.py b/raxtax_amd/_build.py
--- a/raxtax_amd/_build.py
+++ b/raxtax_amd/_build.py
@@ -9,8 +9,8 @@
 ROOT = PKG.parent
 CSRC = PKG / "csrc"
 LIB = PKG / "libraxtax_hip.so"
-SOURCES = ["rtx_kernels.hip", "rtx_hit_pair.hip", "rtx_prob_tables.hip", "rtx_cluster.hip", "rtx_segments.hip", "rtx_prune.hip", "rtx_bounds2.hip", "rtx_records.hip", "rtx_finalise.hip", "rtx_text.hip", "rtx_exact.hip", "rtx_strand.hip", "rtx_ingest.hip", "rtx_api_index.hip", "rtx_api_batch.hip", "rtx_api_download.hip", "rtx_api_shard.hip", "rtx_api_debug.hip", "host_tree.cpp", "host_format.cpp", "host_raxtax.cpp", "host_bin.cpp", "host_threads.cpp"]
-HEADERS = ["rtx_index.hpp", "rtx_kernels.hpp", "rtx_hit_common.hpp", "rtx_internal.hpp", "rtx_math.hpp", "rtx_wave.hpp", "rtx_walk.hpp", "host_raxtax.hpp"]
+SOURCES = ["rtx_kernels.hip", "rtx_hit_pair.hip", "rtx_prob_tables.hip", "rtx_cluster.hip", "rtx_segments.hip", "rtx_prune.hip", "rtx_bounds2.hip", "rtx_subtile.hip", "rtx_records.hip", "rtx_finalise.hip", "rtx_text.hip", "rtx_exact.hip", "rtx_strand.hip", "rtx_ingest.hip", "rtx_api_index.hip", "rtx_api_batch.hip", "rtx_api_download.hip", "rtx_api_shard.hip", "rtx_api_debug.hip", "host_tree.cpp", "host_format.cpp", "host_raxtax.cpp", "host_bin.cpp", "host_threads.cpp"]
+HEADERS = ["rtx_index.hpp", "rtx_kernels.hpp", "rtx_hit_common.hpp", "rtx_bounds2.hpp", "rtx_internal.hpp", "rtx_math.hpp", "rtx_wave.hpp", "rtx_walk.hpp", "host_raxtax.hpp"]
 CLI = PKG / "raxtax-hip"
 SYNTH = PKG / "raxtax-synth"
 
diff --git a/raxtax_amd/_lib.py b/raxtax_amd/_lib.py
--- a/raxtax_amd/_lib.py
+++ b/raxtax_amd/_lib.py
@@ -132,6 +132,8 @@
     "rtx_debug_order": (C.c_int, [C.c_void_p, u32p]),
     "rtx_debug_tile_bounds": (C.c_int, [C.c_void_p, C.c_uint64, u16p]),
     "rtx_debug_prune_stats": (C.c_int, [C.c_void_p, u64p]),
+    "rtx_debug_subtile_stats": (C.c_int, [C.c_void_p, u64p]),
+    "rtx_debug_rec_seg_len": (C.c_int, [C.c_void_p, u32p]),
     "rtx_debug_run_counts": (C.c_int, [C.c_void_p, C.c_uint64, u16p, u8p, u32p, u32p, u32p]),
     "rtx_debug_run_mode": (C.c_int, [C.c_void_p, C.c_uint64, u32p]),
     "rtx_batch_last_sub_batch": (C.c_int, [C.c_void_p, u64p, u32p]),
diff --git a/raxtax_amd/api.py b/raxtax_amd/api.py
--- a/raxtax_amd/api.py
+++ b/raxtax_amd/api.py
@@ -201,7 +201,8 @@
                  tile_skip: Optional[bool] = None, hit_pair=None, locator: Optional[bool] = None, tile_prune: Optional[bool] = None,
                  debug_taps: bool = False, device_exact: Optional[bool] = None, fine_bounds: Optional[bool] = None,
                  records: Optional[int] = None, overlap: Optional[bool] = None, two_level: Optional[int] = None,
-                 prune_self_sample: Optional[bool] = None, device_text: bool = False, strand: str = "plus"):
+                 prune_self_sample: Optional[bool] = None, device_text: bool = False, strand: str = "plus",
+                 subtile_count: Optional[bool] = None):
         self._lib = _lib.load()
         self.tree = tree
         if segment_classes is None:
@@ -247,6 +248,8 @@
             check(self._lib.rtx_index_set_option(self._h, 21, int(two_level)))
         if prune_self_sample is not None:
             check(self._lib.rtx_index_set_option(self._h, 22, int(prune_self_sample)))
+        if subtile_count is not None:
+            check(self._lib.rtx_index_set_option(self._h, 26, int(subtile_count)))
         if strand not in ("plus", "both"):
             raise ValueError(f"strand must be 'plus' or 'both', not {strand!r}")
         self.strand = strand
@@ -474,6 +477,16 @@
         check(self._lib.rtx_debug_order(self._h, ptr(out, u32p)))
         return out
 
+    def debug_subtile_stats(self) -> dict:
+        out = np.zeros(8, np.uint64)
+        check(self._lib.rtx_debug_subtile_stats(self._h, ptr(out, u64p)))
+        return dict(sub_items=int(out[0]), tile_items=int(out[1]), subtiles=int(out[2]), fallback_no_bounds=int(out[3]), fallback_too_many=int(out[4]))
+
+    def debug_rec_seg_len(self) -> int:
+        out = np.zeros(1, np.uint32)
+        check(self._lib.rtx_debug_rec_seg_len(self._h, ptr(out, u32p)))
+        return int(out[0])
+
     def debug_prune_stats(self) -> dict:
         out = np.zeros(16, dtype=np.uint64)
         check(self._lib.rtx_debug_prune_stats(self._h, ptr(out, u64p)))
diff --git a/raxtax_amd/csrc/rtx_api_batch.hip b/raxtax_amd/csrc/rtx_api_batch.hip
--- a/raxtax_amd/csrc/rtx_api_batch.hip
+++ b/raxtax_amd/csrc/rtx_api_batch.hip
@@ -1,8 +1,5 @@
 #include "rtx_index.hpp"
 
-#ifndef RTX_B2_HEAVY_PER_ATILE
-#define RTX_B2_HEAVY_PER_ATILE 4u
-#endif
 
 namespace rtxi {
 
@@ -185,6 +182,10 @@
     return up;
 }
 
+static bool subtile_on(const rtx_index *ix, const rtx_index::Scratch &sc, uint32_t nq) {
+    return ix->subtile_opt != 0u && ix->rec_opt != 0u && ix->d_sbitmap.p != nullptr && nq <= sc.subtile_B;
+}
+
 static Bounds2Params bounds2_params(const rtx_index *ix, const rtx_index::Scratch &sc, const HitParams &up, bool heavy) {
     Bounds2Params bp{};
     bp.abitmap = ix->d_abitmap.p;
@@ -208,7 +209,13 @@
     bp.group_rows = up.group_rows;
     bp.group_base = up.group_base;
     bp.heavy = heavy ? sc.d_heavy.p : nullptr;
-    bp.heavy_max = std::max<uint32_t>(1u, std::min<uint32_t>(RTX_B2_HEAVY_PER_ATILE * ix->n_atiles, ix->n_btiles / 2u));
+    bp.heavy_max = ix->heavy_max();
+    if (heavy && subtile_on(ix, sc, up.nq)) {
+        bp.keep_planes = sc.d_keep_planes.p;
+        bp.keep_bt = sc.d_keep_bt.p;
+        bp.keep_n = sc.d_keep_n.p;
+        bp.keep_cap = ix->keep_cap();
+    }
     return bp;
 }
 
@@ -281,6 +288,8 @@
     ix->last_set = b.set;
     HitParams hp = hit_params(ix, b, flags);
     const bool prune = run_prunes(ix, k);
+    bool subtile = false, kept_bounds = false;
+    SubtileParams sp{};
     if (k.pair && part != 2) {
         if (b.timed_all) RTX_HIP(hipEventRecord(stage_event(ix, b, RTX_STAGE_PAIR_UNION, 0), s));
         launch_pair_union(s, sc.d_rows.p, sc.d_nrows.p, k.rstride, b.nq, sc.d_urec.p, sc.d_nu.p, 2u * k.rstride);
@@ -295,7 +304,9 @@
             ix->two_level_used = part == 0 && ix->two_level_opt && ix->d_abitmap.p && ix->d_bbitmap.p && ix->n_refs == ix->n_total && k.planes <= kBounds2MaxPlanes;
             if (ix->two_level_used) {
                 const bool heavy_ok = sc.d_heavy.p && sc.d_heavy_items.p && sc.d_heavy_items.n >= HeavyItemsLayout(b.nq, ix->u_ntiles).total();
-                launch_bounds2(s, bounds2_params(ix, sc, up, heavy_ok), b.nq, k.planes, up, ix->u_ntiles, heavy_ok ? sc.d_heavy_items.p : nullptr);
+                const Bounds2Params bp = bounds2_params(ix, sc, up, heavy_ok);
+                kept_bounds = bp.keep_planes != nullptr && k.planes <= (int)kKeepPlanes;
+                launch_bounds2(s, bp, b.nq, k.planes, up, ix->u_ntiles, heavy_ok ? sc.d_heavy_items.p : nullptr);
             } else {
                 RTX_HIP(hipMemsetAsync(sc.d_best_key.p, 0, (size_t)b.nq * 4, s));
                 launch_hit_count_pair_bounds(s, up, b.nq, ix->u_ntiles, k.planes);
@@ -338,11 +349,39 @@
             launch_live_items(s, sc.d_live.p, pr.live_words, pr.pair_live, b.nq, ix->ntiles, items.offsets(sc.d_items.p), items.items(sc.d_items.p), items.count(sc.d_items.p));
             hp.items = items.items(sc.d_items.p);
             hp.n_items = items.count(sc.d_items.p);
+            subtile = records && kept_bounds && subtile_on(ix, sc, b.nq);
+            if (subtile) {
+                const SubItemsLayout sub(b.nq, ix->ntiles);
+                const HeavyItemsLayout rest(b.nq, ix->ntiles);
+                sp.sbitmap = ix->d_sbitmap.p;
+                sp.n_rows1 = ix->n_rows + 1;
+                sp.zero_row = ix->n_rows;
+                sp.keep_planes = sc.d_keep_planes.p;
+                sp.keep_bt = sc.d_keep_bt.p;
+                sp.keep_n = sc.d_keep_n.p;
+                sp.keep_cap = ix->keep_cap();
+                sp.keep_np = k.planes <= 8 ? 8u : 10u;
+                sp.items = hp.items;
+                sp.n_items = hp.n_items;
+                sp.tile_items = rest.items(sc.d_tile_items.p);
+                sp.tile_count = rest.count(sc.d_tile_items.p);
+                sp.sub_items = sub.items(sc.d_sub_items.p);
+                sp.sub_count = sub.count(sc.d_sub_items.p);
+                sp.live_lists = sc.d_live_lists.p;
+                sp.codes = sub.codes(sc.d_sub_items.p);
+                sp.parts = sub.parts(sc.d_sub_items.p);
+                sp.n_parts = 4u * std::max<uint32_t>(1u, std::min<uint32_t>(kSubtileMaxParts / 4u, (b.nq + 255u) / 256u));
+                sp.stats = ix->d_prune_stats.p ? ix->d_prune_stats.p + 4 * kPruneStatCopies * 8 : nullptr;
+                RTX_HIP(hipMemcpyAsync(sc.d_live_lists.p, sc.d_live.p, (size_t)b.nq * pr.live_words * 4, hipMemcpyDeviceToDevice, s));
+                launch_subtile_split(s, sp, hp);
+                hp.items = sp.tile_items;
+                hp.n_items = sp.tile_count;
+            }
         }
         if (ix->seg_blocks) {
             KmerParams kp = kmer_params(ix, b);
             kp.mode = 2u;
-            kp.live = sc.d_live.p;
+            kp.live = subtile ? sc.d_live_lists.p : sc.d_live.p;
             kp.live_words = pr.live_words;
             launch_kmer_extract(s, kp, b.nq);
         }
@@ -351,6 +390,7 @@
             RTX_HIP(hipEventRecord(stage_event(ix, b, RTX_STAGE_HIT_COUNT, 0), s));
         }
     }
+    if (subtile) launch_subtile_count(s, sp, hp, k.planes);
     if (k.pair) launch_hit_count_pair(s, hp, b.nq, ix->ntiles, k.planes);
     else launch_hit_count(s, hp, b.nq, ix->ntiles, k.planes);
     if (b.timed) RTX_HIP(hipEventRecord(stage_event(ix, b, RTX_STAGE_HIT_COUNT, 1), s));
@@ -703,10 +743,10 @@
     ix->groups_per_sub = (b_max + 1u) / 2u;
     ix->dbg_full = false;
     if (any_prune) {
-        int rc_s = ix->d_prune_stats.alloc(kPruneStatCopies * 32);
+        int rc_s = ix->d_prune_stats.alloc(kPruneStatCopies * 40);
         if (!rc_s && ix->debug_taps) rc_s = ix->d_prune_detail.alloc((size_t)b_max * kPruneDetailWords);
         if (rc_s) return rc_s;
-        RTX_HIP(hipMemsetAsync(ix->d_prune_stats.p, 0, kPruneStatCopies * 256, ix->stream));
+        RTX_HIP(hipMemsetAsync(ix->d_prune_stats.p, 0, kPruneStatCopies * 320, ix->stream));
     }
     if (any_pair) {
         ix->n_groups_run = n_sub * ix->groups_per_sub;
@@ -1084,6 +1124,14 @@
             return rc;
         if (ix->d_abitmap.p && (sc.d_heavy.alloc(n.heavy) || sc.d_heavy_items.alloc(n.heavy_items))) { sc.d_heavy.release(); sc.d_heavy_items.release(); }
         if (ix->d_fbitmap.p && sc.d_fine_items.alloc(n.fine_items)) sc.d_fine_items.release();
+        if (!(ix->d_sbitmap.p && ix->subtile_opt && ix->rec_opt && ix->n_refs == ix->n_total && sc.d_heavy.p) ||
+            sc.d_keep_planes.alloc(n.keep_planes) || sc.d_keep_bt.alloc(n.keep_bt) || sc.d_keep_n.alloc(n.keep_n) || sc.d_sub_items.alloc(n.sub_items) ||
+            sc.d_tile_items.alloc(n.tile_items) || sc.d_live_lists.alloc(n.live_lists)) {
+            sc.d_keep_planes.release(); sc.d_keep_bt.release(); sc.d_keep_n.release(); sc.d_sub_items.release(); sc.d_tile_items.release(); sc.d_live_lists.release();
+            sc.subtile_B = 0;
+        } else {
+            sc.subtile_B = (uint32_t)(n.keep_n - 1u);
+        }
         if (ix->rec_opt && ix->n_refs == ix->n_total) {
             if (sc.d_rec_nslots.alloc(n.rec_nslots) || sc.d_rec_slots.alloc(n.rec_slots) || sc.d_rec_cnt.alloc(n.rec_cnt) ||
                 sc.d_rec.alloc(n.rec) || sc.d_cnt_row.alloc(n.cnt_row) || sc.d_cnt_cursor.alloc(n.cnt_cursor))
diff --git a/raxtax_amd/csrc/rtx_api_debug.hip b/raxtax_amd/csrc/rtx_api_debug.hip
--- a/raxtax_amd/csrc/rtx_api_debug.hip
+++ b/raxtax_amd/csrc/rtx_api_debug.hip
@@ -340,6 +340,24 @@
         out[14] += h[(3 * kPruneStatCopies + c) * 8 + 1];
         out[15] += h[(3 * kPruneStatCopies + c) * 8 + 3];
     }
+    return RTX_OK;
+}
+
+int rtx_debug_subtile_stats(rtx_index *ix, uint64_t *out) {
+    if (!ix || !out) { set_error("null argument"); return RTX_ERR_INVALID; }
+    std::memset(out, 0, 8 * sizeof(uint64_t));
+    if (!ix->any_prune || !ix->d_prune_stats.p || ix->d_prune_stats.n < (size_t)kPruneStatCopies * 40) return RTX_OK;
+    RTX_HIP(hipStreamSynchronize(ix->stream));
+    unsigned long long h[kPruneStatCopies * 8];
+    RTX_HIP(hipMemcpy(h, ix->d_prune_stats.p + 4 * kPruneStatCopies * 8, sizeof(h), hipMemcpyDeviceToHost));
+    for (uint32_t c = 0; c < kPruneStatCopies; c++)
+        for (uint32_t k = 0; k < kSubtileStats; k++) out[k] += h[c * 8 + k];
+    return RTX_OK;
+}
+
+int rtx_debug_rec_seg_len(const rtx_index *ix, uint32_t *seg_len) {
+    if (!ix || !seg_len) { set_error("null argument"); return RTX_ERR_INVALID; }
+    *seg_len = ix->rec_seg_len;
     return RTX_OK;
 }
 
diff --git a/raxtax_amd/csrc/rtx_api_index.hip b/raxtax_amd/csrc/rtx_api_index.hip
--- a/raxtax_amd/csrc/rtx_api_index.hip
+++ b/raxtax_amd/csrc/rtx_api_index.hip
@@ -51,6 +51,7 @@
 }
 
 
+static uint32_t g_rec_seg_len = 1024;
 static int create_common(int device, uint64_t n_total, uint64_t ref_lo, uint64_t ref_hi, const uint64_t *cuts,
                          uint32_t n_cuts, uint32_t n_nodes, const uint32_t *node_begin, const uint32_t *node_end,
                          const uint32_t *node_first_child, const uint32_t *node_n_children, const uint8_t *node_type,
@@ -74,6 +75,7 @@
         return RTX_ERR_NO_DEVICE;
     }
     auto ix = new rtx_index();
+    ix->rec_seg_len = g_rec_seg_len;
     ix->device = device;
     ix->n_refs = n_refs;
     ix->n_total = n_total;
@@ -470,7 +472,20 @@
         e = hipGetLastError();
         if (e == hipSuccess) e = hipStreamSynchronize(ix->stream);
     }
-    if (e != hipSuccess) { (void)hipGetLastError(); ix->d_cbitmap.release(); }
+    if (e != hipSuccess) { (void)hipGetLastError(); ix->d_cbitmap.release(); return; }
+    const size_t sbytes = (size_t)ix->ntiles * kSubPerTile * rows1 * kSubRowBytes;
+    if (rows1 * kSubRowBytes > 0xFFFFFFFFull || hipMemGetInfo(&free_b, &total_b) != hipSuccess || sbytes > free_b / 4 || sbytes > total_b / 16 || ix->d_sbitmap.alloc(sbytes)) {
+        (void)hipGetLastError();
+        ix->d_sbitmap.release();
+        return;
+    }
+    e = hipMemsetAsync(ix->d_sbitmap.p, 0, sbytes, ix->stream);
+    if (e == hipSuccess) {
+        launch_subtile_build(ix->stream, ix->d_bitmap.p, (uint32_t)rows1, ix->ntiles, ix->stride_bytes, ix->d_sbitmap.p);
+        e = hipGetLastError();
+        if (e == hipSuccess) e = hipStreamSynchronize(ix->stream);
+    }
+    if (e != hipSuccess) { (void)hipGetLastError(); ix->d_sbitmap.release(); }
 }
 
 static void build_locator(rtx_index *ix, const uint8_t *d_seq, const uint64_t *d_off, uint64_t n_refs) {
@@ -654,7 +669,7 @@
 uint64_t rtx_index_num_refs(const rtx_index *index) { return index ? index->n_total : 0; }
 uint64_t rtx_index_device_bytes(const rtx_index *index) {
     if (!index) return 0;
-    return index->d_seg_dbits.n * 8 + index->d_seg_sbits.n * 8 + index->d_seg_sbase.n * 4 + index->d_seginfo.n * 4 + index->d_segcls.n * 4 + index->d_segslots.n * 2 + index->d_bitmap.n * 4 + index->d_row_of.n * 4 + index->d_row_len.n * 8 + index->d_list_len.n * 4 + index->d_loc_table.n * 4 + index->d_ubitmap.n * 4 + index->d_fbitmap.n * 4 + index->d_abitmap.n * 4 + index->d_bbitmap.n + index->d_cbitmap.n + index->d_em_table.n * 8 + index->d_em_rep_off.n * 8 + index->d_em_rep_bytes.n + index->d_em_goff.n * 4 + index->d_em_gids.n * 4 + index->d_lnfact.n * 8 +
+    return index->d_seg_dbits.n * 8 + index->d_seg_sbits.n * 8 + index->d_seg_sbase.n * 4 + index->d_seginfo.n * 4 + index->d_segcls.n * 4 + index->d_segslots.n * 2 + index->d_bitmap.n * 4 + index->d_row_of.n * 4 + index->d_row_len.n * 8 + index->d_list_len.n * 4 + index->d_loc_table.n * 4 + index->d_ubitmap.n * 4 + index->d_fbitmap.n * 4 + index->d_abitmap.n * 4 + index->d_bbitmap.n + index->d_cbitmap.n + index->d_sbitmap.n + index->d_em_table.n * 8 + index->d_em_rep_off.n * 8 + index->d_em_rep_bytes.n + index->d_em_goff.n * 4 + index->d_em_gids.n * 4 + index->d_lnfact.n * 8 +
            index->d_noderec.n * 16 + index->d_bnd_bits.n + index->d_bnd_rank.n * 4;
 }
 uint64_t rtx_index_workspace_bytes(const rtx_index *ix) {
@@ -704,6 +719,11 @@
 int rtx_set_default_option(int option, uint64_t value) {
     if (option == RTX_DEFAULT_SEGMENT_CLASSES) { g_seg_classes = value ? 1 : 0; return RTX_OK; }
     if (option == RTX_DEFAULT_EXACT_HASH_MASK) { g_em_hash_mask = value ? value : ~0ull; return RTX_OK; }
+    if (option == RTX_DEFAULT_REC_SEG_LEN) {
+        if (value != 0 && (value < 16 || value > 8192 || (value & (value - 1)) != 0)) { set_error("RTX_DEFAULT_REC_SEG_LEN: a power of two in 16 .. 8192 (0: the default)"); return RTX_ERR_INVALID; }
+        g_rec_seg_len = value ? (uint32_t)value : 1024u;
+        return RTX_OK;
+    }
     set_error("rtx_set_default_option: unknown option %d", option);
     return RTX_ERR_INVALID;
 }
@@ -785,6 +805,12 @@
                 index->b2_delta[3] = (uint32_t)((value >> 48) & 0xFFFFu);
             }
             return RTX_OK;
+        case RTX_OPT_SUBTILE_COUNT:
+            if (value > 1) break;
+            index->uploaded = index->ran = index->synced = false;
+            index->ws_valid = false;
+            index->subtile_opt = (uint32_t)value;
+            return RTX_OK;
         case RTX_OPT_MIN_SUB_BATCHES:
             if (value < 1 || value > 64) break;
             index->uploaded = index->ran = index->synced = false;
diff --git a/raxtax_amd/csrc/rtx_bounds2.hip b/raxtax_amd/csrc/rtx_bounds2.hip
--- a/raxtax_amd/csrc/rtx_bounds2.hip
+++ b/raxtax_amd/csrc/rtx_bounds2.hip
@@ -3,73 +3,10 @@
 #include <algorithm>
 #include <type_traits>
 
+#include "rtx_bounds2.hpp"
 #include "rtx_hit_common.hpp"
 
 namespace rtx {
-
-constexpr uint32_t kB2Pad = 256u;
-constexpr uint32_t b2_cap(int planes) { return planes > 10 ? 2048u : 1024u; }
-constexpr uint32_t b2_lds_dw(int planes) { return 3u * b2_cap(planes) + kB2Pad; }
-
-template <int SHIFT>
-__device__ __forceinline__ void load_unit(uint4 (&buf)[8], __amdgpu_buffer_rsrc_t rsrc, const uint32_t *unit, uint32_t grp, uint32_t col) {
-    const uint4 i0 = reinterpret_cast<const uint4 *>(unit)[grp * 2u], i1 = reinterpret_cast<const uint4 *>(unit)[grp * 2u + 1u];
-    const uint32_t id[8] = {i0.x, i0.y, i0.z, i0.w, i1.x, i1.y, i1.z, i1.w};
-#pragma unroll
-    for (int j = 0; j < 8; j++) {
-        const u32x4_t v = __builtin_amdgcn_raw_buffer_load_b128(rsrc, (id[j] << SHIFT) + col, 0, 0);
-        buf[j] = make_uint4(v.x, v.y, v.z, v.w);
-    }
-}
-
-template <int NP, int MODE, int R, int NB, int SHIFT>
-__device__ __forceinline__ void fold_list(uint32_t (&pa)[4][NP], uint32_t (&pb)[4][NP], uint4 (&buf)[4][8], const uint32_t *list, uint32_t ng,
-                                          const uint32_t *next, uint32_t grp, uint32_t col, __amdgpu_buffer_rsrc_t rsrc) {
-    constexpr uint32_t kUnit = 8u * (uint32_t)R, kGroup = kUnit * (uint32_t)NB;
-    for (uint32_t g = 0; g < ng; g++) {
-        const uint32_t *src = g + 1 < ng ? list + (g + 1) * kGroup : next;
-        uint4 c[NB];
-#pragma unroll
-        for (int b = 0; b < NB; b++) {
-            c[b] = MODE == 1 ? tree8<NP>(pa, buf[b]) : tree8<NP>(pb, buf[b]);
-            load_unit<SHIFT>(buf[b], rsrc, src + (uint32_t)b * kUnit, grp, col);
-        }
-        if (MODE == 1) {
-            if constexpr (NB == 4) ripple4<NP, 5>(pa, csa_plane<NP, 4>(pa, csa_plane<NP, 3>(pa, c[0], c[1]), csa_plane<NP, 3>(pa, c[2], c[3])));
-            else ripple4<NP, 4>(pa, csa_plane<NP, 3>(pa, c[0], c[1]));
-        } else {
-            if constexpr (NB == 4) ripple4<NP, 5>(pb, csa_plane<NP, 4>(pb, csa_plane<NP, 3>(pb, c[0], c[1]), csa_plane<NP, 3>(pb, c[2], c[3])));
-            else ripple4<NP, 4>(pb, csa_plane<NP, 3>(pb, c[0], c[1]));
-        }
-    }
-}
-
-template <int NP>
-__device__ __forceinline__ void reduce_rows(const uint32_t (&pl)[4][NP], uint32_t lane, uint32_t (&out)[NP]) {
-    const bool hi = (lane & 32u) != 0u, mid = (lane & 16u) != 0u;
-    uint32_t k0[NP], k1[NP];
-    {
-        uint32_t s0[NP], s1[NP];
-#pragma unroll
-        for (int p = 0; p < NP; p++) {
-            k0[p] = hi ? pl[2][p] : pl[0][p];
-            k1[p] = hi ? pl[3][p] : pl[1][p];
-            s0[p] = (uint32_t)__shfl_xor((int)(hi ? pl[0][p] : pl[2][p]), 32, 64);
-            s1[p] = (uint32_t)__shfl_xor((int)(hi ? pl[1][p] : pl[3][p]), 32, 64);
-        }
-        planes_add<NP>(k0, s0);
-        planes_add<NP>(k1, s1);
-    }
-    uint32_t s[NP];
-#pragma unroll
-    for (int p = 0; p < NP; p++) {
-        out[p] = mid ? k1[p] : k0[p];
-        s[p] = (uint32_t)__shfl_xor((int)(mid ? k0[p] : k1[p]), 16, 64);
-    }
-    planes_add<NP>(out, s);
-}
-
-__device__ __forceinline__ uint32_t umax(uint32_t a, uint32_t b) { return a > b ? a : b; }
 
 template <int NP>
 __global__ __launch_bounds__(64, 2) void bounds2_kernel(Bounds2Params p) {
@@ -208,6 +145,7 @@
             if (has_b) p.heavy[qb] = heavy_b ? 1u : 0u;
         }
     }
+    uint32_t kept_a = 0, kept_b = 0;
     for (uint32_t at = 0; at < p.n_atiles; at++) {
         uint32_t mask_a, mask_b;
         wanted(at, mask_a, mask_b);
@@ -225,7 +163,7 @@
             fold_level(std::integral_constant<int, 16>{}, std::integral_constant<int, 2>{}, std::integral_constant<int, 6>{}, rsrc, grp16, sub4 * 16u, for_a, for_b);
             const uint32_t T = bt * 4u + sub4;
             const bool real = T < p.ntiles;
-            auto finish = [&](const uint32_t (&pl)[4][NP], uint16_t *tub, uint32_t &best) {
+            auto finish = [&](const uint32_t (&pl)[4][NP], uint16_t *tub, uint32_t &best, uint32_t q, uint32_t &kept) {
                 uint32_t r[NP];
                 reduce_rows<NP>(pl, lane, r);
 #pragma unroll
@@ -236,6 +174,19 @@
                         sh[pp] = k == 0 ? (uint32_t)__builtin_amdgcn_update_dpp(0, (int)r[pp], 0x124, 0xF, 0xF, true)
                                         : (uint32_t)__builtin_amdgcn_update_dpp(0, (int)r[pp], 0x128, 0xF, 0xF, true);
                     planes_add<NP>(r, sh);
+                }
+                if constexpr (NP <= (int)kKeepPlanes) {
+                    if (p.keep_planes) {
+                        if (kept < p.keep_cap) {
+                            if ((lane & 12u) == 0u) {
+                                uint32_t *dst = p.keep_planes + ((size_t)q * p.keep_cap + kept) * ((uint32_t)NP * 16u) + sub4 * 4u + row4;
+#pragma unroll
+                                for (int pp = 0; pp < NP; pp++) dst[pp * 16] = r[pp];
+                            }
+                            if (lane == 0u) p.keep_bt[(size_t)q * p.keep_cap + kept] = (uint16_t)bt;
+                        }
+                        kept++;
+                    }
                 }
                 uint32_t c;
                 const uint32_t w = planes_max<NP>(r, c);
@@ -246,14 +197,18 @@
                 const uint32_t g = real ? ((key >> 8) << 20) | (0xFFFFFu - (T * 128u + (127u - (key & 0xFFu)))) : 0u;
                 best = umax(best, wave_max_u32(g));
             };
-            if (for_a) finish(pa, tub_a, best_a);
-            if (for_b) finish(pb, tub_b, best_b);
+            if (for_a) finish(pa, tub_a, best_a, qa, kept_a);
+            if (for_b) finish(pb, tub_b, best_b, qb, kept_b);
         }
     }
     if (lane == 0u) {
         p.best_key[qa] = heavy_a ? 0u : best_a;
         if (has_b) p.best_key[qb] = heavy_b ? 0u : best_b;
         if (p.group_rows) atomicAdd(&p.group_rows[p.group_base + pair], n_instr);
+        if (p.keep_n) {
+            p.keep_n[qa] = (uint8_t)(heavy_a || kept_a > p.keep_cap || NP > (int)kKeepPlanes ? kKeepNone : kept_a);
+            if (has_b) p.keep_n[qb] = (uint8_t)(heavy_b || kept_b > p.keep_cap || NP > (int)kKeepPlanes ? kKeepNone : kept_b);
+        }
     }
 }
 
diff --git a/raxtax_amd/csrc/rtx_bounds2.hpp b/raxtax_amd/csrc/rtx_bounds2.hpp
--- /dev/null
+++ b/raxtax_amd/csrc/rtx_bounds2.hpp
@@ -0,0 +1,73 @@
+#pragma once
+
+#include <hip/hip_runtime.h>
+
+#include "rtx_hit_common.hpp"
+
+namespace rtx {
+
+constexpr uint32_t kB2Pad = 256u;
+constexpr uint32_t b2_cap(int planes) { return planes > 10 ? 2048u : 1024u; }
+constexpr uint32_t b2_lds_dw(int planes) { return 3u * b2_cap(planes) + kB2Pad; }
+
+template <int SHIFT>
+__device__ __forceinline__ void load_unit(uint4 (&buf)[8], __amdgpu_buffer_rsrc_t rsrc, const uint32_t *unit, uint32_t grp, uint32_t col) {
+    const uint4 i0 = reinterpret_cast<const uint4 *>(unit)[grp * 2u], i1 = reinterpret_cast<const uint4 *>(unit)[grp * 2u + 1u];
+    const uint32_t id[8] = {i0.x, i0.y, i0.z, i0.w, i1.x, i1.y, i1.z, i1.w};
+#pragma unroll
+    for (int j = 0; j < 8; j++) {
+        const u32x4_t v = __builtin_amdgcn_raw_buffer_load_b128(rsrc, (id[j] << SHIFT) + col, 0, 0);
+        buf[j] = make_uint4(v.x, v.y, v.z, v.w);
+    }
+}
+
+template <int NP, int MODE, int R, int NB, int SHIFT>
+__device__ __forceinline__ void fold_list(uint32_t (&pa)[4][NP], uint32_t (&pb)[4][NP], uint4 (&buf)[4][8], const uint32_t *list, uint32_t ng,
+                                          const uint32_t *next, uint32_t grp, uint32_t col, __amdgpu_buffer_rsrc_t rsrc) {
+    constexpr uint32_t kUnit = 8u * (uint32_t)R, kGroup = kUnit * (uint32_t)NB;
+    for (uint32_t g = 0; g < ng; g++) {
+        const uint32_t *src = g + 1 < ng ? list + (g + 1) * kGroup : next;
+        uint4 c[NB];
+#pragma unroll
+        for (int b = 0; b < NB; b++) {
+            c[b] = MODE == 1 ? tree8<NP>(pa, buf[b]) : tree8<NP>(pb, buf[b]);
+            load_unit<SHIFT>(buf[b], rsrc, src + (uint32_t)b * kUnit, grp, col);
+        }
+        if (MODE == 1) {
+            if constexpr (NB == 4) ripple4<NP, 5>(pa, csa_plane<NP, 4>(pa, csa_plane<NP, 3>(pa, c[0], c[1]), csa_plane<NP, 3>(pa, c[2], c[3])));
+            else ripple4<NP, 4>(pa, csa_plane<NP, 3>(pa, c[0], c[1]));
+        } else {
+            if constexpr (NB == 4) ripple4<NP, 5>(pb, csa_plane<NP, 4>(pb, csa_plane<NP, 3>(pb, c[0], c[1]), csa_plane<NP, 3>(pb, c[2], c[3])));
+            else ripple4<NP, 4>(pb, csa_plane<NP, 3>(pb, c[0], c[1]));
+        }
+    }
+}
+
+template <int NP>
+__device__ __forceinline__ void reduce_rows(const uint32_t (&pl)[4][NP], uint32_t lane, uint32_t (&out)[NP]) {
+    const bool hi = (lane & 32u) != 0u, mid = (lane & 16u) != 0u;
+    uint32_t k0[NP], k1[NP];
+    {
+        uint32_t s0[NP], s1[NP];
+#pragma unroll
+        for (int p = 0; p < NP; p++) {
+            k0[p] = hi ? pl[2][p] : pl[0][p];
+            k1[p] = hi ? pl[3][p] : pl[1][p];
+            s0[p] = (uint32_t)__shfl_xor((int)(hi ? pl[0][p] : pl[2][p]), 32, 64);
+            s1[p] = (uint32_t)__shfl_xor((int)(hi ? pl[1][p] : pl[3][p]), 32, 64);
+        }
+        planes_add<NP>(k0, s0);
+        planes_add<NP>(k1, s1);
+    }
+    uint32_t s[NP];
+#pragma unroll
+    for (int p = 0; p < NP; p++) {
+        out[p] = mid ? k1[p] : k0[p];
+        s[p] = (uint32_t)__shfl_xor((int)(mid ? k0[p] : k1[p]), 16, 64);
+    }
+    planes_add<NP>(out, s);
+}
+
+__device__ __forceinline__ uint32_t umax(uint32_t a, uint32_t b) { return a > b ? a : b; }
+
+}
diff --git a/raxtax_amd/csrc/rtx_index.hpp b/raxtax_amd/csrc/rtx_index.hpp
--- a/raxtax_amd/csrc/rtx_index.hpp
+++ b/raxtax_amd/csrc/rtx_index.hpp
@@ -190,6 +190,10 @@
     uint32_t n_atiles = 0, n_btiles = 0;
     DevBuf<uint8_t> d_cbitmap;
     uint32_t two_level_opt = 1;
+    DevBuf<uint8_t> d_sbitmap;
+    uint32_t subtile_opt = 1;
+    uint32_t heavy_max() const { return std::max<uint32_t>(1u, std::min<uint32_t>(RTX_B2_HEAVY_PER_ATILE * n_atiles, n_btiles / 2u)); }
+    uint32_t keep_cap() const { return std::min<uint32_t>(heavy_max(), 254u); }
     uint32_t b2_delta[4] = {283u, 205u, 92u, 128u};
     bool two_level_used = false;
     uint32_t rec_seg_len = 1024;
@@ -275,14 +279,21 @@
         DevBuf<uint16_t> d_rec_nslots, d_rec_slots;
         DevBuf<uint32_t> d_rec_cnt, d_rec;
         DevBuf<uint32_t> d_cnt_row, d_cnt_cursor;
+        DevBuf<uint32_t> d_keep_planes;
+        DevBuf<uint16_t> d_keep_bt;
+        DevBuf<uint8_t> d_keep_n;
+        DevBuf<uint2> d_sub_items;
+        DevBuf<uint32_t> d_tile_items;
+        DevBuf<uint32_t> d_live_lists;
         template <class S, class F>
         static void each(S &s, F &&f) {
             f(s.d_kmers); f(s.d_counts); f(s.d_tilemax); f(s.d_rows); f(s.d_t); f(s.d_nrows); f(s.d_hist); f(s.d_order); f(s.d_srows); f(s.d_nsparse);
             f(s.d_dmask); f(s.d_table_z); f(s.d_prefix); f(s.d_urec); f(s.d_nu); f(s.d_live); f(s.d_best_key); f(s.d_items); f(s.d_tile_ub); f(s.d_prune_thr);
             f(s.d_prune_i1); f(s.d_best); f(s.d_heavy); f(s.d_heavy_items); f(s.d_fine_items); f(s.d_rec_nslots); f(s.d_rec_slots); f(s.d_rec_cnt); f(s.d_rec);
-            f(s.d_cnt_row); f(s.d_cnt_cursor);
-        }
-        void release_all() { each(*this, [](auto &b) { b.release(); }); }
+            f(s.d_cnt_row); f(s.d_cnt_cursor); f(s.d_keep_planes); f(s.d_keep_bt); f(s.d_keep_n); f(s.d_sub_items); f(s.d_tile_items); f(s.d_live_lists);
+        }
+        uint32_t subtile_B = 0;
+        void release_all() { each(*this, [](auto &b) { b.release(); }); subtile_B = 0; }
         uint64_t bytes() const {
             uint64_t b = 0;
             each(*this, [&](const auto &buf) { b += buf.bytes(); });
@@ -476,6 +487,14 @@
     using ItemList::ItemList;
     size_t total() const { return end(); }
 };
+struct SubItemsLayout : ItemList {
+    using ItemList::ItemList;
+    size_t total() const { return cap() + 5u + (cap() + 1u) / 2u + kSubtileMaxParts; }
+    uint2 *items(uint2 *p) const { return p; }
+    uint32_t *count(uint2 *p) const { return reinterpret_cast<uint32_t *>(p + cap()); }
+    uint32_t *codes(uint2 *p) const { return reinterpret_cast<uint32_t *>(p + cap() + 5u); }
+    uint32_t *parts(uint2 *p) const { return reinterpret_cast<uint32_t *>(p + cap() + 5u + (cap() + 1u) / 2u); }
+};
 struct LiveLayout {
     uint32_t ntiles;
     uint32_t words() const { return (ntiles + 31u) / 32u + 1u; }
@@ -491,6 +510,7 @@
     size_t tile_ub = 0, best_key = 0, prune_thr = 0, prune_i1 = 0, best = 0, live = 0, items = 0;
     size_t heavy = 0, heavy_items = 0, fine_items = 0;
     size_t rec_nslots = 0, rec_slots = 0, rec_cnt = 0, rec = 0, cnt_row = 0, cnt_cursor = 0;
+    size_t keep_planes = 0, keep_bt = 0, keep_n = 0, sub_items = 0, tile_items = 0, live_lists = 0;
     ScratchNeed &set_queries(const rtx_index *ix, size_t B) {
         const size_t nt = ix->ntiles;
         t = nrows = order = best_key = prune_thr = prune_i1 = rec_nslots = cnt_row = B;
@@ -506,6 +526,12 @@
         rec_slots = rec_cnt = B * kRecMaxSlots;
         rec = B * ix->rec_slots() * ix->rec_seg_len;
         cnt_cursor = 4;
+        keep_bt = B * ix->keep_cap();
+        keep_planes = keep_bt * kKeepPlanes * 16u;
+        keep_n = B + 1u;
+        sub_items = SubItemsLayout(B, nt).total();
+        tile_items = HeavyItemsLayout(B, nt).total();
+        live_lists = live;
         return *this;
     }
     void add_class(const rtx_index *ix, const rtx_index::BatchClass &kc, size_t B, size_t cnt_rows) {
diff --git a/raxtax_amd/csrc/rtx_kernels.hpp b/raxtax_amd/csrc/rtx_kernels.hpp
--- a/raxtax_amd/csrc/rtx_kernels.hpp
+++ b/raxtax_amd/csrc/rtx_kernels.hpp
@@ -203,9 +203,18 @@
     uint32_t heavy_max;
     uint32_t *group_rows;
     uint32_t group_base;
-};
+    uint32_t *keep_planes;
+    uint16_t *keep_bt;
+    uint8_t *keep_n;
+    uint32_t keep_cap;
+};
+constexpr uint32_t kKeepNone = 0xFFu;
+constexpr uint32_t kKeepPlanes = 10;
 struct HitParams;
 void launch_bounds2(hipStream_t s, const Bounds2Params &p, uint32_t nq, int planes, const HitParams &hp, uint32_t u_ntiles, uint32_t *items);
+#ifndef RTX_B2_HEAVY_PER_ATILE
+#define RTX_B2_HEAVY_PER_ATILE 4u
+#endif
 constexpr uint32_t kTwoLevelMinTiles = 16;
 void launch_bounds2_build(hipStream_t s, const uint32_t *ubitmap, uint32_t n_rows1, uint32_t u_ntiles, uint8_t *bbitmap, uint32_t *abitmap);
 constexpr uint32_t kFineShift = 3;
@@ -408,6 +417,37 @@
 void launch_hit_count_pair_bounds_items(hipStream_t s, const HitParams &p, uint32_t nq, uint32_t u_ntiles, int planes);
 void launch_fine_bounds(hipStream_t s, const HitParams &p, uint32_t nq, uint32_t ntiles, uint32_t f_ntiles, uint32_t *pair_live, uint32_t *cnt,
                         uint32_t *items, uint32_t *n_items, int planes);
+
+#ifndef RTX_SUBTILE_MAX
+#define RTX_SUBTILE_MAX 6
+#endif
+constexpr uint32_t kSubtileMax = RTX_SUBTILE_MAX;
+constexpr uint32_t kSubRefs = 1024, kSubRowBytes = kSubRefs / 8u, kSubPerTile = 8192u / kSubRefs;
+constexpr int kSubRows = 8;
+constexpr uint32_t kSubtileMaxParts = 4096;
+constexpr uint32_t kSubtileStats = 5;
+struct SubtileParams {
+    const uint8_t *sbitmap;
+    uint32_t n_rows1, zero_row;
+    const uint32_t *keep_planes;
+    const uint16_t *keep_bt;
+    const uint8_t *keep_n;
+    uint32_t keep_cap, keep_np;
+    const uint32_t *items;
+    const uint32_t *n_items;
+    uint32_t *tile_items;
+    uint32_t *tile_count;
+    uint2 *sub_items;
+    uint32_t *sub_count;
+    uint32_t *live_lists;
+    uint32_t *codes;
+    uint32_t *parts;
+    uint32_t n_parts;
+    unsigned long long *stats;
+};
+void launch_subtile_split(hipStream_t s, const SubtileParams &sp, const HitParams &hp);
+void launch_subtile_count(hipStream_t s, const SubtileParams &sp, const HitParams &hp, int planes);
+void launch_subtile_build(hipStream_t s, const uint32_t *bitmap, uint32_t n_rows1, uint32_t ntiles, uint32_t stride_bytes, uint8_t *sbitmap);
 size_t prob_table_lds_bytes(uint32_t tmax);
 void launch_prob_table(hipStream_t s, const ProbParams &p, uint32_t nq);
 size_t prob_lookup_lds_bytes(uint32_t tmax);
diff --git a/raxtax_amd/csrc/rtx_subtile.hip b/raxtax_amd/csrc/rtx_subtile.hip
--- /dev/null
+++ b/raxtax_amd/csrc/rtx_subtile.hip
@@ -0,0 +1,360 @@
+#include <hip/hip_runtime.h>
+
+#include <algorithm>
+
+#include "rtx_bounds2.hpp"
+#include "rtx_hit_common.hpp"
+
+namespace rtx {
+
+__device__ __forceinline__ uint32_t kept_gt(const uint32_t *pl, uint32_t np, uint32_t c) {
+    uint32_t gt = 0, eq = 0xFFFFFFFFu;
+    for (int b = (int)np - 1; b >= 0; b--) {
+        const uint32_t v = pl[(uint32_t)b * 16u], cb = (c >> b) & 1u ? 0xFFFFFFFFu : 0u;
+        gt |= eq & v & ~cb;
+        eq &= ~(v ^ cb);
+    }
+    return (c >> np) ? 0u : gt;
+}
+
+constexpr uint32_t kCodeWhole = 1u << 31, kCodeNoBounds = 1u << 30, kCodeLiveA = 1u << 28;
+
+__device__ __forceinline__ uint32_t stretch_len(uint32_t n, uint32_t waves) { return ((n + waves - 1u) / waves + 63u) & ~63u; }
+
+__global__ __launch_bounds__(256) void subtile_classify_kernel(SubtileParams sp, HitParams hp) {
+    const uint32_t lane = threadIdx.x & 63u, wave = blockIdx.x * 4u + (threadIdx.x >> 6);
+    const uint32_t n = sp.n_items[0], len = stretch_len(n, gridDim.x * 4u);
+    const uint32_t i_end = (uint64_t)(wave + 1u) * len < n ? (wave + 1u) * len : n;
+    uint32_t n_sub = 0, n_whole = 0;
+    for (uint64_t i0 = (uint64_t)wave * len; i0 < i_end; i0 += 64u) {
+        const uint32_t i = (uint32_t)i0 + lane;
+        const bool valid = i < i_end;
+        const uint32_t item = valid ? sp.items[i] : 0u;
+        const uint32_t pair = item / hp.ntiles, tile = item - pair * hp.ntiles;
+        uint32_t mask[2] = {0u, 0u}, code = 0u;
+        bool bounds = true;
+        if (valid)
+            for (uint32_t h = 0; h < 2u; h++) {
+                const uint32_t q = pair * 2u + h;
+                if (q >= hp.nq) continue;
+                if (!((hp.live[(size_t)q * hp.live_words + (tile >> 5)] >> (tile & 31u)) & 1u)) continue;
+                code |= kCodeLiveA << h;
+                const uint32_t ns = hp.rec.nslots ? hp.rec.nslots[q] : 0u, nk = sp.keep_n[q];
+                bool slot = false;
+                for (uint32_t k = 0; k < ns && k < kRecMaxSlots; k++) slot = slot || hp.rec.slots[(size_t)q * kRecMaxSlots + k] == tile;
+                uint32_t e = 0xFFFFFFFFu;
+                if (slot && nk != kKeepNone)
+                    for (uint32_t k = 0; k < nk; k++)
+                        if (sp.keep_bt[(size_t)q * sp.keep_cap + k] == (tile >> 2)) e = k;
+                if (e == 0xFFFFFFFFu) { bounds = false; continue; }
+                const uint32_t u = hp.prune_thr[q];
+                const uint32_t *pl = sp.keep_planes + ((size_t)q * sp.keep_cap + e) * (sp.keep_np * 16u) + (tile & 3u) * 4u;
+                for (uint32_t w = 0; w < 4u; w++) {
+                    const uint32_t gt = kept_gt(pl + w, sp.keep_np, u);
+                    if (gt & 0xFFFFu) mask[h] |= 1u << (w * 2u);
+                    if (gt >> 16) mask[h] |= 2u << (w * 2u);
+                }
+            }
+        const bool few = (uint32_t)__popc(mask[0] | mask[1]) <= kSubtileMax;
+        const bool sub = valid && bounds && few, whole = valid && !sub;
+        code |= mask[0] | (mask[1] << 16) | (whole ? kCodeWhole : 0u) | (bounds ? 0u : kCodeNoBounds);
+        if (valid) sp.codes[i] = code;
+        n_sub += (uint32_t)__popcll(__ballot(sub));
+        n_whole += (uint32_t)__popcll(__ballot(whole));
+    }
+    if (lane == 0u) {
+        sp.parts[wave] = n_sub;
+        sp.parts[sp.n_parts + wave] = n_whole;
+    }
+}
+
+__global__ __launch_bounds__(1024) void subtile_offsets_kernel(SubtileParams sp) {
+    __shared__ uint32_t wsum[2][16];
+    const uint32_t tid = threadIdx.x, lane = tid & 63u, wave = tid >> 6;
+    uint32_t *const count[2] = {sp.sub_count, sp.tile_count};
+    for (uint32_t l = 0; l < 2u; l++) {
+        uint32_t *part = sp.parts + l * sp.n_parts;
+        uint32_t c[4], cnt = 0;
+#pragma unroll
+        for (uint32_t j = 0; j < 4u; j++) {
+            c[j] = tid * 4u + j < sp.n_parts ? part[tid * 4u + j] : 0u;
+            cnt += c[j];
+        }
+        const uint32_t incl = wave_incl_scan_u32(cnt);
+        if (lane == 63u) wsum[l][wave] = incl;
+        __syncthreads();
+        uint32_t o = incl - cnt, tot = 0;
+#pragma unroll
+        for (uint32_t w = 0; w < 16u; w++) {
+            const uint32_t sw = wsum[l][w];
+            o += w < wave ? sw : 0u;
+            tot += sw;
+        }
+#pragma unroll
+        for (uint32_t j = 0; j < 4u; j++) {
+            if (tid * 4u + j < sp.n_parts) part[tid * 4u + j] = o;
+            o += c[j];
+        }
+        if (tid < 9u) count[l][tid] = tid == 0u ? tot : 0u;
+    }
+}
+
+__global__ __launch_bounds__(256) void subtile_scatter_kernel(SubtileParams sp, HitParams hp) {
+    const uint32_t lane = threadIdx.x & 63u, wave = blockIdx.x * 4u + (threadIdx.x >> 6);
+    const uint32_t n = sp.n_items[0], len = stretch_len(n, gridDim.x * 4u);
+    const uint32_t i_end = (uint64_t)(wave + 1u) * len < n ? (wave + 1u) * len : n;
+    const unsigned long long lt_mask = (1ull << lane) - 1ull;
+    uint32_t at_sub = sp.parts[wave], at_whole = sp.parts[sp.n_parts + wave];
+    uint32_t st[kSubtileStats] = {0u, 0u, 0u, 0u, 0u};
+    for (uint64_t i0 = (uint64_t)wave * len; i0 < i_end; i0 += 64u) {
+        const uint32_t i = (uint32_t)i0 + lane;
+        const bool valid = i < i_end;
+        const uint32_t item = valid ? sp.items[i] : 0u, code = valid ? sp.codes[i] : 0u;
+        const bool whole = valid && (code & kCodeWhole), sub = valid && !whole;
+        const unsigned long long bs = __ballot(sub), bw = __ballot(whole);
+        if (sub) {
+            const uint32_t pair = item / hp.ntiles, tile = item - pair * hp.ntiles, masks = code & 0x00FF00FFu;
+            sp.sub_items[at_sub + (uint32_t)__popcll(bs & lt_mask)] = make_uint2(item, masks);
+            for (uint32_t h = 0; h < 2u; h++)
+                if (code & (kCodeLiveA << h)) atomicAnd(&sp.live_lists[(size_t)(pair * 2u + h) * hp.live_words + (tile >> 5)], ~(1u << (tile & 31u)));
+            st[0]++;
+            st[2] += (uint32_t)__popc((masks | (masks >> 16)) & 0xFFu);
+        }
+        if (whole) {
+            sp.tile_items[at_whole + (uint32_t)__popcll(bw & lt_mask)] = item;
+            st[1]++;
+            if (code & kCodeNoBounds) st[3]++;
+            else st[4]++;
+        }
+        at_sub += (uint32_t)__popcll(bs);
+        at_whole += (uint32_t)__popcll(bw);
+    }
+    if (sp.stats) {
+#pragma unroll
+        for (uint32_t k = 0; k < kSubtileStats; k++) {
+            const uint32_t tot = wave_incl_scan_u32(st[k]);
+            if (lane == 63u && tot) atomicAdd(&sp.stats[(size_t)(blockIdx.x & (kPruneStatCopies - 1u)) * 8u + k], (unsigned long long)tot);
+        }
+    }
+}
+
+template <int NP>
+__device__ __forceinline__ void subtile_item(const SubtileParams &sp, const HitParams &p, uint32_t *lds, const uint32_t item, const uint32_t masks,
+                                             const uint32_t lane) {
+    constexpr uint32_t kCap = b2_cap(NP);
+    const uint32_t pair = item / p.ntiles, tile = item - pair * p.ntiles;
+    const uint32_t qa = pair * 2u, qb = qa + 1u;
+    const uint32_t mask_a = masks & 0xFFFFu, mask_b = masks >> 16;
+    const bool has_a = (p.live[(size_t)qa * p.live_words + (tile >> 5)] >> (tile & 31u)) & 1u;
+    const bool has_b = qb < p.nq && ((p.live[(size_t)qb * p.live_words + (tile >> 5)] >> (tile & 31u)) & 1u);
+    uint32_t *l_both = lds, *l_a = lds + kCap, *l_b = lds + 2u * kCap, *l_zero = lds + 3u * kCap;
+    for (uint32_t i = lane; i < kB2Pad; i += 64) l_zero[i] = p.zero_row;
+
+    const uint2 *urec = p.pair_urec + (size_t)pair * p.pair_ustride;
+    const uint32_t n_u = std::min<uint32_t>(p.pair_nu[pair], p.pair_ustride);
+    const unsigned long long lt_mask = (1ull << lane) - 1ull;
+    uint32_t n_both = 0, n_a = 0, n_b = 0;
+    for (uint32_t u0 = 0; u0 < n_u; u0 += 512u) {
+        uint2 rec[8];
+#pragma unroll
+        for (int c = 0; c < 8; c++) {
+            const uint32_t i = u0 + (uint32_t)c * 64u + lane;
+            rec[c] = urec[i < p.pair_ustride ? i : p.pair_ustride - 1u];
+        }
+#pragma unroll
+        for (int c = 0; c < 8; c++) {
+            const uint32_t i = u0 + (uint32_t)c * 64u + lane;
+            const bool in = i < n_u;
+            const bool ia = in && (rec[c].x & (1u << 30)) && mask_a != 0u, ib = in && (rec[c].x & (1u << 31)) && mask_b != 0u;
+            const uint32_t row = rec[c].x & 0x3FFFFFFFu;
+            const bool sh = ia && ib, oa = ia && !ib, ob = ib && !ia;
+            const unsigned long long bs = __ballot(sh), ba = __ballot(oa), bo = __ballot(ob);
+            const uint32_t ps = n_both + (uint32_t)__popcll(bs & lt_mask), pa_ = n_a + (uint32_t)__popcll(ba & lt_mask), pb_ = n_b + (uint32_t)__popcll(bo & lt_mask);
+            if (sh && ps < kCap) l_both[ps] = row;
+            if (oa && pa_ < kCap) l_a[pa_] = row;
+            if (ob && pb_ < kCap) l_b[pb_] = row;
+            n_both += (uint32_t)__popcll(bs);
+            n_a += (uint32_t)__popcll(ba);
+            n_b += (uint32_t)__popcll(bo);
+        }
+    }
+    n_both = std::min(n_both, kCap);
+    n_a = std::min(n_a, kCap);
+    n_b = std::min(n_b, kCap);
+    for (uint32_t i = n_both + lane; i < ((n_both + kB2Pad - 1u) & ~(kB2Pad - 1u)); i += 64) l_both[i] = p.zero_row;
+    for (uint32_t i = n_a + lane; i < ((n_a + kB2Pad - 1u) & ~(kB2Pad - 1u)); i += 64) l_a[i] = p.zero_row;
+    for (uint32_t i = n_b + lane; i < ((n_b + kB2Pad - 1u) & ~(kB2Pad - 1u)); i += 64) l_b[i] = p.zero_row;
+    wave_lds_sync();
+
+    const uint32_t slot_a = has_a ? rec_slot_of(p, qa, tile, lane) : 0xFFFFFFFFu, slot_b = has_b ? rec_slot_of(p, qb, tile, lane) : 0xFFFFFFFFu;
+    const uint32_t u_a = has_a ? (uint32_t)__builtin_amdgcn_readfirstlane((int)p.prune_thr[qa]) : 0u;
+    const uint32_t u_b = has_b ? (uint32_t)__builtin_amdgcn_readfirstlane((int)p.prune_thr[qb]) : 0u;
+    const uint32_t in_tile = (((uint64_t)tile + 1u) << 13) <= p.n_refs ? 8192u : (uint32_t)(p.n_refs - ((uint64_t)tile << 13));
+    const bool skip_exact = (p.flags & RTX_SKIP_EXACT_MATCHES) != 0u;
+    uint32_t run_a = 0, run_b = 0, mx_a = 0, mx_b = 0;
+
+    uint32_t pa[4][NP], pb[4][NP];
+    uint4 buf[4][8];
+    uint32_t n_instr = 0;
+    constexpr int R = kSubRows, NB = 2, SHIFT = 7;
+    constexpr uint32_t kGroup = 8u * (uint32_t)R * (uint32_t)NB;
+    const uint32_t sub8 = lane & 7u, grp8 = lane >> 3, row4 = lane >> 4;
+    const uint32_t wd = sub8 * 4u + row4;
+    const bool owner = (lane & 8u) == 0u;
+    const uint32_t col = sub8 * 16u;
+
+    uint32_t todo = mask_a | mask_b;
+    while (todo) {
+        const uint32_t s = (uint32_t)__builtin_ctz(todo);
+        todo &= todo - 1u;
+        const bool need_a = (mask_a >> s) & 1u, need_b = (mask_b >> s) & 1u;
+        const char *base = reinterpret_cast<const char *>(sp.sbitmap) + ((size_t)tile * kSubPerTile + s) * sp.n_rows1 * kSubRowBytes;
+        const __amdgpu_buffer_rsrc_t rsrc = __builtin_amdgcn_make_buffer_rsrc(const_cast<char *>(base), 0, sp.n_rows1 * kSubRowBytes, 0x00027000);
+#pragma unroll
+        for (int w = 0; w < 4; w++)
+#pragma unroll
+            for (int b = 0; b < NP; b++) { pa[w][b] = 0; pb[w][b] = 0; }
+        const uint32_t g_both = (n_both + kGroup - 1u) / kGroup, g_a = need_a ? (n_a + kGroup - 1u) / kGroup : 0u, g_b = need_b ? (n_b + kGroup - 1u) / kGroup : 0u;
+        const uint32_t *first = g_both ? l_both : (g_a ? l_a : (g_b ? l_b : nullptr));
+        if (first) {
+#pragma unroll
+            for (int b = 0; b < NB; b++) load_unit<SHIFT>(buf[b], rsrc, first + (uint32_t)b * 8u * (uint32_t)R, grp8, col);
+            const uint32_t *after_a = g_b ? l_b : l_zero, *after_both = g_a ? l_a : after_a;
+            if (g_both) {
+                fold_list<NP, 1, R, NB, SHIFT>(pa, pb, buf, l_both, g_both, after_both, grp8, col, rsrc);
+#pragma unroll
+                for (int w = 0; w < 4; w++)
+#pragma unroll
+                    for (int b = 0; b < NP; b++) pb[w][b] = pa[w][b];
+            }
+            if (g_a) fold_list<NP, 1, R, NB, SHIFT>(pa, pb, buf, l_a, g_a, after_a, grp8, col, rsrc);
+            if (g_b) fold_list<NP, 2, R, NB, SHIFT>(pa, pb, buf, l_b, g_b, l_zero, grp8, col, rsrc);
+            n_instr += (g_both + g_a + g_b) * 8u * (uint32_t)NB;
+        }
+        auto emit = [&](const uint32_t (&pl)[4][NP], uint32_t q, uint32_t u, uint32_t slot, uint32_t &running, uint32_t &mx) {
+            uint32_t r[NP];
+            reduce_rows<NP>(pl, lane, r);
+            {
+                uint32_t sh[NP];
+#pragma unroll
+                for (int pp = 0; pp < NP; pp++) sh[pp] = (uint32_t)__builtin_amdgcn_update_dpp(0, (int)r[pp], 0x128, 0xF, 0xF, true);
+                planes_add<NP>(r, sh);
+            }
+            const uint32_t rl0 = s * kSubRefs + wd * 32u;
+            if (skip_exact) {
+                const uint64_t qin = p.perm[p.q0 + q];
+                uint64_t e0, e1;
+                const uint32_t *xids;
+                exact_range(p.exact, qin, e0, e1, xids);
+                for (uint64_t e = e0; e < e1; e++) {
+                    const uint32_t id = xids[e] - p.ref_base;
+                    if (id < p.n_refs && (id >> 13) == tile && ((id & 8191u) >> 5) == (rl0 >> 5)) {
+                        const uint32_t msk = ~(1u << (id & 31u));
+#pragma unroll
+                        for (int b = 0; b < NP; b++) r[b] &= msk;
+                    }
+                }
+            }
+            uint32_t cand = owner ? planes_gt<NP>(r, u) : 0u;
+            if (rl0 >= in_tile) cand = 0u;
+            else if (in_tile - rl0 < 32u) cand &= (1u << (in_tile - rl0)) - 1u;
+            if (__ballot(cand != 0u) == 0ull) return;
+            const uint32_t nc = (uint32_t)__popc(cand);
+            uint32_t before = 0, total = 0;
+#pragma unroll
+            for (uint32_t k = 0; k < kSubRefs / 32u; k++) {
+                const uint32_t v = (uint32_t)__shfl((int)nc, (int)((k & 3u) * 16u + (k >> 2)), 64);
+                before += k < wd ? v : 0u;
+                total += v;
+            }
+            uint32_t pos = running + before;
+            uint32_t *seg = p.rec.rec + ((size_t)q * p.rec.stride + slot) * p.rec.seg_len;
+            uint32_t *hist = p.hist + (size_t)q * p.hstride;
+            while (cand) {
+                const uint32_t j = (uint32_t)__builtin_ctz(cand);
+                cand &= cand - 1u;
+                uint32_t c = 0;
+#pragma unroll
+                for (int b = 0; b < NP; b++) c |= ((r[b] >> j) & 1u) << b;
+                if (pos < p.rec.seg_len) seg[pos] = (rl0 + j) | (c << 13);
+                pos++;
+                atomicAdd(&hist[c], 1u);
+                mx = c > mx ? c : mx;
+            }
+            running += total;
+        };
+        if (need_a) emit(pa, qa, u_a, slot_a, run_a, mx_a);
+        if (need_b) emit(pb, qb, u_b, slot_b, run_b, mx_b);
+    }
+    auto leave = [&](uint32_t q, uint32_t slot, uint32_t running, uint32_t mx) {
+        mx = wave_max_u32(mx);
+        if (lane == 0u) {
+            atomicAdd(&p.hist[(size_t)q * p.hstride], in_tile - running);
+            if (running > p.rec.seg_len) atomicOr(p.rec.flags_out, 8u);
+            p.rec.cnt[(size_t)q * kRecMaxSlots + slot] = running < p.rec.seg_len ? running : p.rec.seg_len;
+            if (running == 0u) atomicAnd(const_cast<uint32_t *>(p.live) + (size_t)q * p.live_words + (tile >> 5), ~(1u << (tile & 31u)));
+            if (p.tile_max) p.tile_max[(size_t)q * p.ntiles + tile] = (uint16_t)mx;
+        }
+    };
+    if (has_a && slot_a != 0xFFFFFFFFu) leave(qa, slot_a, run_a, mx_a);
+    if (has_b && slot_b != 0xFFFFFFFFu) leave(qb, slot_b, run_b, mx_b);
+    if (lane == 0u && p.group_rows) atomicAdd(&p.group_rows[p.group_base + pair], n_instr);
+}
+
+template <int NP>
+__global__ __launch_bounds__(64, 2) void subtile_count_kernel(SubtileParams sp, HitParams p) {
+    extern __shared__ uint32_t st_lds[];
+    const uint32_t lane = threadIdx.x;
+    const uint32_t n_items = (uint32_t)__builtin_amdgcn_readfirstlane((int)sp.sub_count[0]), g8 = gridDim.x >> 3, x = blockIdx.x & 7u;
+    const uint32_t e8 = (n_items + 7u) >> 3, first = x * e8;
+    const uint32_t end = first + e8 < n_items ? first + e8 : n_items;
+    uint32_t j = first + (blockIdx.x >> 3);
+    while (j < end) {
+        const uint2 it = sp.sub_items[j];
+        const uint32_t item = (uint32_t)__builtin_amdgcn_readfirstlane((int)it.x), masks = (uint32_t)__builtin_amdgcn_readfirstlane((int)it.y);
+        uint32_t lane_v = lane;
+        asm volatile("" : "+v"(lane_v));
+        subtile_item<NP>(sp, p, st_lds, item, masks, lane_v);
+        wave_lds_sync();
+        if (e8 <= g8) break;
+        uint32_t nxt = 0;
+        if (lane_v == 0u) nxt = atomicAdd(&sp.sub_count[1u + x], 1u);
+        j = first + g8 + (uint32_t)__builtin_amdgcn_readfirstlane((int)nxt);
+    }
+}
+
+void launch_subtile_split(hipStream_t s, const SubtileParams &sp, const HitParams &hp) {
+    const uint32_t blocks = sp.n_parts / 4u;
+    hipLaunchKernelGGL(subtile_classify_kernel, dim3(blocks), dim3(256), 0, s, sp, hp);
+    hipLaunchKernelGGL(subtile_offsets_kernel, dim3(1), dim3(1024), 0, s, sp);
+    hipLaunchKernelGGL(subtile_scatter_kernel, dim3(blocks), dim3(256), 0, s, sp, hp);
+}
+
+void launch_subtile_count(hipStream_t s, const SubtileParams &sp, const HitParams &hp, int planes) {
+    const uint32_t np = (hp.nq + 1u) / 2u;
+    const dim3 grid((uint32_t)((std::min<uint64_t>((uint64_t)np * hp.ntiles, std::max<uint64_t>(2ull * np, 2048ull)) + 7u) & ~7ull));
+    const size_t lds = (size_t)b2_lds_dw(10) * 4u;
+    if (planes <= 8) hipLaunchKernelGGL((subtile_count_kernel<8>), grid, dim3(64), lds, s, sp, hp);
+    else hipLaunchKernelGGL((subtile_count_kernel<10>), grid, dim3(64), lds, s, sp, hp);
+}
+
+__global__ __launch_bounds__(256) void subtile_build_kernel(const uint32_t *__restrict__ bitmap, uint32_t n_rows1, uint32_t stride_bytes,
+                                                            uint8_t *__restrict__ sbitmap) {
+    const uint32_t row = blockIdx.x, tile = blockIdx.y, word = threadIdx.x;
+    const uint32_t v = bitmap[((size_t)tile * n_rows1 + row) * 256u + word];
+    if (v == 0u) return;
+    const uint32_t l = word >> 2, wi = word & 3u, L = tile_lanes(stride_bytes, tile);
+    if (l >= L) return;
+#pragma unroll
+    for (uint32_t k = 0; k < 4u; k++) {
+        const uint32_t byte = (v >> (8u * k)) & 0xFFu;
+        if (byte == 0u) continue;
+        const uint32_t rl = ((wi * 4u + k) * L + l) * 8u;
+        sbitmap[(((size_t)tile * kSubPerTile + rl / kSubRefs) * n_rows1 + row) * kSubRowBytes + ((rl % kSubRefs) >> 3)] = (uint8_t)byte;
+    }
+}
+void launch_subtile_build(hipStream_t s, const uint32_t *bitmap, uint32_t n_rows1, uint32_t ntiles, uint32_t stride_bytes, uint8_t *sbitmap) {
+    hipLaunchKernelGGL(subtile_build_kernel, dim3(n_rows1, ntiles), dim3(256), 0, s, bitmap, n_rows1, stride_bytes, sbitmap);
+}
+
+}
```

Result: faster. 13.87 million, median of 6 (+6.4%).
